# wadx2019/rpo

Measured on AMD Instinct MI355X. Metric: env-steps/sec (whole node), SafeCartpole-v0 (CartSafe-v0) RPODDPG, rollout + one batch-256 constrained policy update per vector step, higher is better.
Workload: dtype f32; 1 GPU; CartSafe-v0 RPODDPG, 4096 vectorised envs per MI355X, scripts/cart_exp.py hyper-parameters, update batch 256 every vector step (reference cadence), replay capacity 20000 per env; envs_per_gpu=4096, global_envs=4096, update_batch=256, hip_graph=True, training_batch_projection=row-wise, rccl_ranks=0, collectives_in_graph=False, graphs_replayed_on_all_ranks=True, graph_capture_fell_back_to_eager=False

## Files before the change

### include/rpo_hip.h

```cpp
#ifndef RPO_HIP_H
#define RPO_HIP_H

#ifdef __cplusplus
extern "C" {
#endif

#define RPO_ABI_VERSION 6

#define RPO_ERR_ARG (-1)
#define RPO_ERR_NULL (-2)

#define RPO_CART_STATE_DIM 6
#define RPO_CART_ACTION_DIM 2
#define RPO_CART_INEQ 6
#define RPO_CART_ROW 24
#define RPO_CART_RING 32
#define RPO_CART_CONSTS_LEN 35

#define RPO_PEND_INTERNAL_DIM 4
#define RPO_PEND_OBS_DIM 5
#define RPO_PEND_ACTION_DIM 2
#define RPO_PEND_ROW 16
#define RPO_PEND_RING 16

// ... 259 lines not shown
int rpo_mlp_split_head(const rpo_mlp* net_host, int n, const float* part, float* out, int out_mode, float scale,
                       float base, void* stream);

typedef struct {
    const rpo_mlp *actor, *actor_target, *critic1, *critic2, *critic_target1, *critic_target2;
    const rpo_mlp_grad *critic1_grad, *critic2_grad, *actor_grad;
    int env;
    int twin;
    int batch;
    const float* rows; long long cap_steps; int n_envs;
    float* batch_out; long long* idx_out; const long long* idx_in;
    unsigned long long sample_seed; unsigned sample_salt;
    const float* eps_in; unsigned long long noise_seed; unsigned noise_id_base, noise_salt;
    const long long* ctrl;
    float scale, base, box_lo, box_hi;
    int max_steps; float corr_lr, corr_eps, corr_momentum;
    const float* consts_host; int partial;
    float alpha, gamma;
    float eps_start, eps_end, eps_decay;
    float *part_pi, *part_q1, *part_q2, *part_qn1, *part_qn2;
    float *x0_1, *h1_1, *x0_2, *h1_2, *x0_a, *h1_a;
    float *logp;
    float *next_actions;
    int *proj_iters;
    float *dq1, *dq2;
    float *loss_partial;
    float *dx0_1, *dx0_2, *dx0_a;
    float *gradmax;
    const float* nu; float* nu_grad;
    float *ap_det, *noise_out, *raw, *actions, *g_act, *lag_partial, *lag_out, *da_part, *dout;
    int shared_embedding;
    long long* rollout_ctrl; float* rollout_stats; int rollout_stats_cap;
    int* prep_step; float prep_beta1, prep_beta2; long long* clock_out; float* gradmax_reset;
    int* prep2_step[3]; float prep2_beta1[3], prep2_beta2[3]; float* gradmax_reset2;
    long long* updates_out;
    float* part_pol;
    unsigned* tile_sync;
    unsigned long long* proj_ws; int proj_store_mode;
    int debug;
} rpo_split_update;


int rpo_split_critic_fwd_a(const rpo_split_update* u, void* stream);
int rpo_split_critic_fwd_b(const rpo_split_update* u, void* stream);
int rpo_split_critic_front(const rpo_split_update* u, void* stream);
int rpo_split_critic_front_pol(const rpo_split_update* u, void* stream);
int rpo_split_critic_mid(const rpo_split_update* u, void* stream);
int rpo_split_critic_mid_pol(const rpo_split_update* u, void* stream);
int rpo_split_critic_pfront(const rpo_split_update* u, void* stream);
int rpo_split_critic_pfront_pol(const rpo_split_update* u, void* stream);
int rpo_xcc_probe(int gx, int gy, int gz, int threads, int* out, void* stream);
int rpo_hw_probe(int gx, int gy, int gz, int threads, int lds_bytes, int spin, int* out, void* stream);
int rpo_split_critic_fwd_b_pol(const rpo_split_update* u, void* stream);
int rpo_split_pend_head_project(const rpo_split_update* u, void* stream);
int rpo_split_critic_bwd_a(const rpo_split_update* u, void* stream);
int rpo_split_critic_bwd_b(const rpo_split_update* u, void* stream);
int rpo_split_policy_a(const rpo_split_update* u, void* stream);
int rpo_split_policy_b(const rpo_split_update* u, void* stream);
int rpo_split_policy_c(const rpo_split_update* u, void* stream);
int rpo_split_policy_d(const rpo_split_update* u, void* stream);
int rpo_split_policy_e(const rpo_split_update* u, void* stream);
int rpo_split_policy_front(const rpo_split_update* u, void* stream);
int rpo_split_policy_front_bc(const rpo_split_update* u, void* stream);

typedef struct {
    int n_envs;
    int gauss;
    float scale, base;
    float* state;
    float* obs;
    float* action;
    int* ep_len; float* ep_ret; unsigned* ep_count;
    float* rows; long long cap_steps;
    float* stats; int stats_cap;
    int noise_mode;
    long long* ctrl;
    float eps_start, eps_end, eps_decay, box_lo, box_hi;
    int max_steps; float corr_lr, corr_eps, corr_momentum;
    int max_episode_steps, auto_reset;
    float viol_thresh;
    unsigned env_id_base;
    unsigned long long seed;
    float* part;
    int lane_begin, lane_end;
    int defer_clock;
} rpo_rollout_rider;

int rpo_split_critic_fwd_a_ride(const rpo_split_update* u, const rpo_rollout_rider* r, void* stream);
int rpo_split_critic_fwd_b_ride(const rpo_split_update* u, const rpo_rollout_rider* r, void* stream);
int rpo_split_critic_bwd_b_ride(const rpo_split_update* u, const rpo_rollout_rider* r, void* stream);
int rpo_split_critic_front_ride(const rpo_split_update* u, const rpo_rollout_rider* r, void* stream);
int rpo_split_critic_mid_ride(const rpo_split_update* u, const rpo_rollout_rider* r, void* stream);
int rpo_split_critic_pfront_ride(const rpo_split_update* u, const rpo_rollout_rider* r, void* stream);

int rpo_mlp_backward(const rpo_mlp* net_host, const rpo_mlp_grad* grad_host, int n, const float* s, int s_stride,
                     const float* a, int a_stride, const float* x0, const float* h1, const float* dout, float* dh,
                     float* dx0, float* da, int param_grads, int first_layer_state_only, float* gradmax,
                     const rpo_td* td, void* stream);

int rpo_mlp_backward_pair(const rpo_mlp* net1_host, const rpo_mlp_grad* grad1_host, const rpo_mlp* net2_host,
                          const rpo_mlp_grad* grad2_host, int n, const float* s, int s_stride, const float* a,
                          int a_stride, const float* x0_1, const float* h1_1, const float* dout_1, float* dh_1,
                          float* dx0_1, float* da_1, const float* x0_2, const float* h1_2, const float* dout_2, float* dh_2,
                          float* dx0_2, float* da_2, int param_grads, int first_layer_state_only, float* gradmax,
                          const rpo_td* td1, const rpo_td* td2, void* stream);


int rpo_evopf_reset(int n_envs, float* state, int* ep_len, float* ep_ret, const unsigned* ep_count,
                    const float* consts_dev, unsigned long long seed, unsigned env_id_base, void* stream);

int rpo_evopf_step(int n_envs, float* state, const float* action, int* ep_len, float* ep_ret, unsigned* ep_count,
                   float* rows, long long cap_steps, float* stats, int stats_cap, long long* ctrl, int max_episode_steps,
                   int auto_reset, float viol_thresh, const float* consts_dev, unsigned long long seed,
                   unsigned env_id_base, void* stream);

int rpo_evopf_act_project(int n, const float* state, int state_stride, const float* ap_raw, const float* noise, float* action, int* iters,
                          int noise_mode, int ap_is_raw, float eps_start, float eps_end, float eps_decay, int max_steps,
                          float corr_lr, float corr_eps, float corr_momentum, float newton_tol, int newton_max_iters,
                          const float* consts_dev, unsigned long long seed, unsigned env_id_base, const long long* ctrl,
                          float* stats, int stats_cap, void* stream);

int rpo_evopf_tanh_box_bwd(int n, const float* state, int state_stride, const float* raw, const float* noise,
                           float eps_start, float eps_end, float eps_decay, const long long* ctrl, const float* dap,
                           float* dout, const float* consts_dev, void* stream);

int rpo_evopf_gauss_head(int n, const float* state, int state_stride, const float* raw, const float* eps, int deterministic,
                         float* ap_out, float* logp_out, const float* consts_dev, void* stream);
int rpo_evopf_gauss_head_bwd(int n, const float* state, int state_stride, const float* raw, const float* eps,
                             const float* dap, float dlogp, float* draw, const float* consts_dev, void* stream);

int rpo_evopf_complete_bwd(int n, const float* action, const float* grad_action, const float* grad_action_b, const float* grad_action2,
                           float* grad_ap, const float* consts_dev, void* stream);

int rpo_evopf_resid(int n, const float* state, int state_stride, const float* action, float* eq_out, float* ineq_out,
                    const float* consts_dev, void* stream);

int rpo_evopf_ineq_partial_grad(int n, const float* state, int state_stride, const float* action, float* step_out, const float* consts_dev,
                                void* stream);

int rpo_evopf_eq_vjp(int n, const float* action, const float* grad_eq, float* grad_action, int autograd_sign,
                     const float* consts_dev, void* stream);

int rpo_evopf_lagrangian(int n, const float* state, int state_stride, const float* action, const float* nu, float scale, float* loss_out,
                         float* grad_action, float* grad_nu, const float* consts_dev, int overwrite, void* stream);


int rpo_cartsafe_rollout(const rpo_mlp* actor_host, int gauss, float scale, float base, int n_envs, float* state,
                         float* action, int* ep_len, float* ep_ret, unsigned* ep_count, float* rows, long long cap_steps,
                         float* stats, int stats_cap, long long* ctrl, int noise_mode, float eps_start, float eps_end,
                         float eps_decay, float box_lo, float box_hi, int max_steps, float corr_lr, float corr_eps,
                         float corr_momentum, const float* consts_host, int partial, int max_episode_steps,
                         int auto_reset, float viol_thresh, unsigned long long seed, unsigned env_id_base, int defer_clock,
                         void* stream);
int rpo_pendulum_rollout(const rpo_mlp* actor_host, int gauss, float scale, float base, int n_envs, float* internal,
                         float* obs, float* action, int* ep_len, float* ep_ret, unsigned* ep_count, float* rows,
                         long long cap_steps, float* stats, int stats_cap, long long* ctrl, int noise_mode,
                         float eps_start, float eps_end, float eps_decay, float box_lo, float box_hi, int max_steps,
                         float corr_lr, float corr_eps, float corr_momentum, int max_episode_steps, int auto_reset,
                         float viol_thresh, unsigned long long seed, unsigned env_id_base, int defer_clock, void* stream);

int rpo_cartsafe_evaluate(const rpo_mlp* actor_host, int gauss, float scale, float base, int n_envs, float* state,
                          float* action, int* ep_len, float* ep_ret, unsigned* ep_count, long long* ctrl, float* acc, int t0,
                          int steps, float box_lo, float box_hi, int max_steps, float corr_lr, float corr_eps,
                          float corr_momentum, const float* consts_host, int partial, int max_episode_steps,
                          float viol_thresh, void* stream);
int rpo_pendulum_evaluate(const rpo_mlp* actor_host, int gauss, float scale, float base, int n_envs, float* internal,
                          float* obs, float* action, int* ep_len, float* ep_ret, unsigned* ep_count, long long* ctrl,
                          float* acc, int t0, int steps, float box_lo, float box_hi, int max_steps, float corr_lr,
                          float corr_eps, float corr_momentum, int max_episode_steps, float viol_thresh, void* stream);

int rpo_cartsafe_evaluate_record(const rpo_mlp* actor_host, int gauss, float scale, float base, int n_envs, float* state,
                                 float* action, int* ep_len, float* ep_ret, unsigned* ep_count, long long* ctrl, float* acc,
                                 int t0, int steps, float box_lo, float box_hi, int max_steps, float corr_lr, float corr_eps,
                                 float corr_momentum, const float* consts_host, int partial, int max_episode_steps,
                                 float viol_thresh, float* trace, int trace_rows, int trace_steps, void* stream);
int rpo_pendulum_evaluate_record(const rpo_mlp* actor_host, int gauss, float scale, float base, int n_envs, float* internal,
                                 float* obs, float* action, int* ep_len, float* ep_ret, unsigned* ep_count, long long* ctrl,
                                 float* acc, int t0, int steps, float box_lo, float box_hi, int max_steps, float corr_lr,
                                 float corr_eps, float corr_momentum, int max_episode_steps, float viol_thresh, float* trace,
                                 int trace_rows, int trace_steps, void* stream);

int rpo_cartsafe_evaluate_constraints(const rpo_mlp* actor_host, int gauss, float scale, float base, int n_envs, float* state,
                                      float* action, int* ep_len, float* ep_ret, unsigned* ep_count, long long* ctrl,
                                      float* acc, int t0, int steps, float box_lo, float box_hi, int max_steps, float corr_lr,
                                      float corr_eps, float corr_momentum, const float* consts_host, int partial,
                                      int max_episode_steps, float viol_thresh, float* trace, int trace_rows, int trace_steps,
                                      float* con, void* stream);
int rpo_pendulum_evaluate_constraints(const rpo_mlp* actor_host, int gauss, float scale, float base, int n_envs,
                                      float* internal, float* obs, float* action, int* ep_len, float* ep_ret,
                                      unsigned* ep_count, long long* ctrl, float* acc, int t0, int steps, float box_lo,
                                      float box_hi, int max_steps, float corr_lr, float corr_eps, float corr_momentum,
                                      int max_episode_steps, float viol_thresh, float* trace, int trace_rows, int trace_steps,
                                      float* con, void* stream);

int rpo_cartsafe_evaluate_noisy(const rpo_mlp* actor_host, int gauss, float scale, float base, int n_envs, float* state,
                                float* action, int* ep_len, float* ep_ret, unsigned* ep_count, long long* ctrl, float* acc,
                                int t0, int steps, float box_lo, float box_hi, int max_steps, float corr_lr, float corr_eps,
                                float corr_momentum, const float* consts_host, int partial, int max_episode_steps,
                                float viol_thresh, float* trace, int trace_rows, int trace_steps, float* con,
                                const float* sigma_host, int sigma_len, unsigned long long noise_seed, void* stream);
int rpo_pendulum_evaluate_noisy(const rpo_mlp* actor_host, int gauss, float scale, float base, int n_envs, float* internal,
                                float* obs, float* action, int* ep_len, float* ep_ret, unsigned* ep_count, long long* ctrl,
                                float* acc, int t0, int steps, float box_lo, float box_hi, int max_steps, float corr_lr,
                                float corr_eps, float corr_momentum, int max_episode_steps, float viol_thresh, float* trace,
                                int trace_rows, int trace_steps, float* con, const float* sigma_host, int sigma_len,
                                unsigned long long noise_seed, void* stream);

int rpo_cartsafe_evaluate_budgets(const rpo_mlp* actor_host, int gauss, float scale, float base, int n_envs, float* state,
                                  float* action, int* ep_len, float* ep_ret, unsigned* ep_count, long long* ctrl, float* acc,
                                  int t0, int steps, float box_lo, float box_hi, int max_steps, float corr_lr, float corr_eps,
                                  float corr_momentum, const float* consts_host, int partial, int max_episode_steps,
                                  float viol_thresh, float* trace, int trace_rows, int trace_steps, float* con,
                                  const int* lane_steps, const float* lane_lr, void* stream);
int rpo_pendulum_evaluate_budgets(const rpo_mlp* actor_host, int gauss, float scale, float base, int n_envs, float* internal,
                                  float* obs, float* action, int* ep_len, float* ep_ret, unsigned* ep_count, long long* ctrl,
                                  float* acc, int t0, int steps, float box_lo, float box_hi, int max_steps, float corr_lr,
                                  float corr_eps, float corr_momentum, int max_episode_steps, float viol_thresh, float* trace,
                                  int trace_rows, int trace_steps, float* con, const int* lane_steps, const float* lane_lr,
                                  void* stream);

int rpo_cartsafe_evaluate_policies(const rpo_mlp* actor_host, int gauss, float scale, float base, int n_envs, float* state,
                                   float* action, int* ep_len, float* ep_ret, unsigned* ep_count, long long* ctrl, float* acc,
                                   int t0, int steps, float box_lo, float box_hi, int max_steps, float corr_lr, float corr_eps,
                                   float corr_momentum, const float* consts_host, int partial, int max_episode_steps,
                                   float viol_thresh, float* con, int policy_stride, int group_lanes, int episodes,
                                   void* stream);
int rpo_pendulum_evaluate_policies(const rpo_mlp* actor_host, int gauss, float scale, float base, int n_envs, float* internal,
                                   float* obs, float* action, int* ep_len, float* ep_ret, unsigned* ep_count, long long* ctrl,
                                   float* acc, int t0, int steps, float box_lo, float box_hi, int max_steps, float corr_lr,
                                   float corr_eps, float corr_momentum, int max_episode_steps, float viol_thresh, float* con,
                                   int policy_stride, int group_lanes, int episodes, void* stream);

int rpo_cartsafe_evaluate_noise_sweep(const rpo_mlp* actor_host, int gauss, float scale, float base, int n_envs, float* state,
                                      float* action, int* ep_len, float* ep_ret, unsigned* ep_count, long long* ctrl,
                                      float* acc, int t0, int steps, float box_lo, float box_hi, int max_steps, float corr_lr,
                                      float corr_eps, float corr_momentum, const float* consts_host, int partial,
                                      int max_episode_steps, float viol_thresh, float* con, const float* sigma_table,
                                      unsigned long long noise_seed, int group_lanes, int episodes, void* stream);
int rpo_pendulum_evaluate_noise_sweep(const rpo_mlp* actor_host, int gauss, float scale, float base, int n_envs,
                                      float* internal, float* obs, float* action, int* ep_len, float* ep_ret,
                                      unsigned* ep_count, long long* ctrl, float* acc, int t0, int steps, float box_lo,
                                      float box_hi, int max_steps, float corr_lr, float corr_eps, float corr_momentum,
                                      int max_episode_steps, float viol_thresh, float* con, const float* sigma_table,
                                      unsigned long long noise_seed, int group_lanes, int episodes, void* stream);

int rpo_eval_obs_noise(int n, const float* obs, int obs_stride, int obs_dim, const float* sigma, unsigned long long seed,
                       int step, float* out, int out_stride, void* stream);

int rpo_cartsafe_policy_act(const rpo_mlp* actor_host, int gauss, float scale, float base, int n, const float* obs,
                            int obs_stride, float* action, float* proposal, int* iters, float* eq_resid, float* ineq_resid,
                            float box_lo, float box_hi, int max_steps, float corr_lr, float corr_eps, float corr_momentum,
                            const float* consts_host, int partial, int form, void* stream);
int rpo_pendulum_policy_act(const rpo_mlp* actor_host, int gauss, float scale, float base, int n, const float* obs,
                            int obs_stride, float* action, float* proposal, int* iters, float* eq_resid, float* ineq_resid,
                            float box_lo, float box_hi, int max_steps, float corr_lr, float corr_eps, float corr_momentum,
                            int form, void* stream);

int rpo_cartsafe_policy_act_profile(const rpo_mlp* actor_host, int gauss, float scale, float base, int n, const float* obs,
                                    int obs_stride, float* action, float* proposal, int* iters, float* eq_resid,
                                    float* ineq_resid, float box_lo, float box_hi, int max_steps, float corr_lr, float corr_eps,
                                    float corr_momentum, const float* consts_host, int partial, float* profile, void* stream);
int rpo_pendulum_policy_act_profile(const rpo_mlp* actor_host, int gauss, float scale, float base, int n, const float* obs,
                                    int obs_stride, float* action, float* proposal, int* iters, float* eq_resid,
                                    float* ineq_resid, float box_lo, float box_hi, int max_steps, float corr_lr, float corr_eps,
                                    float corr_momentum, float* profile, void* stream);
int rpo_cartsafe_project_profile(int n, const float* ap_raw, float* action, int* iters, int max_steps, float corr_lr,
                                 float corr_eps, float corr_momentum, const float* consts_host, int partial, float* profile,
                                 void* stream);
int rpo_pendulum_project_profile(int n, const float* obs, int obs_stride, const float* ap_raw, float* action, int* iters,
                                 int max_steps, float corr_lr, float corr_eps, float corr_momentum, float* profile,
                                 void* stream);

int rpo_eval_record(int n, const float* rows, int row_stride, int reward_col, int done_col, int eq_col, int eq_num,
                    int ineq_col, int ineq_num, const float* obs, int obs_stride, int obs_dim, const float* proposal,
                    int partial_dim, const float* action, int action_dim, const int* iters, int step, const float* acc,
                    float* trace, int trace_rows, int trace_steps, void* stream);

int rpo_eval_constraints(int n, const float* rows, int row_stride, int eq_col, int eq_num, int ineq_col, int ineq_num, int step,
                         float viol_thresh, const float* acc, float* con, void* stream);

int rpo_eval_accumulate(int n, const float* rows, int row_stride, int reward_col, int done_col, int eq_col, int eq_num,
                        int ineq_col, int ineq_num, const int* iters, int step, float viol_thresh, float* acc, void* stream);

int rpo_eval_summarize(int n, const float* acc, const long long* ctrl, double* row_out, double* ws, void* stream);

int rpo_eval_keep_best(long long n_params, const float* src, float* best, const double* row, double* best_row,
                       long long* best_point, long long point, double max_violation_rate, void* stream);

int rpo_cartsafe_ddpg_critic_forward(const rpo_mlp* actor_target_host, const rpo_mlp* critic_target_host,
                                     const rpo_mlp* critic_host, float scale, float base, const float* rows,
                                     long long cap_steps, int n_envs, int batch, float* batch_out, long long* idx_out,
                                     const long long* idx_in, unsigned long long seed, unsigned sample_salt,
                                     const long long* ctrl, int max_steps, float corr_lr, float corr_eps,
                                     float corr_momentum, float box_lo, float box_hi, const float* consts_host,
                                     int partial, float* q_out, float* qn_out, float* x0_save, float* h1_save,
                                     void* stream);

int rpo_ddpg_actor_forward(int env, const rpo_mlp* actor_host, const rpo_mlp* critic_host, float scale, float base,
                                    float box_lo, float box_hi, float eps_start, float eps_end, float eps_decay,
                                    const float* batch, int batch_size, const float* noise_in, unsigned long long seed,
                                    unsigned noise_id_base, unsigned noise_salt, const long long* ctrl, const float* nu,
                                    const float* consts_host, int partial, float* ap_det, float* noise_out,
                                    float* actions, float* q_out, float* dq_out, float* g_act, float* partial_out,
                                    float* actor_x0, float* actor_h1, float* critic_x0, float* critic_h1, void* stream);
int rpo_ddpg_actor_backward(int env, const rpo_mlp* actor_host, const rpo_mlp_grad* actor_grad_host,
                                     const rpo_mlp* critic_host, int shared_embedding, const float* batch,
// ... 73 lines not shown
```

### rpo_amd/algo/rpo_ddpg.py

```python
import torch

from .. import ops as hip_ops
from .agent import PDDDPG_PA
from .model import BoxConstraint
from .agent.flat import FusedAdam
from .trainer import _SALT_ACTOR, RPOTrainerBase, _LagrangianFn, _TDHuberFn


class _LazySum(object):

    def __init__(self, parts):
        self.parts = parts

    def __float__(self):
        return float(self.parts.sum())

    def detach(self):
        return self.parts.sum()


class _LazyDiff(object):

    def __init__(self, pair):
        self.pair = pair
# ... 105 lines not shown
        td = self.backend.Td(q.view(-1), qn.view(-1), None, None, cols[3], cols[4], 0.0, self.agent.gamma,
                             f.buf("dq", B, 1).view(-1), parts)
        self._zero_grads()
        gm = self._critic_gradmax()
        f.backward("critic", cols[0], cols[1], None, gradmax=gm, td=td)
        self._gradmax_ready = gm is not None
        self.last_losses["critic"] = _LazySum(parts)

    def _critic_update(self, cols):
        if self.fused is None:
            return super()._critic_update(cols)
        if self._pipelines:
            su = self._split_state()
            if su is not None:
                return self._critic_update_split(su)
            return self._critic_update_pipeline(cols)
        f, ag, B = self.fused, self.agent, self.batch_size
        state, action, next_state, reward, done = cols[:5]
        next_actions = self._project_batch(next_state, self._actor_out("actor_target", next_state))
        qn, q = f.forward_multi([("critic_target", next_state, next_actions, f.buf("qn", B, 1), False),
                                 ("critic", state, action, f.buf("q", B, 1), True)])
        self._critic_backward_td(cols, q, qn, f.buf("loss_parts", (B + 15) // 16))

    @property
    def _actor_pipeline(self):
        d = self.fused.descs if self.fused is not None else {}
        return (hasattr(self.backend, "ddpg_actor_forward") and "actor" in d and "critic" in d and d["actor"].E == 128
                and d["critic"].E == 128 and not d["critic"].cat and self._box_affine is not None
                and self.kernels.partial_dim == 1 and self.kernels.action_dim == 2
                and self.schedule["fused_actor"] and not self._large_batch)

    def _actor_update_pipeline(self, cols):
        f, ag, B, k = self.fused, self.agent, self.batch_size, self.kernels
        da_, dc = f.descs["actor"], f.descs["critic"]
        scale, base = self._box_affine
        b = f.buf
        parts = b("actor.parts", (B + 15) // 16, 8)
        ap_det, noise, actions = b("act.ap_det", B), b("act.noise", B), b("act_pi", B, k.action_dim)
        q, dq, g_act = b("q_pi", B, 1), b("dq_pi", B, 1), b("g_act", B, k.action_dim)
        noise_in = None
        if self._idx_inject is not None:
            self.backend.philox_normal(self._noise_b, self.seed, self.dist.rank * B * k.partial_dim, _SALT_ACTOR, hip_ops.STREAM_POLICY,
                                       self._uctrl)
            noise_in = self._noise_b.view(-1)
        self.backend.ddpg_actor_forward(k, da_, dc, scale, base, self._box_lo, self._box_hi, self.eps_start, self.eps, self.decay_value,
                             self._batch, noise_in, self.seed, self.dist.rank * B, _SALT_ACTOR, self._uctrl,
                             ag.nju.weight.view(-1), ap_det, noise, actions, q, dq, g_act, parts, b("actor.x0", B, da_.ein),
                             b("actor.h1", B, da_.H), b("critic.x0", B, dc.ein), b("critic.h1", B, dc.H))
        self._zero_grads()
        shared = ag.flat.sizes[1] > 0
        opt = ag.actor_optim
        fuse_max = self._self_cleaning and not self.dist.on and opt.clip_thres and opt.clip_thres != float("inf")
        lag = b("actor.lag", 2)
        self.backend.ddpg_actor_backward(k, da_, dc, shared, self._batch, actions, g_act, ap_det, noise, dq, self.eps_start, self.eps,
                              self.decay_value, self._box_lo, self._box_hi, scale, base, self._uctrl,
                              b("actor.x0", B, da_.ein), b("actor.h1", B, da_.H), b("critic.x0", B, dc.ein),
                              b("critic.h1", B, dc.H), b("actor.dh", B, da_.H), b("actor.dx0", B, da_.ein),
                              b("critic.dh", B, dc.H), b("critic.dx0", B, dc.ein), b("da", B, k.action_dim), b("do", B),
                              parts, lag, ag.nju.weight.grad.view(-1), opt.gradmax if fuse_max else None)
        self._actor_gradmax_ready = bool(fuse_max)
        loss = _LazyDiff(lag)
        self.last_losses["actor"] = loss
        return loss

    def _actor_update(self, cols):
        if self.fused is None:
            return super()._actor_update(cols)
        if self._actor_pipeline:
            su = self._split_state()
            if su is not None:
                lag, _, _ = self._actor_update_split(su)
                loss = _LazyDiff(lag)
                self.last_losses["actor"] = loss
                return loss
            return self._actor_update_pipeline(cols)
        f, ag, B, k = self.fused, self.agent, self.batch_size, self.kernels
        state = cols[0]
        pre, self._actor_pre = getattr(self, "_actor_pre", None), None
        if pre is None:
            pre = self._actor_prefix(cols)
        ap_det, noise, actions, lag, g_act, fa = pre
        q = f.forward("critic", state, actions, f.buf("q_pi", B, 1), save=True)
        dq = self._const_dq(B)
        da = f.buf("da", B, k.action_dim)
        shared = ag.flat.sizes[1] > 0
        f.backward("critic", state, actions, dq, da=da, param_grads=shared, first_layer_state_only=True)
        P = k.partial_dim
        dap, do = f.buf("dap", B * P), f.buf("do", B, P)
        if fa:
            k.complete_bwd(state, da, dap, action=actions, grad_action2=g_act)
        else:
            da.add_(g_act)
            k.complete_bwd(state, da, dap, action=actions)
        if self._box_affine is None:
            k.tanh_box_bwd(state, ap_det, noise, self.eps_start, self.eps, self.decay_value, self._uctrl, dap, do.view(-1))
        else:
            scale, base = self._box_affine
            self.backend.tanh_box_bwd(dap, ap_det, noise, self.eps_start, self.eps, self.decay_value, self._uctrl,
                                      self._box_lo, self._box_hi, scale, base, do.view(-1))
        opt = ag.actor_optim
        fuse_max = self._self_cleaning and not self.dist.on and opt.clip_thres and opt.clip_thres != float("inf") and not shared
        f.backward("actor", state, None, do, gradmax=opt.gradmax if fuse_max else None)
        self._actor_gradmax_ready = bool(fuse_max)
        loss = _LazyMeanDiff(lag, q)
        self.last_losses["actor"] = loss
        return loss

    def _actor_prefix(self, cols):
        f, ag, B, k = self.fused, self.agent, self.batch_size, self.kernels
        state = cols[0]
        ap_det = self._actor_out("actor", state, save=True, tag="pi")
        self.backend.philox_normal(self._noise_b, self.seed, self.dist.rank * B * k.partial_dim, _SALT_ACTOR, hip_ops.STREAM_POLICY,
                                   self._uctrl)
        noise = self._noise_b.view(-1)
        actions = self._complete_only(state, ap_det, noise)
        lag, g_act = f.buf("loss_lag", 1), f.buf("g_act", B, k.action_dim)
        fa = bool(getattr(k, "fused_adds", False))
        if not fa:
            lag.zero_()
        self._zero_grads()
        k.lagrangian(actions, ag.nju.weight.view(-1), 1.0 / B, lag, g_act, ag.nju.weight.grad.view(-1), obs=state,
                     **(dict(overwrite=True) if fa else {}))
        return ap_det, noise, actions, lag, g_act, fa

    def _const_dq(self, B):
        key = ("dq_pi_const", B)
        if key not in self.fused._scratch:
            self.fused._scratch[key] = torch.full((B, 1), -1.0 / B, device=self.device)
        return self.fused._scratch[key]

    def critic_loss(self, state, action, next_state, done, reward, ineq_viol=None, eq_viol=None):
        ag = self.agent
        with torch.no_grad():
            next_partial = ag.take_action(next_state, deterministic=True, target=True)
            next_actions = self.process_action(next_state, next_partial)
            next_q = ag.critic_target(next_state, next_actions)
        q = ag.critic(state, action)
        return _TDHuberFn.apply(self.backend, ag.gamma, 0.0, reward, done, next_q, None, None, q, None)

    def actor_loss(self, state):
        ag = self.agent
        ap = ag.actor(state)
        self.backend.philox_normal(self._noise_b, self.seed, self.dist.rank * self.batch_size * self.kernels.partial_dim, _SALT_ACTOR,
                                   hip_ops.STREAM_POLICY, self._uctrl)
        ap = ag.actor.box_constraint.clip(ap + self._eps_now() * self._noise_b, state)
        actions = self.base_env.complete_partial(state, ap)
        loss = (-ag.critic(state, actions)).mean()
        return loss + _LagrangianFn.apply(self.kernels, actions, ag.nju.weight, state)

    def _critic_step(self, actor_step):
        ag = self.agent
        fuse = actor_step and ag.flat.sizes[1] == 0
        prepared, self._critic_prepared = getattr(self, "_critic_prepared", False), False
        ag.critic_optim.step(target=ag.critic_target_flat if fuse else None, tau=ag.tau,
                             gradmax_ready=self._gradmax_ready, clock=self._clock(not actor_step), prepared=prepared)
        self._gradmax_ready = False

    def _actor_step(self, actor_out):
        ag, fl = self.agent, self.agent.flat
        c = fl.actor_range[0]
        sh = fl.critic_range[1] - c if fl.sizes[1] > 0 else 0
        segs = [ag.actor_optim.segment(target=ag.actor_target_flat, tau=ag.tau,
                                       gradmax_ready=getattr(self, "_actor_gradmax_ready", False),
                                       target2=ag.critic_target_flat[c:c + sh] if sh > 0 else None, n2=sh)]
        self._actor_gradmax_ready = False
        if not self.fixed:
            segs.append(ag.nju_optim.segment())
        if sh > 0 and c > 0:
            segs.append(dict(polyak_only=True, param=fl.param((0, c)), target=ag.critic_target_flat[:c], tau=ag.tau))
        prepared, self._actor_prepared = getattr(self, "_actor_prepared", False), False
        FusedAdam.step_many(self.backend, segs, clock=self._clock(True), prepared=prepared)
```

### rpo_amd/algo/trainer.py

```python
import contextlib
import copy
import os

import numpy as np
import torch
import torch.distributed as dist

from .. import ops as hip_ops
from .agent.fused import FusedNets
from .model import BoxConstraint



class NonFiniteError(FloatingPointError):
    """An env lane was stepped with a NaN action or reached a non-finite state (ctrl[RPO_CTRL_NONFINITE] of the step
    kernels; the reference's `assert self.action_space.contains(action_fixed)`, cartpole.py:170-174, pendulum.py:85-89)."""


_SALT_CRITIC = 1 << 20
_SALT_ACTOR = 2 << 20


class _TDHuberFn(torch.autograd.Function):

# ... 29 lines not shown
        return loss[0]

    @staticmethod
    def backward(ctx, grad_out):
        g_a, g_nu = ctx.saved_tensors
        return None, grad_out * g_a, grad_out * g_nu.view(ctx.nu_shape), None


class _Dist(object):
    def __init__(self, force=False):
        init = dist.is_available() and dist.is_initialized()
        self.on = init and (dist.get_world_size() > 1 or bool(force))
        self.rank = dist.get_rank() if self.on else 0
        self.world = dist.get_world_size() if self.on else 1
        self.in_graph = self.on and dist.get_backend() == "nccl"

    def mean_(self, tensors):
        if not self.on:
            return
        avg = dist.get_backend() == "nccl"
        for t in tensors:
            if avg:
                dist.all_reduce(t, op=dist.ReduceOp.AVG)
            else:
                dist.all_reduce(t, op=dist.ReduceOp.SUM)
                t.mul_(1.0 / self.world)

    def sync_initial_state(self, seed, agent, device):
        bufs = [agent.flat.data, agent.critic_target_flat]
        if agent.actor_target_flat is not None:
            bufs.append(agent.actor_target_flat)
        for b in bufs:
            dist.broadcast(b, src=0)
        s = torch.tensor([int(seed)], dtype=torch.int64, device=device)
        dist.broadcast(s, src=0)
        return int(s.item())

    def sum_(self, t):
        if self.on:
            dist.all_reduce(t, op=dist.ReduceOp.SUM)
        return t

    def all_ok(self, ok, device):
        if not self.on:
            return bool(ok)
        flag = torch.tensor([1 if ok else 0], dtype=torch.int32, device=device)
        dist.all_reduce(flag, op=dist.ReduceOp.MIN)
        return bool(int(flag.item()))

    def replaying_everywhere(self, graphs, device):
        mine = bool(graphs.enabled and not graphs.capture_failed and any(e["graph"] is not None for e in graphs.entries.values()))
        return self.all_ok(mine, device)


_NODE_KINDS = ("kernel", "memcpy", "memset", "host", "graph", "empty", "wait_event", "event_record", "sem_signal", "sem_wait",
               "mem_alloc", "mem_free", "memcpy_from_symbol", "memcpy_to_symbol", "batch_mem_op")


def _graph_node_kinds(g):
    import ctypes
    from .. import _lib
    _lib._bind_to_torch_hip_runtime()
    bundled = os.path.join(os.path.dirname(torch.__file__), "lib", "libamdhip64.so")
    hip = ctypes.CDLL(bundled if os.path.exists(bundled) else "libamdhip64.so", mode=ctypes.RTLD_GLOBAL)
    graph = ctypes.c_void_p(int(g.raw_cuda_graph()))
    n = ctypes.c_size_t(0)
    if hip.hipGraphGetNodes(graph, None, ctypes.byref(n)) != 0:
        raise RuntimeError("hipGraphGetNodes failed")
    nodes = (ctypes.c_void_p * max(1, n.value))()
    if n.value and hip.hipGraphGetNodes(graph, nodes, ctypes.byref(n)) != 0:
        raise RuntimeError("hipGraphGetNodes failed")
    kinds = {}
    for i in range(n.value):
        t = ctypes.c_int(-1)
        if hip.hipGraphNodeGetType(ctypes.c_void_p(nodes[i]), ctypes.byref(t)) != 0:
            raise RuntimeError("hipGraphNodeGetType failed")
        name = _NODE_KINDS[t.value] if 0 <= t.value < len(_NODE_KINDS) else "type_%d" % t.value
        kinds[name] = kinds.get(name, 0) + 1
    return kinds


class _GraphCache(object):

    def __init__(self, enabled, warm=3, owner=None):
        self.enabled, self.warm = enabled, warm
        self.capture_failed = False
        self.entries = {}
        self.side = None
        self.audit = os.environ.get("RPO_GRAPH_AUDIT", "0") == "1"
        import weakref
        self._owner = weakref.ref(owner) if owner is not None else None

    def run(self, key, fn):
        if not self.enabled:
            return fn()
        e = self.entries.setdefault(key, {"count": 0, "graph": None})
        if e["graph"] is not None:
            e["graph"].replay()
            return
        if e["count"] < self.warm:
            e["count"] += 1
            if self.side is None:
                self.side = torch.cuda.Stream()
            cur = torch.cuda.current_stream()
            self.side.wait_stream(cur)
            with torch.cuda.stream(self.side):
                fn()
            cur.wait_stream(self.side)
            return
        g = torch.cuda.CUDAGraph(keep_graph=True) if self.audit else torch.cuda.CUDAGraph()
        owner = self._owner() if self._owner is not None else None
        state = owner._host_state() if owner is not None else None
        import gc
        gc_was_on = gc.isenabled()
        gc.collect()
        gc.disable()
        failure = None
        try:
            try:
                with torch.cuda.graph(g, capture_error_mode="thread_local"):
                    fn()
            except Exception as exc:
                failure = exc
            ok_everywhere = failure is None
            if owner is not None and owner.dist.on and owner.dist.world > 1:
                ok_everywhere = owner.dist.all_ok(failure is None, owner.device)
            if not ok_everywhere:
                import warnings
                why = "%s: %s" % (type(failure).__name__, failure) if failure is not None else "another rank's capture failed"
                warnings.warn("hipGraph capture failed (%s); continuing with eager launches" % why)
                self.enabled = False
                self.capture_failed = True
                del g
                torch.cuda.synchronize()
                if owner is not None:
                    owner._set_host_state(state)
                fn()
                return
            e["graph"] = g
            if self.audit:
                e["node_kinds"] = _graph_node_kinds(g)
            g.replay()
        finally:
            if gc_was_on:
                gc.enable()


def _env_int(name, default):
    v = os.environ.get(name)
    return default if v in (None, "") else int(v)


SCHEDULE_DEFAULTS = dict(fused_mlp=1, fused_rollout=1, fused_critic=1, fused_actor=1, split=1, ride=1, front=1, branch=1,
                         fused_eval=1, fused_act=1, eval_overlap=1, force_dist=0)


def parse_schedule(overrides=None):
    out = dict(SCHEDULE_DEFAULTS)
    text = os.environ.get("RPO_SCHEDULE", "")
    for item in filter(None, (x.strip() for x in text.split(","))):
        k, _, v = item.partition("=")
        if k.strip() not in out:
            raise ValueError("RPO_SCHEDULE: unknown part %r (have: %s)" % (k, ", ".join(sorted(out))))
        out[k.strip()] = int(v) if v.strip() else 1
    for k, v in (overrides or {}).items():
        if k not in out:
            raise ValueError("schedule: unknown part %r (have: %s)" % (k, ", ".join(sorted(out))))
        out[k] = int(v)
    return out


class RPOTrainerBase(object):

    sac = False

    def _setup(self, env, work_dir, name, logger, agent, hp, device, num_envs=None, seed=None, backend=None,
               use_graph=None, updates_per_step=None, fused=None, schedule=None):
        self.env, self.agent, self.device = env, agent, device
        self.schedule = parse_schedule(schedule)
        if fused is not None:
            self.schedule["fused_mlp"] = int(bool(fused))
        self.work_dir, self.name, self.logger = work_dir, name, logger
        for k, v in hp.items():
            setattr(self, k, v)
        if self.eval_steps is None:
            self.eval_steps = self.max_steps
        if self.corr_mode != 0:
            raise ValueError("corr_mode=%r: only corr_mode=0 (reduced-gradient projection) is defined; the reference's "
                             "corr_mode=1 branch (rpo_ddpg.py:276-278) raises a shape error for every env" % (self.corr_mode,))
        self.backend = backend if backend is not None else hip_ops
        self.base_env = getattr(env, "unwrapped", env)
        self.kernels = self.base_env.kernels
        self.env_eval = copy.deepcopy(self.env)
        self.box_constraint = BoxConstraint(*self.base_env.box_constraint, device=device)
        self.decay_value = (hp["eps_start"] - hp["eps"]) / hp["eps_epoch"]
        self.dist = _Dist(force=self.schedule["force_dist"])
        n_total = int(num_envs) if num_envs is not None else _env_int("RPO_NUM_ENVS", 1)
        if n_total % self.dist.world:
            raise ValueError("num_envs (%d) must be divisible by the world size (%d)" % (n_total, self.dist.world))
        self.num_envs, self.n_local = n_total, n_total // self.dist.world
        if seed is None:
            seed = _env_int("RPO_SEED", None)
        if seed is None:
            seed = int(torch.randint(0, 2 ** 62, (1,)).item())
        if self.dist.on:
            seed = self.dist.sync_initial_state(seed, agent, device)
        self.seed = int(seed)
        self.max_episode_steps = getattr(env, "_max_episode_steps", None)
        self.vec = self.base_env.make_vec(self.n_local, seed=self.seed, env_id_base=self.dist.rank * self.n_local,
                                          max_episode_steps=self.max_episode_steps, device=device)
        self.buffer = agent.attach_env(self.kernels, self.n_local, self.seed + 7919 * (self.dist.rank + 1), self.vec.ctrl)
        self._batch = torch.zeros(self.batch_size, self.kernels.row_floats, device=device)
        P = self.kernels.partial_dim
        self._noise_b = torch.zeros(self.batch_size, P, device=device)
        self._noise_n = torch.zeros(self.n_local, P, device=device)
        self._box_lo, self._box_hi = self.base_env.partial_box
        cycle = _env_int("RPO_GRAPH_CYCLE", 16)
        if use_graph is None:
            use_graph = cycle > 0 and device.type == "cuda"
        self._graphs = _GraphCache(use_graph, owner=self)
        self._tail = None
        self._last_cols = self._last_actor_out = None
        self._cycle = max(cycle, 1) // max(1, self.policy_fre) * max(1, self.policy_fre)
        rowwise = _env_int("RPO_ROWWISE_PROJECTION", None)
        self.batch_reference = not bool(rowwise)
        if self.batch_size > 1024 and self.batch_reference and hasattr(self.kernels, "project_batchref"):
            raise ValueError(
                "batch_size=%d > 1024 on %s: the reference's sample-coupled batched projection is defined up to 1024 rows "
                "here; set RPO_ROWWISE_PROJECTION=1 to project training batches row by row (per-sample stop test, "
                "no coupling between samples)" % (self.batch_size, self.kernels.name))
        self.projection_mode = ("batch-reference" if self.batch_reference and hasattr(self.kernels, "project_batchref")
                                else "row-wise")
        self.fused = FusedNets.build(agent, self.backend, device) if self.schedule["fused_mlp"] else None
        if self.fused is not None and self.batch_size >= hip_ops.CONST.get("RPO_SPLITK_FROM", 1 << 30) and device.type == "cuda":
            self.fused.enable_splitk(self.batch_size)
        self.updates_per_step = max(1, int(updates_per_step) if updates_per_step is not None
                                    else _env_int("RPO_UPDATES_PER_STEP", 1))
        self._updates = 0
        box = agent.actor.box_constraint
        self._box_affine = (float(np.asarray(box.scale).reshape(-1)[0]), float(np.asarray(box.base).reshape(-1)[0])) \
            if box is not None and not box.volatile else None
        self._self_cleaning = self.fused is not None
        self._gradmax_ready = False
        for opt in (agent.critic_optim, agent.actor_optim, agent.nju_optim):
            opt.zero_grad_after = self._self_cleaning
        self._act_kw = dict(ap_is_raw=True) if (self.fused is not None and self._box_affine is None) else {}
        self._uctrl, self._uclock_ok, self._ovl_stream = self.vec.ctrl, True, None
        self._ride, self._rider_cache, self._ride_cut = None, None, 0
        self._clock_pending, self._iter_actor_step, self._critic_prepared, self._gradmax_stale = False, None, False, False
        self._actor_prepared, self._actor_gradmax_stale = False, False
        self._bump_updates_now, self._updates_out, self._pol_a_done = False, None, False
        self._bump = self.updates_per_step == 1
        if self.fused is not None and device.type == "cuda" and getattr(self.backend, "ADAM_CLOCK", False):
            self._uctrl, self._uclock_ok = torch.zeros_like(self.vec.ctrl), False
        self.buffer.sample_ctrl = self._uctrl
        self._split_state()
        self._t = 0
        self._harvested = 0
        self._pending = []
        self._vec_eval = None
        self.last_losses = {}
        self._idx_inject = None
        self._eval_init_inject = None
        self.viol_steps, self.env_steps, self.viol_rate, self.proj_iters_mean = 0.0, 0.0, 0.0, 0.0
        from .evaluation import CurveRunner
        ee = getattr(self, "eval_episodes", None)
        if ee is None:
            ee = _env_int("RPO_EVAL_EPISODES", None)
        from .evaluation import check_keep_best, keep_best_from_env
        kb = getattr(self, "keep_best", None)
        if kb is None:
            kb = keep_best_from_env(os.environ.get("RPO_KEEP_BEST"))
        kb = check_keep_best(kb)
        if kb is not None and ee is None:
            raise ValueError("keep_best needs curve mode: the points it chooses among are those of eval_episodes=N "
                             "(RPO_EVAL_EPISODES), which is not set")
        self._curve = CurveRunner(self, ee, keep_best=kb) if ee is not None else None
        self.eval_episodes = self._curve.n if self._curve is not None else None
        self.keep_best = False if kb is None else kb

    def process_action(self, state, action_partial, train=True):
        ref = self.batch_reference
        if train:
            return self.base_env.project(state, action_partial, self.max_steps, self.corr_lr, self.corr_eps,
                                         self.corr_momentum, batch_reference=ref)
        action, iters = self.base_env.project(state, action_partial, self.eval_steps, self.eval_lr, self.corr_eps,
                                              self.corr_momentum, return_iters=True, batch_reference=ref)
        return action, int(iters.max())

    def grad_steps(self, state, action, train=True):
        idx = torch.as_tensor(np.asarray(self.base_env.partial_actions), device=self.device)
        return self.process_action(state, torch.as_tensor(action, device=self.device)[:, idx], train=train)

    def _policy_partial(self, obs, warm):
        raise NotImplementedError

    _gauss_policy = False

    @property
    def _large_batch(self):
        return self.batch_size >= hip_ops.CONST.get("RPO_SPLITK_FROM", 1 << 30)

    @property
    def _rollout_pipeline(self):
        return (self.fused is not None and hasattr(self.kernels, "rollout") and "actor" in self.fused.descs
                and self.schedule["fused_rollout"])

    @property
    def _defer_ok(self):
        return bool(getattr(self, "_pipelines", False) and self._split_state() is not None)

    def _rollout(self, warm, defer_clock=False):
        v = self.vec
        defer_clock = bool(defer_clock and not warm and self._rollout_pipeline and self._defer_ok)
        if not warm and self._rollout_pipeline:
            scale, base = self._box_affine
            self.kernels.rollout(self.fused.descs["actor"], self._gauss_policy, scale, base, v.internal,
                                 None if v.obs is v.internal else v.obs, v.action, v.ep_len, v.ep_ret, v.ep_count,
                                 self.buffer.rows, self.buffer.capacity, v.stats, v.ctrl,
                                 hip_ops.NOISE_NONE if self._gauss_policy else hip_ops.NOISE_PHILOX, self.eps_start,
                                 self.eps, self.decay_value, self._box_lo, self._box_hi, self.max_steps, self.corr_lr,
                                 self.corr_eps, self.corr_momentum, v.max_episode_steps, True, v.viol_thresh, self.seed,
                                 v.env_id_base, **(dict(defer_clock=True) if defer_clock else {}))
            self._clock_pending = defer_clock
            v.steps_host += 1
            return
        with torch.no_grad():
            ap, mode = self._policy_partial(v.obs, warm)
            self.kernels.act_project(v.obs, ap, None, v.action, None, mode, self.eps_start, self.eps, self.decay_value,
                                     self._box_lo, self._box_hi, self.max_steps, self.corr_lr, self.corr_eps,
                                     self.corr_momentum, self.seed, v.env_id_base, v.ctrl, v.stats,
                                     **({} if warm else self._act_kw))
            v.step(v.action, rows=self.buffer.rows, cap_steps=self.buffer.capacity, auto_reset=True)

    def _sample(self):
        self.buffer.sample_rows(self.batch_size, out=self._batch)
        c = self.buffer.split(self._batch)
        return c["state"], c["action"], c["next_state"], c["reward"], c["done"], c["ineq_viol"], c["eq_viol"]

    def _eps_now(self):
        if self.decay_value == 0:
            return self.eps_start
        t = self._uctrl[0].to(torch.float32)
        return torch.clamp(self.eps_start - self.decay_value * t, min=self.eps)

    def _critic_gradmax(self):
        opt = self.agent.critic_optim
        ok = self._self_cleaning and not self.dist.on and opt.clip_thres and opt.clip_thres != float("inf")
        self._gradmax_ready = False
        return opt.gradmax if ok else None

    def _zero_grads(self):
        if not self._self_cleaning:
            self.agent.flat.grad.zero_()
        elif self.fixed:
            self.agent.nju.weight.grad.zero_()

    def _critic_update(self, cols):
        state, action, next_state, reward, done, ineq_viol, eq_viol = cols
        loss = self.critic_loss(state, action, next_state, done, reward, ineq_viol, eq_viol)
        self.agent.flat.grad.zero_()
        loss.backward()
        self.last_losses["critic"] = loss.detach()

    def _actor_update(self, cols):
        out = self.actor_loss(cols[0])
        loss = out[0] if isinstance(out, tuple) else out
        self.agent.flat.grad.zero_()
        loss.backward()
        self.last_losses["actor"] = loss.detach()
        return tuple(x.detach() for x in out) if isinstance(out, tuple) else loss.detach()

    def _segments(self, warm, do_train, actor_step, rollout=True):
        ag, fl = self.agent, self.agent.flat
        segs = []
        if not do_train:
            return [(lambda: self._rollout(warm), [])]

        def s1():
            if rollout:
                self._rollout(warm, defer_clock=True)
            self._last_cols = self._sample()
            self._iter_actor_step = actor_step
            self._bump_updates_now = self._updates_inkernel
            self._critic_update(self._last_cols)
        segs.append((s1, [fl.gradient(fl.critic_range)]))
        if actor_step:
            def s2():
                self._critic_step(actor_step)
                self._last_actor_out = self._actor_update(self._last_cols)
            segs.append((s2, [fl.gradient(fl.policy_bucket)]))

            def s3():
                self._actor_step(self._last_actor_out)
            segs.append((s3, []))
        else:
            segs.append((lambda: self._critic_step(actor_step), []))
        return segs

    def _critic_step(self, actor_step):
        raise NotImplementedError

    def _clock(self, last):
        return self._uctrl if (last and self._bump and self._uctrl is not self.vec.ctrl) else None

    def _sync_uclock(self, rollout_pending):
        if self._uctrl is self.vec.ctrl or self._uclock_ok:
            return
        if rollout_pending:
            torch.add(self.vec.ctrl[0:1], 1, out=self._uctrl[0:1])
        else:
            self._uctrl[0:1].copy_(self.vec.ctrl[0:1])

    def _actor_step(self, actor_out):
        raise NotImplementedError

    def _policy_optims(self):
        ag = self.agent
        out = [ag.actor_optim]
        if not self.fixed:
            out.append(ag.nju_optim)
        if getattr(self, "automatic_entropy_tuning", False):
            out.append(ag.alpha_optim)
        return out

    def _iteration(self, warm, do_train, actor_step, rollout=True):
        segs = self._segments(warm, do_train, actor_step, rollout)
        if do_train:
            self._sync_uclock(rollout_pending=rollout)
        self._uclock_ok = do_train and self._bump
        if not self.dist.on or self.dist.in_graph:
            self._graphs.run((warm, do_train, actor_step, rollout), lambda: self._run_segments(segs))
            return
        tail, self._tail = self._tail, None
        for i, (fn, reduce_after) in enumerate(segs):
            key = (warm, do_train, actor_step, rollout, i)
            if i == 0 and tail is not None:
                prev_fn, first = tail[1], fn
                key, fn = ("after",) + tail[0] + key, (lambda: (prev_fn(), first()))
            if i == len(segs) - 1 and not reduce_after and i > 0:
                self._tail = (key, fn)
                return
            self._graphs.run(key, fn)
            self.dist.mean_(reduce_after)

    def _run_segments(self, segs):
        for fn, reduce_after in segs:
            fn()
            self.dist.mean_(reduce_after)

    def _flush_tail(self):
        tail, self._tail = self._tail, None
        if tail is not None:
            self._graphs.run(tail[0], tail[1])

    @property
    def _updates_inkernel(self):
        return bool(self.updates_per_step > 1 and getattr(self, "_pipelines", False) and getattr(self, "_actor_pipeline", False)
                    and self._split_state() is not None)

    def _extra_body(self, actor_step):
        if self._updates_inkernel:
            self._bump_updates_now = True
        else:
            self._uctrl[hip_ops.CONST["RPO_CTRL_UPDATES"]] += 1
        cols = self._sample()
        self._iter_actor_step = actor_step
        self._critic_update(cols)
        fl = self.agent.flat
        self.dist.mean_([fl.gradient(fl.critic_range)])
        self._critic_step(actor_step)
        if actor_step:
            out = self._actor_update(cols)
            self.dist.mean_([fl.gradient(fl.policy_bucket)])
            self._actor_step(out)

    def _extra_updates(self):
        F, k, U = self.policy_fre, 1, self.updates_per_step
        while k < U:
            L = self._cycle
            if L > 1 and U - k >= L and self._updates % F == 0 and self._graphs.enabled and \
                    (not self.dist.on or self.dist.in_graph):
                base = self._updates
                self._graphs.run(("extra", L), lambda: [self._extra_body((base + j + 1) % F == 0) for j in range(L)])
            else:
                L = 1
                actor_step = (self._updates + 1) % F == 0
                if self.dist.on and not self.dist.in_graph:
                    self._extra_body(actor_step)
                else:
                    self._graphs.run(("extra", actor_step), lambda: self._extra_body(actor_step))
            self._updates += L
            k += L

    def train(self, t):
        self._uclock_ok = False
        self._sync_uclock(rollout_pending=False)
        bump, self._bump = self._bump, False
        try:
            self._train_body(t)
        finally:
            self._bump = bump
            self._uclock_ok = False

    def _train_body(self, t):
        cols = self._sample()
        actor_step = self._iter_actor_step = t % self.policy_fre == 0
        self._critic_update(cols)
        fl = self.agent.flat
        self.dist.mean_([fl.gradient(fl.critic_range)])
        self._critic_step(actor_step)
        if actor_step:
            out = self._actor_update(cols)
            self.dist.mean_([fl.gradient(fl.policy_bucket)])
            self._actor_step(out)

    def _split_state(self):
        if getattr(self, "_split_cache", False) is not False:
            return self._split_cache
        self._split_cache = None
        f, k, be = self.fused, self.kernels, self.backend
        if f is None or not hasattr(be, "SplitUpdate") or not self.schedule["split"] or self._box_affine is None \
                or self.device.type != "cuda":
            return None
        if not isinstance(k, (be.CartSafeKernels, be.PendulumKernels)) or self.batch_size > 1024:
            return None
        if isinstance(k, be.PendulumKernels) and not self.batch_reference:
            return None
        d = f.descs
        names = ("actor", "critic1", "critic2", "critic_target1", "critic_target2") if self.sac else \
            ("actor", "actor_target", "critic", "critic_target")
        if any(n not in d or not be.mlp_split_supported(d[n]) for n in names):
            return None
        B, ag, buf = self.batch_size, self.agent, self.buffer
        T = (B + 15) // 16
        b = f.buf
        descs = dict(actor=d["actor"])
        if self.sac:
            descs.update(critic1=d["critic1"], critic2=d["critic2"], critic_target1=d["critic_target1"],
                         critic_target2=d["critic_target2"])
        else:
            descs.update(actor_target=d["actor_target"], critic1=d["critic"], critic_target1=d["critic_target"])
        scale, base = self._box_affine
        c1 = "critic1" if self.sac else "critic"
        fields = dict(
            rows=buf.rows, cap_steps=buf.capacity, n_envs=buf.n_envs, batch_out=self._batch, sample_seed=buf.seed,
            sample_salt=0, noise_seed=self.seed, noise_id_base=self.dist.rank * B, noise_salt=_SALT_CRITIC, ctrl=self._uctrl,
            scale=scale, base=base, box_lo=self._box_lo, box_hi=self._box_hi, max_steps=self.max_steps,
            corr_lr=self.corr_lr, corr_eps=self.corr_eps, corr_momentum=self.corr_momentum,
            alpha=float(getattr(ag, "alpha", 0.0)), gamma=ag.gamma, eps_start=self.eps_start, eps_end=self.eps,
            eps_decay=self.decay_value,
            part_pi=b("split.part_pi", 8, B, 2), part_pol=b("split.part_pol", 8, B, 2),
            part_q1=b("split.part_q1", 8, B, 2), part_qn1=b("split.part_qn1", 8, B, 2),
            x0_1=b(c1 + ".x0", B, d[c1].ein), h1_1=b(c1 + ".h1", B, d[c1].H), dq1=b("dq1" if self.sac else "dq", B, 1),
            dx0_1=b(c1 + ".dx0", B, d[c1].ein), loss_partial=b("split.loss_parts", 2, T),
            next_actions=b("split.next_actions", B, 2), logp=b("crit.logp", B),
            tile_sync=torch.zeros((3 * T + 1) * 32, dtype=torch.int32, device=self.device))
        if self.sac:
            fields.update(part_q2=b("split.part_q2", 8, B, 2), part_qn2=b("split.part_qn2", 8, B, 2),
                          x0_2=b("critic2.x0", B, d["critic2"].ein), h1_2=b("critic2.h1", B, d["critic2"].H),
                          dq2=b("dq2", B, 1), dx0_2=b("critic2.dx0", B, d["critic2"].ein))
        da_ = d["actor"]
        fields.update(nu=ag.nju.weight.view(-1), nu_grad=ag.nju.weight.grad.view(-1), noise_out=b("act.noise", B),
                      actions=b("act_pi", B, 2), g_act=b("g_act", B, 2), lag_partial=b("actor.parts", T, 8),
                      lag_out=b("actor.lag", 2), da_part=b("split.da_part", 2, 8, B, 2), dout=b("split.dout", B, 2),
                      x0_a=b("actor.x0", B, da_.ein), h1_a=b("actor.h1", B, da_.H), dx0_a=b("actor.dx0", B, da_.ein),
                      shared_embedding=int(ag.flat.sizes[1] > 0))
        if self.sac:
            fields.update(raw=b("pi.raw", B, 2))
        else:
            fields.update(ap_det=b("act.ap_det", B))
        if isinstance(k, be.PendulumKernels) and self.schedule["front"] and B <= 256 and self.max_steps <= 30:
            fields.update(proj_ws=torch.zeros(hip_ops.PROJ_WS_WORDS, dtype=torch.int64, device=self.device), proj_store_mode=1)
        self._split_cache = be.SplitUpdate(k, descs, self.sac, B, fields)
        self._front_cache = bool(self.schedule["front"]) and hasattr(be, "front_launch_ok") and be.front_launch_ok(B, self.sac)
        self._pfront = bool(self._front_cache and "proj_ws" in fields and be.front_launch_ok(B, self.sac, 1))
        self._split_loss = fields["loss_partial"]
        self._split_logp = (fields["logp"], b("pi.logp", B))
        return self._split_cache

    def _actor_update_split(self, su):
        B, ag, k = self.batch_size, self.agent, self.kernels
        noise_in = None
        if self._idx_inject is not None:
            self.backend.philox_normal(self._noise_b, self.seed, self.dist.rank * B * k.partial_dim, _SALT_ACTOR,
                                       hip_ops.STREAM_POLICY, self._uctrl)
            noise_in = self._noise_b.view(-1)
        crit_logp, pi_logp = self._split_logp
        su.set(noise_salt=_SALT_ACTOR, eps_in=noise_in, logp=pi_logp)
        early, self._pol_a_done = self._pol_a_done, False
        front = self._front_ok()
        if front:
            su.run("policy_front_bc" if early else "policy_front")
        else:
            if not early:
                su.run("policy_a")
            su.run("policy_b")
            su.run("policy_c")
        self._zero_grads()
        opt = ag.actor_optim
        fuse_max = self._self_cleaning and not self.dist.on and opt.clip_thres and opt.clip_thres != float("inf")
        su.set(gradmax=opt.gradmax if fuse_max else None)
        if not front:
            su.run("policy_d")
        prep = bool(fuse_max) and bool(getattr(self, "_pipelines", False))
        optims = [o for o in self._policy_optims() if o is not None] if prep else []
        su.set_prep2([(o.step_dev, o.betas[0], o.betas[1]) for o in optims])
        su.set(clock_out=self._clock(True) if prep else None, updates_out=self._updates_out)
        su.run("policy_e")
        su.set(clock_out=None, updates_out=None)
        self._updates_out = None
        self._actor_prepared = prep
        self._actor_gradmax_stale = prep
        su.set(noise_salt=_SALT_CRITIC, eps_in=None, logp=crit_logp)
        self._actor_gradmax_ready = bool(fuse_max)
        f = self.fused
        return f.buf("actor.lag", 2), f.buf("actor.parts", (B + 15) // 16, 8), pi_logp

    def _set_hand_overs(self, su, actor_step):
        opt = self.agent.critic_optim
        prep = actor_step is not None
        self._critic_prepared = bool(prep)
        bump_updates, self._bump_updates_now = self._bump_updates_now, False
        self._updates_out = self._uctrl if bump_updates else None
        pending, self._clock_pending = self._clock_pending, False
        su.set(prep_step=opt.step_dev if prep else None, prep_beta1=opt.betas[0], prep_beta2=opt.betas[1],
               clock_out=self._clock(not actor_step) if prep else None,
               updates_out=self._updates_out if not actor_step else None,
               gradmax_reset=opt.gradmax if (prep or self._gradmax_stale) else None,
               gradmax_reset2=self.agent.actor_optim.gradmax if (prep or self._actor_gradmax_stale) else None,
               rollout_ctrl=self.vec.ctrl if pending else None, rollout_stats=self.vec.stats if pending else None,
               rollout_stats_cap=self.vec.stats.shape[0] if pending else 0)
        self._gradmax_stale, self._actor_gradmax_stale = bool(prep), False

    def _critic_update_split(self, su):
        inject = self._idx_inject is not None
        idx_in = self._idx_inject() if inject else None
        eps_in = None
        if inject and self.sac:
            B = self.batch_size
            self.backend.philox_normal(self._noise_b, self.seed, self.dist.rank * B * self.kernels.partial_dim, _SALT_CRITIC,
                                       hip_ops.STREAM_POLICY, self._uctrl)
            eps_in = self._noise_b.view(-1)
        buf = self.buffer
        su.set(idx_in=idx_in, eps_in=eps_in, rows=buf.rows, cap_steps=buf.capacity, n_envs=buf.n_envs)
        actor_step, self._iter_actor_step = self._iter_actor_step, None
        self._set_hand_overs(su, actor_step)
        ride = self._ride
        if ride is not None:
            n, cut = self.vec.internal.shape[0], self._ride_cut
            ride.set(lane_begin=0, lane_end=cut)
        early = bool(actor_step) and ride is None and self.agent.flat.sizes[1] == 0 and getattr(self, "_actor_pipeline", False)
        if su.st.env == 0 and self._front_ok():
            self._pol_a_done = early
            if ride is not None:
                ride.set(lane_begin=0, lane_end=n)
            su.run("critic_front_pol" if early else "critic_front", rider=ride)
            self._critic_update_split_back(su, ride, bwd_a=False)
            return
        if su.st.env == 1 and self._pfront:
            self._pol_a_done = early
            if ride is not None:
                ride.set(lane_begin=0, lane_end=n)
            su.run("critic_pfront_pol" if early else "critic_pfront", rider=ride)
            self._critic_update_split_back(su, ride, bwd_a=False)
            return
        su.run("critic_fwd_a", rider=ride)
        if su.st.env == 1:
            su.run("pend_head_project")
        if ride is not None:
            ride.set(lane_begin=cut, lane_end=n)
        self._pol_a_done = early
        if su.st.env == 1 and self._front_ok():
            su.run("critic_mid_pol" if early else "critic_mid", rider=ride)
            self._critic_update_split_back(su, ride, bwd_a=False)
            return
        su.run("critic_fwd_b_pol" if early else "critic_fwd_b", rider=ride)
        self._critic_update_split_back(su, ride)

    _HOST_STATE = ("_actor_pre", "_clock_pending", "_iter_actor_step", "_critic_prepared", "_gradmax_stale", "_actor_prepared",
                   "_actor_gradmax_stale", "_pol_a_done", "_gradmax_ready", "_actor_gradmax_ready", "_bump_updates_now",
                   "_updates_out", "_last_cols", "_last_actor_out")

    def _host_state(self):
        import ctypes
        st = {k: getattr(self, k) for k in self._HOST_STATE if hasattr(self, k)}
        st["steps_host"] = self.vec.steps_host
        su = getattr(self, "_split_cache", None)
        if su:
            st["su"] = (ctypes.string_at(ctypes.addressof(su.st), ctypes.sizeof(su.st)), dict(su._held))
        rc = getattr(self, "_rider_cache", None)
        if rc is not None and hasattr(rc, "st"):
            st["rider"] = ctypes.string_at(ctypes.addressof(rc.st), ctypes.sizeof(rc.st))
        return st

    def _set_host_state(self, st):
        import ctypes
        st = dict(st)
        self.vec.steps_host = st.pop("steps_host")
        su_state, rider = st.pop("su", None), st.pop("rider", None)
        if su_state is not None:
            ctypes.memmove(ctypes.addressof(self._split_cache.st), su_state[0], len(su_state[0]))
            self._split_cache._held = dict(su_state[1])
        if rider is not None:
            ctypes.memmove(ctypes.addressof(self._rider_cache.st), rider, len(rider))
        for k, v in st.items():
            setattr(self, k, v)

    def _handover_flags(self):
        su = getattr(self, "_split_cache", None)
        sync = su._held.get("tile_sync") if su else None
        ws = su._held.get("proj_ws") if su else None
        return (sync[-32:-31] if sync is not None and getattr(self, "_front_cache", False) else None,
                ws[hip_ops.PROJ_WS_GAVE_UP:hip_ops.PROJ_WS_GAVE_UP + 1] if ws is not None else None)

    def _device_flags(self):
        f, g = self._handover_flags()
        nf = hip_ops.CONST["RPO_CTRL_NONFINITE"]
        return [(k, x) for k, x in (("front", f), ("proj", g), ("nonfinite", self.vec.ctrl[nf:nf + 1])) if x is not None]

    def _raise_flags(self, vals):
        if vals.get("front"):
            raise RuntimeError("rpo_split_*_front: a workgroup gave up waiting for its row tile (tile_sync flag set); the "
                               "values of that launch are undefined -- rerun with RPO_SCHEDULE=front=0")
        if vals.get("proj"):
            raise RuntimeError("rpo_split_pend_head_project / rpo_split_critic_pfront: a workgroup gave up waiting for another "
                               "one's granules (workspace flag set); the values of that launch are undefined -- rerun with "
                               "RPO_SCHEDULE=front=0")
        if vals.get("nonfinite"):
            raise NonFiniteError("vector step %d (0-based): an env lane was stepped with a NaN action or reached a non-finite "
                                 "next state / reward (ctrl[RPO_CTRL_NONFINITE]).  The reference stops at this point too "
                                 "(`assert self.action_space.contains(action_fixed)`, cartpole.py:170-174); the transitions "
                                 "of that step are in the replay ring, so this trainer must not be trained on or "
                                 "checkpointed -- restart from the last checkpoint" % (int(vals["nonfinite"]) - 1))

    def _check_flags(self):
        vals = {k: int(x[0]) for k, x in self._device_flags()}
        if self.dist.on:
            kinds = ("front", "proj", "nonfinite")
            word = torch.tensor([vals.get(k, 0) for k in kinds], dtype=torch.int64, device=self.device)
            dist.all_reduce(word, op=dist.ReduceOp.MAX)
            vals = dict(zip(kinds, word.tolist()))
        self._raise_flags(vals)

    def _poll_flags(self, every=4):
        if self.device.type != "cuda":
            return self._raise_flags({k: int(x[0]) for k, x in self._device_flags()})
        st = getattr(self, "_flag_poll", None)
        if st is None:
            st = self._flag_poll = dict(event=None, calls=0, host={}, pending=[])
        if st["event"] is not None:
            if not st["event"].query():
                return
            st["event"] = None
            self._raise_flags({k: int(st["host"][k][0]) for k in st["pending"]})
        st["calls"] += 1
        if every > 1 and st["calls"] % every != 1:
            return
        flags = self._device_flags()
        st["pending"] = [k for k, _ in flags]
        for k, x in flags:
            h = st["host"].get(k)
            if h is None or h.dtype != x.dtype:
                h = st["host"][k] = torch.zeros(1, dtype=x.dtype).pin_memory()
            h.copy_(x, non_blocking=True)
        st["event"] = torch.cuda.Event()
        st["event"].record()

    def _front_ok(self):
        return self._front_cache

    def _critic_update_split_back(self, su, ride, bwd_a=True):
        self._zero_grads()
        gm = self._critic_gradmax()
        su.set(gradmax=gm)
        if bwd_a:
            su.run("critic_bwd_a")
        if ride is not None:
            ride.set(defer_clock=int(self._defer_ok))
        su.run("critic_bwd_b", rider=ride)
        if ride is not None:
            self._clock_pending = bool(self._defer_ok)
            self.vec.steps_host += 1
        self._gradmax_ready = gm is not None
        from .rpo_ddpg import _LazySum
        self.last_losses["critic"] = _LazySum(self._split_loss if self.sac else self._split_loss[0])

    def _project_batch(self, state, ap_flat):
        return self.base_env.project(state, ap_flat, self.max_steps, self.corr_lr, self.corr_eps, self.corr_momentum,
                                     batch_reference=self.batch_reference, **self._act_kw)

    def _complete_only(self, state, ap_flat, noise=None):
        f = self.fused
        act = f.buf("act_pi", state.shape[0], self.kernels.action_dim)
        mode = hip_ops.NOISE_NONE if noise is None else hip_ops.NOISE_EXPLICIT
        self.kernels.act_project(state, ap_flat, noise, act, None, mode, self.eps_start, self.eps, self.decay_value,
                                 self._box_lo, self._box_hi, 0, 0.0, self.corr_eps, 0.0, self.seed, 0, self._uctrl, None,
                                 **self._act_kw)
        return act

    def run(self, logger=None, eval=True):
        if logger is not None:
            self.logger = logger
        if self._t == 0:
            self.vec.reset()
        self.run_steps(self.max_epochs - self._t, eval=eval)
        self._harvest(final=True)

    def run_steps(self, n, eval=False, train=True):
        left = int(n)
        while left > 0:
            t = self._t
            warm = t < self.warmup
            do_train = train and (t + 1) >= self.warmup
            actor_step = do_train and (t + 1) % self.policy_fre == 0
            L = self._cycle_len(t, left, warm, do_train, eval)
            eval_now = eval and (t + 1) % self.eval_fre == 0 and (t + 1) > self.warmup
            if eval_now and do_train:
                self._iteration(warm, False, False)
                self._advance_host(t + 1)
                self._flush_tail()
                self._evaluation_point(t + 1)
                self._iteration(warm, True, actor_step, rollout=False)
                self._updates += 1
                if self.updates_per_step > 1:
                    self._flush_tail()
                    self._extra_updates()
                    self._uctrl[hip_ops.CONST["RPO_CTRL_UPDATES"]] = 0
                left -= 1
                if self._curve is not None:
                    self._poll_flags(every=16)
                    if t + 1 - self._harvested >= self.vec.stats.shape[0] // 2:
                        self._harvest()
                continue
            if L > 1:
                if do_train:
                    self._sync_uclock(rollout_pending=True)
                self._uclock_ok = do_train and self._bump
                if self._ride_ok(do_train):
                    self._graphs.run(("cycle", L, True, "ride"), lambda: self._ridden_window(t, L))
                elif self._overlap_ok(do_train):
                    self._graphs.run(("cycle", L, True, "overlap"), lambda: self._overlapped_window(t, L))
                else:
                    self._graphs.run(("cycle", L, do_train), lambda: [self._run_segments(self._segments(
                        False, do_train, do_train and (t + i + 1) % self.policy_fre == 0)) for i in range(L)])
                self._updates += L if do_train else 0
                self._poll_flags()
            else:
                self._iteration(warm, do_train, actor_step)
                self._poll_flags(every=16)
                if do_train:
                    self._updates += 1
                    if self.updates_per_step > 1:
                        self._flush_tail()
                        self._extra_updates()
                        self._uctrl[hip_ops.CONST["RPO_CTRL_UPDATES"]] = 0
            for _ in range(L):
                t = t + 1
                self._advance_host(t)
            left -= L
            if t - self._harvested >= self.vec.stats.shape[0] // 2:
                self._harvest()
            if eval_now:
                self._flush_tail()
                self._evaluation_point(t)
        self._flush_tail()

    def _evaluation_point(self, t):
        if self._curve is not None:
            self._curve.enqueue()
            return
        self._harvest()
        self._print_eval(t, self.eval())

    @property
    def eval_curve(self):
        from .evaluation import EvalCurve
        if self._curve is None:
            return EvalCurve()
        self._curve.harvest()
        return EvalCurve(self._curve.rows)

    @property
    def eval_curve_last(self):
        return None if self._curve is None else self._curve.last()

    @property
    def best(self):
        return None if self._curve is None else self._curve.best_policy()

    def _need_keep_best(self, what):
        if self._curve is None or self._curve.keep_rate is None:
            raise ValueError("%s needs keep_best (with eval_episodes=N): this trainer keeps no best policy" % what)
        return self._curve

    def restore_best(self):
        self._need_keep_best("restore_best()").restore_best()

    @contextlib.contextmanager
    def using_best(self):
        curve = self._need_keep_best("using_best()")
        curve._alloc_best()
        with torch.no_grad():
            stash = curve.live.clone()
        curve.restore_best()
        try:
            yield self
        finally:
            with torch.no_grad():
                curve.live.copy_(stash)

    def policy_params(self):
        from .evaluation import policy_params
        return policy_params(self)

    def using_policy(self, policy):
        from .evaluation import using_policy
        return using_policy(self, policy)

    def _advance_host(self, t):
        self._t = t
        self.buffer.note_step()
        self.agent.eps_decay(self.decay_value, self.eps)
        self.vec.steps_host = t

    def _ride_ok(self, do_train):
        if not (do_train and self._uctrl is not self.vec.ctrl and self.agent.flat.sizes[1] == 0 and self._bump):
            return False
        if not (getattr(self, "_pipelines", False) and self._split_state() is not None and self._rollout_pipeline):
            return False
        return bool(self.schedule["ride"])

    def _rider(self):
        v, buf = self.vec, self.buffer
        if self._rider_cache is None:
            scale, base = self._box_affine
            self._rider_cache = self.backend.RolloutRider(
                ring_floats=self.kernels.ring_floats, n_envs=v.internal.shape[0], gauss=int(self._gauss_policy), scale=scale, base=base, state=v.internal,
                obs=None if v.obs is v.internal else v.obs, action=v.action, ep_len=v.ep_len, ep_ret=v.ep_ret,
                ep_count=v.ep_count, stats=v.stats, stats_cap=v.stats.shape[0], ctrl=v.ctrl,
                noise_mode=hip_ops.NOISE_NONE if self._gauss_policy else hip_ops.NOISE_PHILOX, eps_start=self.eps_start,
                eps_end=self.eps, eps_decay=self.decay_value, box_lo=self._box_lo, box_hi=self._box_hi,
                max_steps=self.max_steps, corr_lr=self.corr_lr, corr_eps=self.corr_eps, corr_momentum=self.corr_momentum,
                max_episode_steps=v.max_episode_steps, auto_reset=1, viol_thresh=v.viol_thresh, seed=self.seed,
                env_id_base=v.env_id_base, part=self.fused.buf("ride.part", 8, v.internal.shape[0], 2))
        self._rider_cache.set(rows=buf.rows, cap_steps=buf.capacity)
        n = v.internal.shape[0]
        self._ride_cut = min(n, (n // 2 + 15) // 16 * 16)
        return self._rider_cache

    def _ridden_window(self, t, L):
        F, fl = self.policy_fre, self.agent.flat
        self._rollout(False, defer_clock=True)
        for i in range(L):
            actor_step = (t + i + 1) % F == 0
            more = i + 1 < L
            ride = more and not actor_step
            self._ride = self._rider() if ride else None
            self._iter_actor_step = actor_step
            try:
                cols = self._last_cols = self._sample()
                self._critic_update(cols)
            finally:
                self._ride = None
            self.dist.mean_([fl.gradient(fl.critic_range)])
            self._critic_step(actor_step)
            if actor_step:
                self._last_actor_out = self._actor_update(cols)
                self.dist.mean_([fl.gradient(fl.policy_bucket)])
                self._actor_step(self._last_actor_out)
            if more and not ride:
                self._rollout(False, defer_clock=True)

    def _overlap_ok(self, do_train):
        if not (do_train and self._uctrl is not self.vec.ctrl and self.agent.flat.sizes[1] == 0 and self._bump):
            return False
        if getattr(self, "_pipelines", False):
            return False
        return bool(self.schedule["branch"] and getattr(self, "_overlap_enabled", True))

    def _policy_prefix_ok(self):
        return bool(self.fused is not None and hasattr(self, "_actor_prefix") and not getattr(self, "_actor_pipeline", False)
                    and self.agent.flat.sizes[1] == 0 and not self.fixed and getattr(self, "_policy_prefix_enabled", True))

    def _overlapped_window(self, t, L):
        F, fl = self.policy_fre, self.agent.flat
        main = torch.cuda.current_stream()
        if self._ovl_stream is None:
            self._ovl_stream = torch.cuda.Stream()
        side = self._ovl_stream
        self._rollout(False)
        for i in range(L):
            actor_step = (t + i + 1) % F == 0
            more = i + 1 < L
            overlap = more and not actor_step

            self._iter_actor_step = actor_step
            cols = self._last_cols = self._sample()
# ... 244 lines not shown
```

### rpo_amd/csrc/fused.hip

```cpp
#include <stdlib.h>

#include <type_traits>

#include "cartsafe_dev.h"
#include "heads_dev.h"
#include "mlp_bwd.h"
#include "mlp_tile.h"
#include "pendulum_dev.h"
#include "rollout_args.h"
#include "rollout_env.h"

namespace {

using namespace rpo_mlp_dev;
using rpo_cart_dev::ActArgs;
using rpo_cart_dev::CartConsts;
using rpo_cart_dev::cart_explore_project;
using rpo_cart_dev::load_consts;

Mlp to_dev(const rpo_mlp* h) {
    return Mlp{h->Ws, h->bs, h->Wa, h->ba, h->W0, h->b0, h->W1, h->b1, h->W1b, h->b1b, h->S, h->A, h->E, h->H, h->n_out, h->cat, h->head_dim};
}


#ifndef RPO_ROLLOUT_SKIP
#define RPO_ROLLOUT_SKIP 0
#endif

template <class ENV, int EIN, int H, int RT>
__global__ __launch_bounds__(kFwdThreads) void rollout_kernel(RolloutArgs<ENV> p, typename ENV::Consts c) {
    typedef TileLds<EIN, RT, 8, 8> Lds;
    __shared__ Lds lds;
    constexpr int kInS = Lds::kS;
    constexpr int kLanes = rpo_mlp_dev::kRows * RT;
    constexpr int kStats = 10;
    const int row0 = blockIdx.x * kLanes;
    const int tid = threadIdx.x;
    const int n = p.step.n;
    const long long t = p.step.ctrl ? p.step.ctrl[RPO_CTRL_T] : 0;
    RpoEpisode ep{0, 0.0f, 0u};
    if (tid < kLanes && row0 + tid < n) ep = ENV::episode(p.step, row0 + tid);
    ENV::stage_obs(p.step, row0, kLanes, lds.in_s, kInS);
    float draw = 0.0f;
    const bool philox_noise = !p.gauss && p.act.noise_mode == RPO_NOISE_PHILOX;
    if (!(RPO_ROLLOUT_SKIP & 8) && tid < kLanes && row0 + tid < n && (p.gauss || philox_noise)) {
        const rpo_u4 u = p.gauss ? rpo_philox(p.act.seed, p.act.env_id_base + (uint32_t)(row0 + tid), (uint32_t)t, RPO_STREAM_POLICY,
                                              (uint32_t)p.step.ctrl[RPO_CTRL_UPDATES])
                                 : rpo_philox(p.act.seed, p.act.env_id_base + (uint32_t)(row0 + tid), (uint32_t)t, RPO_STREAM_ACT);
        draw = rpo_normal(u.x, u.y);
    }
    if (RPO_ROLLOUT_SKIP & 1) {
        if (tid < 2 * kLanes) lds.out[tid] = 0.25f;
        __syncthreads();
    } else {
        mlp_tile_forward<EIN, H, RT, Lds>(p.actor, lds, row0, n, nullptr, nullptr, p.gauss ? 0 : 1, p.scale, p.base);
    }

    float st[kStats];
#pragma unroll
    for (int k = 0; k < kStats; ++k) st[k] = 0.0f;
    float iters_f = 0.0f;
    const int i = row0 + tid;
    if (tid < kLanes && i < n) {
        const float eps_t = fmaxf(p.act.eps_end, p.act.eps_start - p.act.eps_decay * (float)t);
        float ap = lds.out[tid * 2];
        if (p.gauss) {
            ap = rpo_head_dev::gauss_head_row(ap, lds.out[tid * 2 + 1], draw, p.scale, p.base, p.act.box_lo, p.act.box_hi, 0, nullptr);
        }
        int k;
        typename ENV::ActArgs act = p.act;
        if (philox_noise) {
            ap = rpo_explore_clip(ap, eps_t, draw, p.act.box_lo, p.act.box_hi);
            act.noise_mode = RPO_NOISE_NONE;
        }
        float2 a;
        if (RPO_ROLLOUT_SKIP & 2) { a = make_float2(ap, 0.5f * ap); k = 0; }
        else a = ENV::project(act, c, lds.in_s + tid * kInS, i, ap, eps_t, t, k);
        iters_f = (float)k;
        reinterpret_cast<float2*>(p.act.action)[i] = a;
        const long long ring_base = p.step.rows ? (t % p.step.cap_steps) * (long long)n : 0;
        if (!(RPO_ROLLOUT_SKIP & 4)) ENV::lane(p.step, c, i, lds.in_s + tid * kInS, a, ep, ring_base, st);
    }
    if (RPO_ROLLOUT_SKIP & 16) return;
    if (p.step.stats && tid < 64) {
        float* srow = rpo_stats_row(p.step.stats, p.step.stats_cap, t);
        const int slot[kStats + 1] = {RPO_STAT_REWARD_SUM, RPO_STAT_EPISODES, RPO_STAT_RETURN_SUM, RPO_STAT_LENGTH_SUM,
                                      RPO_STAT_MAX_INEQ_SUM, RPO_STAT_MAX_EQ_SUM, RPO_STAT_VIOL_COUNT, RPO_STAT_TERMINATED,
                                      RPO_STAT_MAX_INEQ_MAX, RPO_STAT_MAX_EQ_MAX, RPO_STAT_PROJ_ITERS};
        float red[kStats + 1];
#pragma unroll
        for (int k = 0; k < kStats; ++k) red[k] = st[k];
        red[kStats] = iters_f;
        if (kLanes <= 16) rpo_row16_reduce_many(red, 3u << 8);
        else rpo_wave_reduce_many<kStats + 1, 32>(red, 3u << 8);
        rpo_stats_commit(red, 3u << 8, slot, srow);
    }
    if (!p.defer_clock) rpo_step_epilogue(p.step.ctrl, t, p.step.stats, p.step.stats_cap);
}

template <class ENV>
int launch_rollout(const RolloutArgs<ENV>& args, const typename ENV::Consts& c, int n_envs, void* stream) {
    {
        const int sel = rpo_tune(RPO_TUNE_ROLLOUT_WIDE);
        if (sel == 3 || sel == 4 || (sel == 2 && n_envs >= RPO_ROLLOUT_STREAM_FROM)) {
            const int e = rpo_rollout_stream_launch(std::is_same<ENV, CartEnv>::value ? 0 : 1, &args, &c, n_envs, stream);
            if (e >= 0) return e;
        }
    }
    const int wide_sel = rpo_tune(RPO_TUNE_ROLLOUT_WIDE);
    const int E = args.actor.E;
    const bool wide = E == 128 && (wide_sel == 0 || wide_sel == 1 ? wide_sel != 0 : n_envs >= 64 * 192);
    if (E == 128 && wide) {
        hipLaunchKernelGGL((rollout_kernel<ENV, 128, 256, 4>), dim3((n_envs + 63) / 64), dim3(kFwdThreads), 0,
                           (hipStream_t)stream, args, c);
    } else if (E == 128) {
        hipLaunchKernelGGL((rollout_kernel<ENV, 128, 256, 1>), dim3((n_envs + 15) / 16), dim3(kFwdThreads), 0,
                           (hipStream_t)stream, args, c);
    } else if (E == 256) {
        hipLaunchKernelGGL((rollout_kernel<ENV, 256, 256, 1>), dim3((n_envs + 15) / 16), dim3(kFwdThreads), 0,
                           (hipStream_t)stream, args, c);
    } else {
        return RPO_ERR_ARG;
    }
    RPO_LAUNCH_CHECK();
    return 0;
}

int check_actor(const Mlp& actor, int obs_dim, int gauss) {
    if (actor.hd > 1 || actor.S != obs_dim || actor.A != 0 || actor.n_out != (gauss ? 2 : 1) || actor.cat || actor.H != 256 || !actor.Ws ||
        !actor.W0 || !actor.W1 || (gauss && !actor.W1b))
        return RPO_ERR_ARG;
    return 0;
}

struct CriticFwdArgs {
    Mlp actor_target, critic_target, critic;
    float scale, base;
    const float* rows;
    long long cap_steps;
    int n_envs;
    int batch;
    float* batch_out;
    long long* idx_out;
    const long long* idx_in;
    uint64_t seed;
    uint32_t salt;
    const long long* ctrl;
    int max_steps; float corr_lr, corr_eps, corr_momentum, box_lo, box_hi;
    float* q_out;
    float* qn_out;
    float* x0_save; float* h1_save;
};

template <int EIN, int H>
__global__ __launch_bounds__(kFwdThreads) void cart_ddpg_critic_forward_kernel(CriticFwdArgs p, CartConsts c) {
    __shared__ TileLds<EIN> lds;
    __shared__ __attribute__((aligned(16))) float4 tile[kRows * 6];
    const int row0 = blockIdx.x * kRows;
    const int tid = threadIdx.x;
    const int B = p.batch;
    const long long t = p.ctrl[RPO_CTRL_T];
    if (tid < kRows * 6) {
        const int r = tid / 6, ch = tid - r * 6;
        float4 v = make_float4(0.0f, 0.0f, 0.0f, 0.0f);
        if (row0 + r < B) {
            long long row;
            if (p.idx_in) {
                row = p.idx_in[row0 + r];
            } else {
                const unsigned long long n_valid = (unsigned long long)((t < p.cap_steps ? t : p.cap_steps) * (long long)p.n_envs);
                const rpo_u4 u = rpo_philox(p.seed, (uint32_t)(row0 + r), (uint32_t)t + p.salt, RPO_STREAM_SAMPLE,
                                            (uint32_t)p.ctrl[RPO_CTRL_UPDATES]);
                row = (long long)__umul64hi(((unsigned long long)u.x << 32) | u.y, n_valid);
            }
            v = reinterpret_cast<const float4*>(p.rows)[row * (RPO_CART_RING / 4) + ch];
            if (blockIdx.y == 0) {
                reinterpret_cast<float4*>(p.batch_out)[(size_t)(row0 + r) * 6 + ch] = v;
                if (p.idx_out && ch == 0) p.idx_out[row0 + r] = row;
            }
        }
        tile[tid] = v;
    }
    __syncthreads();
    const float* tf = reinterpret_cast<const float*>(tile);
    if (blockIdx.y == 0) {
        if (tid < kRows * 6) {
            const int r = tid / 6, i = tid - r * 6;
            lds.in_s[r * kInS + i] = tf[r * 24 + 8 + i];
        }
        mlp_tile_forward<EIN, H>(p.actor_target, lds, row0, B, nullptr, nullptr, 1, p.scale, p.base);
        if (tid < kRows) {
            ActArgs a{};
            a.noise_mode = RPO_NOISE_NONE;
            a.max_steps = p.max_steps; a.corr_lr = p.corr_lr; a.corr_eps = p.corr_eps; a.corr_momentum = p.corr_momentum;
            a.box_lo = p.box_lo; a.box_hi = p.box_hi;
            int k;
            const float2 act = cart_explore_project(a, c, row0 + tid, lds.out[tid * 2], 0.0f, t, k);
            lds.in_a[tid * kInA] = act.x;
            lds.in_a[tid * kInA + 1] = act.y;
        }
        mlp_tile_forward<EIN, H>(p.critic_target, lds, row0, B, nullptr, nullptr, 0, 1.0f, 0.0f);
        if (tid < kRows && row0 + tid < B) p.qn_out[row0 + tid] = lds.out[tid * 2];
    } else {
        if (tid < kRows * 6) {
            const int r = tid / 6, i = tid - r * 6;
            lds.in_s[r * kInS + i] = tf[r * 24 + i];
        }
        if (tid < kRows * 2) {
            const int r = tid >> 1, i = tid & 1;
            lds.in_a[r * kInA + i] = tf[r * 24 + 6 + i];
        }
        mlp_tile_forward<EIN, H>(p.critic, lds, row0, B, p.x0_save, p.h1_save, 0, 1.0f, 0.0f);
        if (tid < kRows && row0 + tid < B) p.q_out[row0 + tid] = lds.out[tid * 2];
    }
}

struct CartRow { static constexpr int ROW = 24, CH = 6, RCH = RPO_CART_RING / 4, S = 6, A_OFF = 6, NS_OFF = 8; };
struct PendRow { static constexpr int ROW = 16, CH = 4, RCH = RPO_PEND_RING / 4, S = 5, A_OFF = 5, NS_OFF = 7; };

struct SacCriticFwdArgs {
    Mlp actor, critic_target1, critic_target2, critic1, critic2;
    float scale, base;
    const float* rows;
    long long cap_steps;
    int n_envs;
    int batch;
    float* batch_out;
    long long* idx_out;
    const long long* idx_in;
    const float* eps_in;
    uint64_t seed, sample_seed;
    uint32_t salt, noise_salt, noise_id_base;
    const long long* ctrl;
    int max_steps; float corr_lr, corr_eps, corr_momentum, box_lo, box_hi;
    float* q1_out; float* q2_out;
    float* qn1_out; float* qn2_out;
    float* x0_save1; float* h1_save1; float* x0_save2; float* h1_save2;
    float* ap_out; float* logp_out;
    const float* next_actions; const float* logp_in;
};

template <class L>
__device__ __forceinline__ void sac_sample(const SacCriticFwdArgs& p, float4* tile, int row0, long long t) {
    const int tid = threadIdx.x, B = p.batch;
    if (tid < kRows * L::CH) {
        const int r = tid / L::CH, ch = tid - r * L::CH;
        float4 v = make_float4(0.0f, 0.0f, 0.0f, 0.0f);
        if (row0 + r < B) {
            long long row;
            if (p.idx_in) {
// ... 357 lines not shown
};

template <class ENV, int EIN, int H>
__global__ __launch_bounds__(kFwdThreads) void sac_actor_forward_kernel(SacActorFwdArgs p, typename ENV::Consts c) {
    __shared__ TileLds<EIN> lds;
    const int row0 = blockIdx.x * kRows, tid = threadIdx.x, B = p.B, role = blockIdx.y;
    const long long t = p.ctrl[RPO_CTRL_T];
    if (tid < kRows * ENV::S) {
        const int r = tid / ENV::S, i = tid - r * ENV::S;
        lds.in_s[r * kInS + i] = row0 + r < B ? p.batch[(size_t)(row0 + r) * ENV::ROW + i] : 0.0f;
    }
    mlp_tile_forward<EIN, H>(p.actor, lds, row0, B, role == 0 ? p.ax0 : nullptr, role == 0 ? p.ah1 : nullptr, 0, 1.0f, 0.0f);
    float vals[7] = {0, 0, 0, 0, 0, 0, 0};
    const float inv_b = 1.0f / (float)B;
    const bool live = tid < kRows && row0 + tid < B;
    if (tid < kRows) {
        float2 act = make_float2(0.0f, 0.0f);
        if (live) {
            const int i = row0 + tid;
            const float rm = lds.out[tid * 2], rl = lds.out[tid * 2 + 1];
            float e;
            if (p.noise_in) {
                e = p.noise_in[i];
            } else {
                const rpo_u4 u = rpo_philox(p.seed, p.noise_id_base + (uint32_t)i, (uint32_t)t + p.noise_salt, RPO_STREAM_POLICY,
                                            (uint32_t)p.ctrl[RPO_CTRL_UPDATES]);
                e = rpo_normal(u.x, u.y);
            }
            float logp = 0.0f;
            const float ap = rpo_head_dev::gauss_head_row(rm, rl, e, p.scale, p.base, p.box_lo, p.box_hi, 0, &logp);
            act = ENV::complete(c, lds.in_s + tid * kInS, i, ap, t);
            if (role == 0) {
                reinterpret_cast<float2*>(p.raw)[i] = make_float2(rm, rl);
                p.noise_out[i] = e;
                p.logp[i] = logp;
                reinterpret_cast<float2*>(p.actions)[i] = act;
                float dist[6];
                float2 g;
                vals[0] = ENV::lagr(c, act.x, act.y, p.nu, inv_b, dist, g);
#pragma unroll
                for (int j = 0; j < 6; ++j) vals[1 + j] = dist[j];
                reinterpret_cast<float2*>(p.g_act)[i] = g;
            }
        }
        lds.in_a[tid * kInA] = act.x;
        lds.in_a[tid * kInA + 1] = act.y;
    }
    if (role == 0) mlp_tile_forward<EIN, H>(p.critic1, lds, row0, B, p.c1x0, p.c1h1, 0, 1.0f, 0.0f);
    else mlp_tile_forward<EIN, H>(p.critic2, lds, row0, B, p.c2x0, p.c2h1, 0, 1.0f, 0.0f);
    if (live) (role == 0 ? p.dq1 : p.dq2)[row0 + tid] = lds.out[tid * 2];
    if (role == 0 && tid < 64) {
        rpo_wave_reduce_many(vals, 0u);
#pragma unroll
        for (int k = 0; k < 7; ++k)
            if (tid == 0) p.partial[blockIdx.x * 8 + k] = vals[k];
    }
}

struct SacActorBwdArgs {
    BwdArgs critic1, critic2, actor;
    const float* g_act; const float* raw; const float* noise;
    float dlogp, box_lo, box_hi, scale, base;
    float* dout;
    float* partial; int n_parts;
    const float* logp;
    float* q_dq1; float* q_dq2;
    float* lag_out;
    float* nu_grad; int n_ineq;
    int shared_embedding;
};

template <class ENV, int EIN, int H>
__global__ __launch_bounds__(kThreads) void sac_actor_backward_kernel(SacActorBwdArgs p, typename ENV::Consts c) {
    const int row0 = blockIdx.x * kRows, tid = threadIdx.x, B = p.actor.n;
    if (tid < 64) {
        float v = 0.0f;
        if (tid < kRows && row0 + tid < B) {
            const int i = row0 + tid;
            const float q1 = p.q_dq1[i], q2 = p.q_dq2[i];
            const float w1 = (q1 < q2 ? 1.0f : 0.0f) + (q1 == q2 ? 0.5f : 0.0f);
            const float inv_b = 1.0f / (float)B;
            p.q_dq1[i] = w1 * -inv_b;
            p.q_dq2[i] = (1.0f - w1) * -inv_b;
            v = p.dlogp * (float)B * p.logp[i] - fminf(q1, q2);
        }
        const float sum = rpo_wave_sum(v);
        if (tid == 0) p.partial[blockIdx.x * 8 + 7] = sum;
    }
    __syncthreads();
    mlp_bwd_rows_body<EIN, H>(p.critic1);
    __syncthreads();
    mlp_bwd_rows_body<EIN, H>(p.critic2);
    __syncthreads();
    if (tid < kRows && row0 + tid < B) {
        const int i = row0 + tid;
        const float2 d1 = reinterpret_cast<const float2*>(p.critic1.da)[i], d2 = reinterpret_cast<const float2*>(p.critic2.da)[i];
        const float2 g = reinterpret_cast<const float2*>(p.g_act)[i];
        const float da0 = (d1.x + d2.x) + g.x, da1 = (d1.y + d2.y) + g.y;
        const float dap = ENV::complete_bwd(c, p.actor.s + (size_t)i * p.actor.s_stride, da0, da1);
        const float2 r = reinterpret_cast<const float2*>(p.raw)[i];
        reinterpret_cast<float2*>(p.dout)[i] = rpo_head_dev::gauss_head_bwd_row(r.x, r.y, p.noise[i], dap, p.dlogp, p.scale,
                                                                                p.base, p.box_lo, p.box_hi);
    }
    __syncthreads();
    mlp_bwd_rows_body<EIN, H>(p.actor);
    if (p.shared_embedding) {
        __syncthreads();
        for (int idx = tid; idx < kRows * EIN; idx += kThreads) {
            const int r = idx / EIN, e = idx - r * EIN;
            if (row0 + r < B) {
                const size_t o = (size_t)(row0 + r) * EIN + e;
                p.actor.dx0[o] += p.critic1.dx0[o] + p.critic2.dx0[o];
            }
        }
    }
    if (blockIdx.x == 0 && tid < 7) {
        float sacc = 0.0f;
        for (int g = 0; g < p.n_parts; ++g) sacc += p.partial[g * 8 + tid];
        const float inv_b = 1.0f / (float)B;
        if (tid == 0) p.lag_out[0] = inv_b * sacc;
        else if (tid - 1 < p.n_ineq) p.nu_grad[tid - 1] += inv_b * sacc;
    }
}

}

extern "C" {

int rpo_cartsafe_rollout(const rpo_mlp* actor_host, int gauss, float scale, float base, int n_envs, float* state,
                         float* action, int* ep_len, float* ep_ret, unsigned* ep_count, float* rows, long long cap_steps,
                         float* stats, int stats_cap, long long* ctrl, int noise_mode, float eps_start, float eps_end,
                         float eps_decay, float box_lo, float box_hi, int max_steps, float corr_lr, float corr_eps,
                         float corr_momentum, const float* consts_host, int partial, int max_episode_steps,
                         int auto_reset, float viol_thresh, unsigned long long seed, unsigned env_id_base, int defer_clock,
                         void* stream) {
    if (!actor_host) return RPO_ERR_NULL;
    if (n_envs <= 0 || max_episode_steps <= 0 || max_steps < 0) return RPO_ERR_ARG;
    if (noise_mode != RPO_NOISE_NONE && noise_mode != RPO_NOISE_PHILOX && noise_mode != RPO_NOISE_CLIP_ONLY) return RPO_ERR_ARG;
    if (!state || !action || !ep_len || !ep_ret || !ep_count || !ctrl) return RPO_ERR_NULL;
    if ((rows && cap_steps <= 0) || (stats && stats_cap <= 0)) return RPO_ERR_ARG;
    RolloutArgs<CartEnv> args{};
    args.actor = to_dev(actor_host);
    if (int e = check_actor(args.actor, 6, gauss)) return e;
    CartConsts c;
    if (int e = load_consts(c, consts_host, partial)) return e;
    args.scale = scale; args.base = base; args.gauss = gauss; args.defer_clock = defer_clock ? 1 : 0;
    args.act = rpo_cart_dev::ActArgs{n_envs, nullptr, nullptr, action, nullptr, noise_mode, eps_start, eps_end, eps_decay,
                                     box_lo, box_hi, max_steps, corr_lr, corr_eps, corr_momentum, (uint64_t)seed,
                                     (uint32_t)env_id_base, ctrl, stats, stats_cap};
    args.step = rpo_cart_dev::StepArgs{n_envs, state, action, ep_len, ep_ret, ep_count, rows, cap_steps, stats, stats_cap,
                                       ctrl, max_episode_steps, auto_reset, viol_thresh, (uint64_t)seed,
                                       (uint32_t)env_id_base, 0};
    return launch_rollout<CartEnv>(args, c, n_envs, stream);
}

int rpo_pendulum_rollout(const rpo_mlp* actor_host, int gauss, float scale, float base, int n_envs, float* internal,
                         float* obs, float* action, int* ep_len, float* ep_ret, unsigned* ep_count, float* rows,
                         long long cap_steps, float* stats, int stats_cap, long long* ctrl, int noise_mode,
                         float eps_start, float eps_end, float eps_decay, float box_lo, float box_hi, int max_steps,
                         float corr_lr, float corr_eps, float corr_momentum, int max_episode_steps, int auto_reset,
                         float viol_thresh, unsigned long long seed, unsigned env_id_base, int defer_clock, void* stream) {
    if (!actor_host) return RPO_ERR_NULL;
    if (n_envs <= 0 || max_episode_steps <= 0 || max_steps < 0) return RPO_ERR_ARG;
    if (noise_mode != RPO_NOISE_NONE && noise_mode != RPO_NOISE_PHILOX && noise_mode != RPO_NOISE_CLIP_ONLY) return RPO_ERR_ARG;
    if (!internal || !action || !ep_len || !ep_ret || !ep_count || !ctrl) return RPO_ERR_NULL;
    if ((rows && cap_steps <= 0) || (stats && stats_cap <= 0)) return RPO_ERR_ARG;
    RolloutArgs<PendEnv> args{};
    args.actor = to_dev(actor_host);
    if (int e = check_actor(args.actor, 5, gauss)) return e;
    args.scale = scale; args.base = base; args.gauss = gauss; args.defer_clock = defer_clock ? 1 : 0;
    args.act = rpo_pend_dev::ActArgs{n_envs, nullptr, 5, nullptr, nullptr, action, nullptr, noise_mode, eps_start, eps_end,
                                     eps_decay, box_lo, box_hi, max_steps, corr_lr, corr_eps, corr_momentum, (uint64_t)seed,
                                     (uint32_t)env_id_base, ctrl, stats, stats_cap};
    args.step = rpo_pend_dev::StepArgs{n_envs, internal, obs, action, ep_len, ep_ret, ep_count, rows, cap_steps, stats,
                                       stats_cap, ctrl, max_episode_steps, auto_reset, viol_thresh, (uint64_t)seed,
                                       (uint32_t)env_id_base};
    return launch_rollout<PendEnv>(args, PendEnv::Consts{0}, n_envs, stream);
}

int rpo_cartsafe_ddpg_critic_forward(const rpo_mlp* actor_target_host, const rpo_mlp* critic_target_host,
                                     const rpo_mlp* critic_host, float scale, float base, const float* rows,
                                     long long cap_steps, int n_envs, int batch, float* batch_out, long long* idx_out,
                                     const long long* idx_in, unsigned long long seed, unsigned sample_salt,
                                     const long long* ctrl, int max_steps, float corr_lr, float corr_eps,
                                     float corr_momentum, float box_lo, float box_hi, const float* consts_host,
                                     int partial, float* q_out, float* qn_out, float* x0_save, float* h1_save,
                                     void* stream) {
    if (!actor_target_host || !critic_target_host || !critic_host) return RPO_ERR_NULL;
    if (batch <= 0 || cap_steps <= 0 || n_envs <= 0 || max_steps < 0) return RPO_ERR_ARG;
    if (!rows || !batch_out || !ctrl || !q_out || !qn_out || !x0_save || !h1_save) return RPO_ERR_NULL;
    CriticFwdArgs a{};
    a.actor_target = to_dev(actor_target_host); a.critic_target = to_dev(critic_target_host); a.critic = to_dev(critic_host);
    const Mlp& at = a.actor_target;
    const Mlp& ct = a.critic_target;
    const Mlp& cr = a.critic;
    if (at.S != 6 || at.A != 0 || at.n_out != 1 || at.cat || ct.S != 6 || ct.A != 2 || ct.cat || cr.S != 6 || cr.A != 2 || cr.cat ||
        at.H != 256 || ct.H != 256 || cr.H != 256 || at.E != ct.E || at.E != cr.E || ct.n_out != 1 || cr.n_out != 1)
        return RPO_ERR_ARG;
    CartConsts c;
    if (int e = load_consts(c, consts_host, partial)) return e;
    a.scale = scale; a.base = base; a.rows = rows; a.cap_steps = cap_steps; a.n_envs = n_envs; a.batch = batch;
    a.batch_out = batch_out; a.idx_out = idx_out; a.idx_in = idx_in; a.seed = (uint64_t)seed; a.salt = (uint32_t)sample_salt;
    a.ctrl = ctrl; a.max_steps = max_steps; a.corr_lr = corr_lr; a.corr_eps = corr_eps; a.corr_momentum = corr_momentum;
    a.box_lo = box_lo; a.box_hi = box_hi; a.q_out = q_out; a.qn_out = qn_out; a.x0_save = x0_save; a.h1_save = h1_save;
    const int grid = (batch + kRows - 1) / kRows;
    if (at.E == 128) {
        hipLaunchKernelGGL((cart_ddpg_critic_forward_kernel<128, 256>), dim3(grid, 2), dim3(kFwdThreads), 0, (hipStream_t)stream, a, c);
    } else if (at.E == 256) {
        hipLaunchKernelGGL((cart_ddpg_critic_forward_kernel<256, 256>), dim3(grid, 2), dim3(kFwdThreads), 0, (hipStream_t)stream, a, c);
    } else {
        return RPO_ERR_ARG;
    }
    RPO_LAUNCH_CHECK();
    return 0;
}

int rpo_cartsafe_sac_critic_forward(const rpo_mlp* actor_host, const rpo_mlp* critic_target1_host,
                                    const rpo_mlp* critic_target2_host, const rpo_mlp* critic1_host,
                                    const rpo_mlp* critic2_host, float scale, float base, const float* rows,
                                    long long cap_steps, int n_envs, int batch, float* batch_out, long long* idx_out,
                                    const long long* idx_in, const float* eps_in, unsigned long long sample_seed,
                                    unsigned sample_salt, unsigned long long noise_seed, unsigned noise_id_base,
                                    unsigned noise_salt, const long long* ctrl, int max_steps, float corr_lr,
                                    float corr_eps, float corr_momentum, float box_lo, float box_hi,
                                    const float* consts_host, int partial, float* q1_out, float* q2_out,
                                    float* qn1_out, float* qn2_out, float* logp_out, float* x0_save1, float* h1_save1,
                                    float* x0_save2, float* h1_save2, void* stream) {
    if (!actor_host || !critic_target1_host || !critic_target2_host || !critic1_host || !critic2_host) return RPO_ERR_NULL;
    if (batch <= 0 || cap_steps <= 0 || n_envs <= 0 || max_steps < 0) return RPO_ERR_ARG;
    if (!rows || !batch_out || !ctrl || !q1_out || !q2_out || !qn1_out || !qn2_out || !logp_out || !x0_save1 || !h1_save1 ||
        !x0_save2 || !h1_save2)
        return RPO_ERR_NULL;
    SacCriticFwdArgs a{};
    a.actor = to_dev(actor_host);
    a.critic_target1 = to_dev(critic_target1_host); a.critic_target2 = to_dev(critic_target2_host);
    a.critic1 = to_dev(critic1_host); a.critic2 = to_dev(critic2_host);
    if (int e = check_actor(a.actor, 6, 1)) return e;
    const Mlp* qs[4] = {&a.critic_target1, &a.critic_target2, &a.critic1, &a.critic2};
    for (const Mlp* q : qs)
        if (q->S != 6 || q->A != 2 || q->cat || q->H != 256 || q->E != a.actor.E || q->n_out != 1 || q->hd > 1) return RPO_ERR_ARG;
    CartConsts c;
    if (int e = load_consts(c, consts_host, partial)) return e;
    a.scale = scale; a.base = base; a.rows = rows; a.cap_steps = cap_steps; a.n_envs = n_envs; a.batch = batch;
    a.batch_out = batch_out; a.idx_out = idx_out; a.idx_in = idx_in; a.eps_in = eps_in; a.seed = (uint64_t)noise_seed;
    a.sample_seed = (uint64_t)sample_seed; a.salt = (uint32_t)sample_salt; a.noise_salt = (uint32_t)noise_salt;
    a.noise_id_base = (uint32_t)noise_id_base; a.ctrl = ctrl; a.max_steps = max_steps; a.corr_lr = corr_lr;
    a.corr_eps = corr_eps; a.corr_momentum = corr_momentum; a.box_lo = box_lo; a.box_hi = box_hi;
    a.q1_out = q1_out; a.q2_out = q2_out; a.qn1_out = qn1_out; a.qn2_out = qn2_out; a.logp_out = logp_out;
    a.x0_save1 = x0_save1; a.h1_save1 = h1_save1; a.x0_save2 = x0_save2; a.h1_save2 = h1_save2;
    const int grid = (batch + kRows - 1) / kRows;
    if (a.actor.E == 128) {
        hipLaunchKernelGGL((cart_sac_critic_forward_kernel<128, 256>), dim3(grid, 4), dim3(kFwdThreads), 0, (hipStream_t)stream, a, c);
    } else if (a.actor.E == 256) {
        hipLaunchKernelGGL((cart_sac_critic_forward_kernel<256, 256>), dim3(grid, 4), dim3(kFwdThreads), 0, (hipStream_t)stream, a, c);
    } else {
        return RPO_ERR_ARG;
    }
    RPO_LAUNCH_CHECK();
    return 0;
}

static int fill_sac_args(SacCriticFwdArgs& a, int obs_dim, const rpo_mlp* actor_host, const rpo_mlp* ct1, const rpo_mlp* ct2,
                         const rpo_mlp* c1, const rpo_mlp* c2, bool need_actor, bool need_critics) {
    if (need_actor) {
        if (!actor_host) return RPO_ERR_NULL;
        a.actor = to_dev(actor_host);
        if (int e = check_actor(a.actor, obs_dim, 1)) return e;
    }
    if (need_critics) {
        if (!ct1 || !ct2 || !c1 || !c2) return RPO_ERR_NULL;
        a.critic_target1 = to_dev(ct1); a.critic_target2 = to_dev(ct2); a.critic1 = to_dev(c1); a.critic2 = to_dev(c2);
        const Mlp* qs[4] = {&a.critic_target1, &a.critic_target2, &a.critic1, &a.critic2};
        for (const Mlp* q : qs)
            if (q->S != obs_dim || q->A != 2 || q->cat || q->H != 256 || (q->E != 128 && q->E != 256) || q->E != qs[0]->E ||
                q->n_out != 1 || q->hd > 1)
                return RPO_ERR_ARG;
    }
    return 0;
}

int rpo_pendulum_sac_critic_front(const rpo_mlp* actor_host, float scale, float base, float box_lo, float box_hi,
                                  const float* rows, long long cap_steps, int n_envs, int batch, float* batch_out,
                                  long long* idx_out, const long long* idx_in, const float* eps_in,
                                  unsigned long long sample_seed, unsigned sample_salt, unsigned long long noise_seed,
                                  unsigned noise_id_base, unsigned noise_salt, const long long* ctrl, float* ap_out,
                                  float* logp_out, void* stream) {
    if (batch <= 0 || cap_steps <= 0 || n_envs <= 0) return RPO_ERR_ARG;
    if (!rows || !batch_out || !ctrl || !ap_out || !logp_out) return RPO_ERR_NULL;
    SacCriticFwdArgs a{};
    if (int e = fill_sac_args(a, 5, actor_host, nullptr, nullptr, nullptr, nullptr, true, false)) return e;
    a.scale = scale; a.base = base; a.box_lo = box_lo; a.box_hi = box_hi; a.rows = rows; a.cap_steps = cap_steps;
    a.n_envs = n_envs; a.batch = batch; a.batch_out = batch_out; a.idx_out = idx_out; a.idx_in = idx_in; a.eps_in = eps_in;
    a.sample_seed = (uint64_t)sample_seed; a.salt = (uint32_t)sample_salt; a.seed = (uint64_t)noise_seed;
    a.noise_id_base = (uint32_t)noise_id_base; a.noise_salt = (uint32_t)noise_salt; a.ctrl = ctrl; a.ap_out = ap_out;
    a.logp_out = logp_out;
    const int grid = (batch + kRows - 1) / kRows;
    if (a.actor.E == 128) {
        hipLaunchKernelGGL((pend_sac_critic_front_kernel<128, 256>), dim3(grid), dim3(kFwdThreads), 0, (hipStream_t)stream, a);
    } else if (a.actor.E == 256) {
        hipLaunchKernelGGL((pend_sac_critic_front_kernel<256, 256>), dim3(grid), dim3(kFwdThreads), 0, (hipStream_t)stream, a);
    } else {
        return RPO_ERR_ARG;
    }
    RPO_LAUNCH_CHECK();
    return 0;
}
// ... 277 lines not shown
```

### rpo_amd/csrc/train_ops.hip

```cpp
#include <stdlib.h>
#include "common.h"
#include "heads_dev.h"

namespace {

__global__ __launch_bounds__(RPO_BLOCK) void td_huber_kernel(
    int n, const float* __restrict__ q1, const float* __restrict__ q2, const float* __restrict__ qn1,
    const float* __restrict__ qn2, const float* __restrict__ logp, float alpha, const float* __restrict__ reward,
    int reward_stride, const float* __restrict__ done, int done_stride, float gamma, float* __restrict__ loss_out,
    float* __restrict__ grad_q1, float* __restrict__ grad_q2, float* __restrict__ target_out) {
    __shared__ float red[RPO_BLOCK / RPO_WAVE];
    const float inv_n = 1.0f / (float)n;
    float acc = 0.0f;
    for (int i = blockIdx.x * RPO_BLOCK + threadIdx.x; i < n; i += gridDim.x * RPO_BLOCK) {
        const float qn = rpo_head_dev::td_next_value(qn1[i], qn2 ? qn2[i] : 0.0f, qn2 != nullptr,
                                                     logp ? logp[i] : 0.0f, logp != nullptr, alpha);
        const float y = rpo_head_dev::td_target(reward[(size_t)i * reward_stride], done[(size_t)i * done_stride], gamma,
                                                qn);
        if (target_out) target_out[i] = y;
        float h1 = 0.0f, h2 = 0.0f;
        const float g1 = rpo_head_dev::td_huber_row(q1[i], y, inv_n, &h1);
        if (grad_q1) grad_q1[i] = g1;
        if (q2) {
            const float g2 = rpo_head_dev::td_huber_row(q2[i], y, inv_n, &h2);
            if (grad_q2) grad_q2[i] = g2;
        }
        acc += h1 + h2;
    }
    const float r = rpo_wave_sum(acc);
    if ((threadIdx.x & (RPO_WAVE - 1)) == 0) red[threadIdx.x / RPO_WAVE] = r;
    __syncthreads();
    if (threadIdx.x == 0 && loss_out) {
        float s = 0.0f;
        for (int w = 0; w < RPO_BLOCK / RPO_WAVE; ++w) s += red[w];
        atomicAdd(loss_out, s);
    }
}

__global__ __launch_bounds__(RPO_BLOCK) void absmax_kernel(long long n, const float* __restrict__ x,
                                                           float* __restrict__ max_out, int slotted) {
    __shared__ float red[RPO_BLOCK / RPO_WAVE];
    float m = 0.0f;
    const long long n4 = n / 4;
    const float4* x4 = reinterpret_cast<const float4*>(x);
    for (long long i = (long long)blockIdx.x * RPO_BLOCK + threadIdx.x; i < n4; i += (long long)gridDim.x * RPO_BLOCK) {
        const float4 v = x4[i];
        m = fmaxf(fmaxf(m, fabsf(v.x)), fmaxf(fabsf(v.y), fmaxf(fabsf(v.z), fabsf(v.w))));
    }
    for (long long i = n4 * 4 + (long long)blockIdx.x * RPO_BLOCK + threadIdx.x; i < n; i += (long long)gridDim.x * RPO_BLOCK)
        m = fmaxf(m, fabsf(x[i]));
    m = rpo_wave_max(m);
    if ((threadIdx.x & (RPO_WAVE - 1)) == 0) red[threadIdx.x / RPO_WAVE] = m;
    __syncthreads();
    if (threadIdx.x == 0) {
        for (int w = 1; w < RPO_BLOCK / RPO_WAVE; ++w) m = fmaxf(m, red[w]);
        m = fmaxf(m, red[0]);
        float* dst = slotted ? max_out + (blockIdx.x % RPO_GRADMAX_SLOTS) * (RPO_GRADMAX_LEN / RPO_GRADMAX_SLOTS) : max_out;
        if (m > 0.0f) rpo_atomic_max_nonneg(dst, m);
    }
}

struct AdamArgs {
    long long n;
    float* param;
    float* grad;
    float* m;
    float* v;
    int* step_dev;
    float lr, beta1, beta2, eps, weight_decay;
    int maximize;
    float clip_thres;
    float* gradmax;
    int reset_gradmax;
    int zero_grad;
    int clamp_min0;
    float* target;
    float tau;
    long long* arrive;
    float* target2;
    long long n2;
    int polyak_only;
    long long* clock;
    int prepared;
};

__device__ __forceinline__ void adam_body(const AdamArgs& p) {
    if (p.polyak_only) {
        for (long long i = (long long)blockIdx.x * RPO_BLOCK + threadIdx.x; i < p.n; i += (long long)gridDim.x * RPO_BLOCK)
            p.target[i] = p.target[i] * (1.0f - p.tau) + p.param[i] * p.tau;
        return;
    }
    const long long i0 = (long long)blockIdx.x * RPO_BLOCK + threadIdx.x, stride = (long long)gridDim.x * RPO_BLOCK;
    float g0 = 0.0f, w0 = 0.0f, m0 = 0.0f, v0 = 0.0f, t0 = 0.0f, t20 = 0.0f;
    if (i0 < p.n) {
        g0 = p.grad[i0]; w0 = p.param[i0]; m0 = p.m[i0]; v0 = p.v[i0];
        if (p.target) t0 = p.target[i0];
        if (p.target2 && i0 < p.n2) t20 = p.target2[i0];
    }
    asm volatile("" ::: "memory");
    float gm = 0.0f;
    if (p.clip_thres > 0.0f) {
#pragma unroll
        for (int j = 0; j < RPO_GRADMAX_SLOTS; ++j) gm = fmaxf(gm, p.gradmax[j * (RPO_GRADMAX_LEN / RPO_GRADMAX_SLOTS)]);
    }
    const int step = p.prepared ? p.step_dev[0] : p.step_dev[0] + 1;
    double* cache = reinterpret_cast<double*>(p.step_dev + 4);
    double bc1 = cache[0], bc2s = cache[1];
    if (bc1 == 0.0 || p.step_dev[1] != step) {
        bc1 = 1.0 - pow((double)p.beta1, (double)step);
        bc2s = sqrt(1.0 - pow((double)p.beta2, (double)step));
    }
    const float step_size = (float)((double)p.lr / bc1);
    const float bc2_sqrt = (float)bc2s;
    const float coef = p.clip_thres > 0.0f ? fminf(p.clip_thres / (gm + 1e-6f), 1.0f) : 1.0f;
    const float omb1 = 1.0f - p.beta1, omb2 = 1.0f - p.beta2;
    for (long long i = i0; i < p.n; i += stride) {
        if (i != i0) {
            g0 = p.grad[i]; w0 = p.param[i]; m0 = p.m[i]; v0 = p.v[i];
            if (p.target) t0 = p.target[i];
            if (p.target2 && i < p.n2) t20 = p.target2[i];
        }
        float g = g0 * coef;
        if (p.zero_grad) p.grad[i] = 0.0f;
        else if (p.clip_thres > 0.0f) p.grad[i] = g;
        if (p.maximize) g = -g;
        float w = w0;
        if (p.weight_decay != 0.0f) g += p.weight_decay * w;
        float m = m0, v = v0;
        m = m + (g - m) * omb1;
        v = v * p.beta2 + omb2 * g * g;
        const float denom = sqrtf(v) / bc2_sqrt + p.eps;
        w = w - step_size * (m / denom);
        if (p.clamp_min0) w = fmaxf(w, 0.0f);
        p.param[i] = w; p.m[i] = m; p.v[i] = v;
        if (p.target) p.target[i] = t0 * (1.0f - p.tau) + w * p.tau;
        if (p.target2 && i < p.n2) p.target2[i] = t20 * (1.0f - p.tau) + w * p.tau;
    }
    if (p.prepared) return;
    __syncthreads();
    if (threadIdx.x == 0) {
        const unsigned n = gridDim.x, sub = blockIdx.x % 16u;
        unsigned long long* top = reinterpret_cast<unsigned long long*>(p.arrive);
        bool last;
        if (n <= 16u) {
            last = atomicAdd(top, 1ull) == (unsigned long long)n - 1ull;
        } else {
            unsigned long long* sc = reinterpret_cast<unsigned long long*>(p.step_dev + 32 + 32 * sub);
            const unsigned long long in_sub = (n - sub + 15u) / 16u;
            last = false;
            if (atomicAdd(sc, 1ull) == in_sub - 1ull) {
                *sc = 0;
                last = atomicAdd(top, 1ull) == 15ull;
            }
        }
        if (last) {
            *top = 0;
            p.step_dev[0] = step;
            cache[0] = 1.0 - pow((double)p.beta1, (double)(step + 1));
            cache[1] = sqrt(1.0 - pow((double)p.beta2, (double)(step + 1)));
            p.step_dev[1] = step + 1;
            if (p.reset_gradmax && p.gradmax)
                for (int j = 0; j < RPO_GRADMAX_SLOTS; ++j) p.gradmax[j * (RPO_GRADMAX_LEN / RPO_GRADMAX_SLOTS)] = 0.0f;
            if (p.clock) p.clock[0] += 1;
        }
    }
}

__global__ __launch_bounds__(RPO_BLOCK) void adam_kernel(AdamArgs p) { adam_body(p); }

struct AdamArgs4 {
    AdamArgs seg[4];
};
__global__ __launch_bounds__(RPO_BLOCK) void adam_multi_kernel(AdamArgs4 p) { adam_body(p.seg[blockIdx.y]); }

__global__ __launch_bounds__(RPO_BLOCK) void min_q_bwd_kernel(int n, const float* __restrict__ q1, const float* __restrict__ q2,
                                                              float scale, float* __restrict__ dq1, float* __restrict__ dq2) {
    for (int i = blockIdx.x * RPO_BLOCK + threadIdx.x; i < n; i += gridDim.x * RPO_BLOCK) {
        const float a = q1[i], b = q2[i];
        const float w = (a < b ? 1.0f : 0.0f) + 0.5f * (a == b ? 1.0f : 0.0f);
        dq1[i] = w * scale;
        dq2[i] = (1.0f - w) * scale;
    }
}

__global__ __launch_bounds__(RPO_BLOCK) void polyak_kernel(long long n, const float* __restrict__ param,
                                                           float* __restrict__ target, float tau) {
    for (long long i = (long long)blockIdx.x * RPO_BLOCK + threadIdx.x; i < n; i += (long long)gridDim.x * RPO_BLOCK)
        target[i] = target[i] * (1.0f - tau) + param[i] * tau;
}

__global__ __launch_bounds__(RPO_BLOCK) void philox_fill_kernel(int n, uint32_t* __restrict__ out, uint64_t seed,
                                                                uint32_t id_base, uint32_t index, uint32_t tag) {
    for (int i = blockIdx.x * RPO_BLOCK + threadIdx.x; i < n; i += gridDim.x * RPO_BLOCK) {
        const rpo_u4 r = rpo_philox(seed, id_base + (uint32_t)i, index, tag);
        reinterpret_cast<uint4*>(out)[i] = make_uint4(r.x, r.y, r.z, r.w);
    }
}

__global__ __launch_bounds__(RPO_BLOCK) void philox_normal_kernel(int n, float* __restrict__ out, uint64_t seed,
                                                                  uint32_t id_base, uint32_t salt, uint32_t tag,
                                                                  const long long* __restrict__ ctrl) {
    const uint32_t t = ctrl ? (uint32_t)ctrl[RPO_CTRL_T] : 0u;
    const uint32_t sub = ctrl ? (uint32_t)ctrl[RPO_CTRL_UPDATES] : 0u;
    for (int i = blockIdx.x * RPO_BLOCK + threadIdx.x; i < n; i += gridDim.x * RPO_BLOCK) {
        const rpo_u4 r = rpo_philox(seed, id_base + (uint32_t)i, t + salt, tag, sub);
        out[i] = rpo_normal(r.x, r.y);
    }
}

}

int g_rpo_tune[RPO_TUNE_COUNT] = { 1,  16,  1,  1,
                                   1,  2,  1,
                                   1,  0};

extern "C" {

int rpo_philox_normal(int n, float* out, unsigned long long seed, unsigned id_base, unsigned salt,
                      unsigned stream_tag, const long long* ctrl, void* stream) {
    if (n <= 0) return RPO_ERR_ARG;
    if (!out) return RPO_ERR_NULL;
    hipLaunchKernelGGL(philox_normal_kernel, dim3(rpo_grid_for(n)), dim3(RPO_BLOCK), 0, (hipStream_t)stream, n, out,
                       (uint64_t)seed, (uint32_t)id_base, (uint32_t)salt, (uint32_t)stream_tag, ctrl);
    RPO_LAUNCH_CHECK();
    return 0;
}

int rpo_abi_version(void) { return RPO_ABI_VERSION; }

int rpo_tuning(int key, int value) {
    if (key < 0 || key >= RPO_TUNE_COUNT) return RPO_ERR_ARG;
    const int old = g_rpo_tune[key];
    if (value >= 0) g_rpo_tune[key] = value;
    return old;
}

int rpo_philox_fill(int n, unsigned* out, unsigned long long seed, unsigned id_base, unsigned index,
                    unsigned stream_tag, void* stream) {
    if (n <= 0) return RPO_ERR_ARG;
    if (!out) return RPO_ERR_NULL;
    hipLaunchKernelGGL(philox_fill_kernel, dim3(rpo_grid_for(n)), dim3(RPO_BLOCK), 0, (hipStream_t)stream, n, out,
                       (uint64_t)seed, (uint32_t)id_base, (uint32_t)index, (uint32_t)stream_tag);
    RPO_LAUNCH_CHECK();
    return 0;
}

int rpo_td_huber(int n, const float* q1, const float* q2, const float* qn1, const float* qn2, const float* logp,
                 float alpha, const float* reward, int reward_stride, const float* done, int done_stride, float gamma,
                 float* loss_out, float* grad_q1, float* grad_q2, float* target_out, void* stream) {
    if (n <= 0 || reward_stride <= 0 || done_stride <= 0) return RPO_ERR_ARG;
    if (!q1 || !qn1 || !reward || !done) return RPO_ERR_NULL;
    hipLaunchKernelGGL(td_huber_kernel, dim3(rpo_grid_for(n)), dim3(RPO_BLOCK), 0, (hipStream_t)stream, n, q1, q2, qn1,
                       qn2, logp, alpha, reward, reward_stride, done, done_stride, gamma, loss_out, grad_q1, grad_q2,
                       target_out);
    RPO_LAUNCH_CHECK();
    return 0;
}

int rpo_absmax(long long n, const float* x, float* max_out, void* stream) {
    if (n <= 0) return RPO_ERR_ARG;
    if (!x || !max_out) return RPO_ERR_NULL;
    if ((reinterpret_cast<uintptr_t>(x) & 15u) != 0) return RPO_ERR_ARG;
    hipLaunchKernelGGL(absmax_kernel, dim3(rpo_grid_for(n / 4 + 1)), dim3(RPO_BLOCK), 0, (hipStream_t)stream, n, x,
                       max_out, 0);
    RPO_LAUNCH_CHECK();
    return 0;
}

int rpo_absmax_slots(long long n, const float* x, float* gradmax, void* stream) {
    if (n <= 0) return RPO_ERR_ARG;
    if (!x || !gradmax) return RPO_ERR_NULL;
    if ((reinterpret_cast<uintptr_t>(x) & 15u) != 0) return RPO_ERR_ARG;
    hipLaunchKernelGGL(absmax_kernel, dim3(rpo_grid_for(n / 4 + 1)), dim3(RPO_BLOCK), 0, (hipStream_t)stream, n, x,
                       gradmax, 1);
    RPO_LAUNCH_CHECK();
    return 0;
}

int rpo_adam_step(long long n, float* param, float* grad, float* exp_avg, float* exp_avg_sq, int* step_dev,
                  float lr, float beta1, float beta2, float eps, float weight_decay, int maximize, float clip_thres,
                  float* gradmax, int reset_gradmax, int zero_grad, int clamp_min0, float* target, float tau,
                  long long* clock, int prepared, void* stream) {
    if (n <= 0) return RPO_ERR_ARG;
    if (!param || !grad || !exp_avg || !exp_avg_sq || !step_dev) return RPO_ERR_NULL;
    if (clip_thres > 0.0f && !gradmax) return RPO_ERR_NULL;
    AdamArgs a{n, param, grad, exp_avg, exp_avg_sq, step_dev, lr, beta1, beta2, eps, weight_decay, maximize,
               clip_thres, gradmax, reset_gradmax, zero_grad, clamp_min0, target, tau,
               reinterpret_cast<long long*>(step_dev + 2), nullptr, 0, 0, clock, prepared ? 1 : 0};
    hipLaunchKernelGGL(adam_kernel, dim3(rpo_grid_for(n)), dim3(RPO_BLOCK), 0, (hipStream_t)stream, a);
// ... 49 lines not shown
```

### rpo_amd/ops.py

```python
import ctypes
import os

import numpy as np
import torch

from . import _lib
from ._lib import CONST, RpoHipError, check

NOISE_NONE = CONST["RPO_NOISE_NONE"]
NOISE_EXPLICIT = CONST["RPO_NOISE_EXPLICIT"]
NOISE_PHILOX = CONST["RPO_NOISE_PHILOX"]
NOISE_UNIFORM = CONST["RPO_NOISE_UNIFORM"]
NOISE_CLIP_ONLY = CONST["RPO_NOISE_CLIP_ONLY"]
STREAM_POLICY = CONST["RPO_STREAM_POLICY"]
ADAM_CLOCK = True
STATS_LEN = CONST["RPO_STATS_LEN"]
STATS_SUB = CONST["RPO_STATS_SUB"]
CTRL_LEN = CONST["RPO_CTRL_LEN"]
PROJ_WS_WORDS = CONST["RPO_PROJ_WS_WORDS"]
PROJ_WS_GAVE_UP = CONST["RPO_PROJ_WS_GAVE_UP"]
STAT = {k[len("RPO_STAT_"):].lower(): v for k, v in CONST.items()
        if k.startswith("RPO_STAT_") and k not in ("RPO_STATS_LEN", "RPO_STATS_SUB")}


TUNE = {k[len("RPO_TUNE_"):].lower(): v for k, v in CONST.items() if k.startswith("RPO_TUNE_") and k != "RPO_TUNE_COUNT"}


class tuning(object):

    def __init__(self, **values):
        lib = _lib.load()
        self._old = {}
        for name, value in values.items():
            if name not in TUNE:
                raise RpoHipError("unknown tuning key %r (have: %s)" % (name, ", ".join(sorted(TUNE))))
            old = lib.rpo_tuning(TUNE[name], int(value))
            if old < 0:
                raise RpoHipError("rpo_tuning(%s) failed" % name)
            self._old[name] = old

    @staticmethod
    def get(name):
        return _lib.load().rpo_tuning(TUNE[name], -1)

    def __enter__(self):
        return self

    def __exit__(self, *exc):
        lib = _lib.load()
        for name, old in self._old.items():
            lib.rpo_tuning(TUNE[name], old)
        return False


def new_stats(stats_cap, device):
    return torch.zeros(int(stats_cap), STATS_SUB, STATS_LEN, device=device)


def reduce_stats(rows):
    out = rows.sum(dim=-2)
    for key in ("max_ineq_max", "max_eq_max"):
        out[..., STAT[key]] = rows[..., STAT[key]].max(dim=-1).values
    return out


def _stream():
    return ctypes.c_void_p(torch.cuda.current_stream().cuda_stream)


def _p(t, dtype=torch.float32, allow_none=False, contiguous=True):
    if t is None:
        if allow_none:
            return None
        raise RpoHipError("required tensor is None")
    if not t.is_cuda:
        raise RpoHipError("rpo_amd kernels need GPU tensors (got %s); there is no CPU fallback" % t.device)
    if t.dtype != dtype:
        raise RpoHipError("expected %s, got %s" % (dtype, t.dtype))
    if contiguous and not t.is_contiguous():
        raise RpoHipError("expected a contiguous tensor, got strides %s" % (t.stride(),))
    return ctypes.c_void_p(t.data_ptr())


def _row_view(t, width):
    if t.dim() != 2 or t.shape[1] != width or t.stride(1) != 1:
        raise RpoHipError("expected a [n,%d] row view with unit column stride, got %s / %s" % (width, tuple(t.shape), t.stride()))
    return _p(t, contiguous=False), int(t.stride(0)) if t.shape[0] > 1 else width


def _col_view(t):
    if t.dim() == 2:
        if t.shape[1] != 1:
            raise RpoHipError("expected [n,1], got %s" % (tuple(t.shape),))
        return _p(t, contiguous=False), int(t.stride(0))
    return _p(t, contiguous=False), int(t.stride(0))


def _ring(rows, ring_floats, allow_none=True):
    if rows is None:
        return _p(rows, allow_none=allow_none)
    if rows.dim() != 2 or rows.shape[-1] != ring_floats:
        raise RpoHipError("replay ring must be [rows, %d] float32 (the kernels' compiled ring stride), got %s"
                          % (ring_floats, tuple(rows.shape)))
    return _p(rows)


def _host_ptr(arr):
    return arr.ctypes.data_as(ctypes.c_void_p)



def philox_fill(out, seed, id_base, index, stream_tag):
    check(_lib.load().rpo_philox_fill(out.shape[0], _p(out, torch.int32), seed, id_base, index, stream_tag, _stream()),
          "rpo_philox_fill")


def philox_normal(out, seed, id_base, salt, stream_tag, ctrl=None):
    check(_lib.load().rpo_philox_normal(out.numel(), _p(out), seed, id_base, salt, stream_tag,
                                        _p(ctrl, torch.int64, allow_none=True), _stream()), "rpo_philox_normal")


def replay_gather(rows, idx, out):
    check(_lib.load().rpo_replay_gather(_p(rows), rows.shape[-1], out.shape[-1], idx.shape[0], _p(idx, torch.int64), _p(out),
                                        _stream()), "rpo_replay_gather")


def replay_sample_gather(rows, cap_steps, n_envs, out, idx_out, seed, salt, ctrl):
    check(_lib.load().rpo_replay_sample_gather(_p(rows), rows.shape[-1], out.shape[-1], cap_steps, n_envs, out.shape[0], _p(out),
                                               _p(idx_out, torch.int64, allow_none=True), seed, salt,
                                               _p(ctrl, torch.int64), _stream()), "rpo_replay_sample_gather")


def td_huber(q1, q2, qn1, qn2, logp, alpha, reward, done, gamma, loss_out, grad_q1, grad_q2, target_out=None):
    n = q1.shape[0]
    rp, rs = _col_view(reward)
    dp, ds = _col_view(done)
    check(_lib.load().rpo_td_huber(n, _p(q1), _p(q2, allow_none=True), _p(qn1), _p(qn2, allow_none=True),
                                   _p(logp, allow_none=True), alpha, rp, rs, dp, ds, gamma, _p(loss_out),
                                   _p(grad_q1, allow_none=True), _p(grad_q2, allow_none=True),
                                   _p(target_out, allow_none=True), _stream()), "rpo_td_huber")


def absmax(x, max_out):
    if max_out.numel() >= CONST["RPO_GRADMAX_LEN"]:
        check(_lib.load().rpo_absmax_slots(x.numel(), _p(x), _p(max_out), _stream()), "rpo_absmax_slots")
    else:
        check(_lib.load().rpo_absmax(x.numel(), _p(x), _p(max_out), _stream()), "rpo_absmax")


def adam_step(param, grad, exp_avg, exp_avg_sq, step_dev, lr, beta1=0.9, beta2=0.999, eps=1e-8, weight_decay=0.0,
              maximize=False, clip_thres=0.0, gradmax=None, reset_gradmax=True, clamp_min0=False, target=None,
              tau=0.0, zero_grad=False, clock=None, prepared=False):
    if step_dev.numel() < CONST["RPO_ADAM_STATE_LEN"]:
        raise RpoHipError("step_dev must be int32[RPO_ADAM_STATE_LEN]: {step, pad, arrival word, cached bias corrections, "
                          "sub-counters} (include/rpo_hip.h)")
    check(_lib.load().rpo_adam_step(param.numel(), _p(param), _p(grad), _p(exp_avg), _p(exp_avg_sq),
                                    _p(step_dev, torch.int32), lr, beta1, beta2, eps, weight_decay, int(maximize),
                                    clip_thres, _p(gradmax, allow_none=True), int(reset_gradmax), int(zero_grad), int(clamp_min0),
                                    _p(target, allow_none=True), tau, _p(clock, torch.int64, allow_none=True), int(prepared),
                                    _stream()),
          "rpo_adam_step")


class _AdamSegStruct(ctypes.Structure):
    _fields_ = [("n", ctypes.c_longlong), ("param", ctypes.c_void_p), ("grad", ctypes.c_void_p), ("exp_avg", ctypes.c_void_p),
                ("exp_avg_sq", ctypes.c_void_p), ("step_dev", ctypes.c_void_p), ("lr", ctypes.c_float),
                ("beta1", ctypes.c_float), ("beta2", ctypes.c_float), ("eps", ctypes.c_float),
                ("weight_decay", ctypes.c_float), ("maximize", ctypes.c_int), ("clip_thres", ctypes.c_float),
                ("gradmax", ctypes.c_void_p), ("reset_gradmax", ctypes.c_int), ("zero_grad", ctypes.c_int),
                ("clamp_min0", ctypes.c_int), ("target", ctypes.c_void_p), ("tau", ctypes.c_float),
                ("target2", ctypes.c_void_p), ("n2", ctypes.c_longlong), ("polyak_only", ctypes.c_int),
                ("prepared", ctypes.c_int)]


def adam_step_multi(segs, clock=None, prepared=False):
    arr = (_AdamSegStruct * len(segs))()
    vp = lambda t, dt=torch.float32: None if t is None else _p(t, dt).value
    for a, g in zip(arr, segs):
        a.n, a.param, a.tau = g["param"].numel(), vp(g["param"]), g.get("tau", 0.0)
        a.target, a.target2, a.n2 = vp(g.get("target")), vp(g.get("target2")), int(g.get("n2", 0))
        a.polyak_only = int(bool(g.get("polyak_only", False)))
        if a.polyak_only:
            continue
        a.grad, a.exp_avg, a.exp_avg_sq = vp(g["grad"]), vp(g["exp_avg"]), vp(g["exp_avg_sq"])
        if g["step_dev"].numel() < CONST["RPO_ADAM_STATE_LEN"]:
            raise RpoHipError("step_dev must be int32[RPO_ADAM_STATE_LEN] (include/rpo_hip.h)")
        a.step_dev = vp(g["step_dev"], torch.int32)
        a.lr, a.beta1, a.beta2, a.eps = g["lr"], g.get("beta1", 0.9), g.get("beta2", 0.999), g.get("eps", 1e-8)
        a.weight_decay, a.maximize, a.clip_thres = g.get("weight_decay", 0.0), int(g.get("maximize", False)), g.get("clip_thres", 0.0)
        a.gradmax, a.reset_gradmax = vp(g.get("gradmax")), int(g.get("reset_gradmax", True))
        a.zero_grad, a.clamp_min0 = int(g.get("zero_grad", False)), int(g.get("clamp_min0", False))
        a.prepared = int(bool(prepared))
    check(_lib.load().rpo_adam_step_multi(len(segs), arr, _p(clock, torch.int64, allow_none=True), _stream()),
          "rpo_adam_step_multi")


def min_q_bwd(q1, q2, scale, dq1, dq2):
    check(_lib.load().rpo_min_q_bwd(q1.numel(), _p(q1), _p(q2), scale, _p(dq1), _p(dq2), _stream()), "rpo_min_q_bwd")


def polyak(param, target, tau):
    check(_lib.load().rpo_polyak(param.numel(), _p(param), _p(target), tau, _stream()), "rpo_polyak")


EVAL_LEN = CONST["RPO_EVAL_LEN"]
EVAL_LANE_STEPS = CONST["RPO_EVAL_LANE_STEPS"]


def _eval_acc(acc, n):
    if acc.dim() != 2 or acc.shape[0] != n or acc.shape[1] != EVAL_LEN:
        raise RpoHipError("evaluation accumulators must be [%d, %d] float32, got %s" % (n, EVAL_LEN, tuple(acc.shape)))
    return _p(acc)


def eval_accumulate(rows, cols, iters, step, viol_thresh, acc):
    n = acc.shape[0]
    rp, stride = _row_view(rows[:n], rows.shape[1])
    (r0, _), (d0, _) = cols["reward"], cols["done"]
    (e0, e1), (i0, i1) = cols["eq_viol"], cols["ineq_viol"]
    check(_lib.load().rpo_eval_accumulate(n, rp, stride, r0, d0, e0, e1 - e0, i0, i1 - i0,
                                          _p(iters, torch.int32, allow_none=True), int(step), viol_thresh, _eval_acc(acc, n),
                                          _stream()), "rpo_eval_accumulate")


TRACE_ALIGN = CONST["RPO_TRACE_ALIGN"]
TRACE_TAIL = CONST["RPO_TRACE_TAIL"]
TRACE_MAX_BYTES = CONST["RPO_TRACE_MAX_BYTES"]
TRACE_SLOT = {k: CONST["RPO_TRACE_" + k.upper()] for k in ("reward", "done", "ineq", "eq")}


def trace_layout(obs_dim, partial_dim, action_dim):
    head = (obs_dim + partial_dim + action_dim + 1 + TRACE_ALIGN - 1) // TRACE_ALIGN * TRACE_ALIGN
    return head, head + TRACE_TAIL


def _trace(trace, n, width):
    if trace.dim() != 3 or trace.shape[2] != width or not 1 <= trace.shape[1] <= n:
        raise RpoHipError("trace buffer must be [steps, 1..%d, %d] float32, got %s" % (n, width, tuple(trace.shape)))
    return _p(trace), int(trace.shape[1]), int(trace.shape[0])


def eval_record(rows, cols, obs, proposal, action, iters, step, acc, trace):
    n = acc.shape[0]
    rp, stride = _row_view(rows[:n], rows.shape[1])
    op, ostride = _row_view(obs, obs.shape[1])
    (r0, _), (d0, _) = cols["reward"], cols["done"]
    (e0, e1), (i0, i1) = cols["eq_viol"], cols["ineq_viol"]
    O, A = obs.shape[1], action.shape[1]
    P = proposal.numel() // n
    if obs.shape[0] != n or action.shape[0] != n or proposal.numel() != n * P or P < 1:
        raise RpoHipError("eval_record: obs / proposal / action do not have %d rows" % n)
    tp, R, T = _trace(trace, n, trace_layout(O, P, A)[1])
    check(_lib.load().rpo_eval_record(n, rp, stride, r0, d0, e0, e1 - e0, i0, i1 - i0, op, ostride, O, _p(proposal), P,
                                      _p(action), A, _p(iters, torch.int32, allow_none=True), int(step), _eval_acc(acc, n),
                                      tp, R, T, _stream()), "rpo_eval_record")


CON_ALIGN = CONST["RPO_CON_ALIGN"]


def con_width(ineq_num, eq_num):
    return (2 * ineq_num + eq_num + CON_ALIGN - 1) // CON_ALIGN * CON_ALIGN


def _con(con, n, width):
    if con.dim() != 2 or tuple(con.shape) != (n, width):
        raise RpoHipError("constraint report must be [%d, %d] float32, got %s" % (n, width, tuple(con.shape)))
    return _p(con)


def eval_constraints(rows, cols, step, viol_thresh, acc, con):
    n = acc.shape[0]
    rp, stride = _row_view(rows[:n], rows.shape[1])
    (e0, e1), (i0, i1) = cols["eq_viol"], cols["ineq_viol"]
    check(_lib.load().rpo_eval_constraints(n, rp, stride, e0, e1 - e0, i0, i1 - i0, int(step), viol_thresh, _eval_acc(acc, n),
                                           _con(con, n, con_width(i1 - i0, e1 - e0)), _stream()), "rpo_eval_constraints")


STREAM_EVAL_OBS = CONST["RPO_STREAM_EVAL_OBS"]


def eval_obs_noise(obs, sigma, seed, step, out):
    n, O = obs.shape
    op, ostride = _row_view(obs, O)
    dp, dstride = _row_view(out, O)
    if out.shape[0] != n or sigma.numel() != O:
        raise RpoHipError("eval_obs_noise: out must have %d rows and sigma %d entries" % (n, O))
    check(_lib.load().rpo_eval_obs_noise(n, op, ostride, O, _p(sigma), int(seed), int(step), dp, dstride, _stream()),
          "rpo_eval_obs_noise")


def _eval_noise(noise, obs_dim):
    sigma, seed = noise
    sigma = np.ascontiguousarray(sigma, dtype=np.float32)
    if sigma.shape != (obs_dim,):
        raise RpoHipError("evaluate: noise sigma must be float32 [%d], got %s" % (obs_dim, sigma.shape))
    return sigma, (_host_ptr(sigma), obs_dim, int(seed))


def _eval_lanes(lane_steps, lane_lr, n):
    if tuple(lane_steps.shape) != (n,) or tuple(lane_lr.shape) != (n,):
        raise RpoHipError("evaluate_budgets: lane_steps / lane_lr must be [%d], got %s / %s"
                          % (n, tuple(lane_steps.shape), tuple(lane_lr.shape)))
    return _p(lane_steps, torch.int32), _p(lane_lr)


POLICY_GROUP_ALIGN = 64


def _eval_policies(actor_desc, bank, n, group_lanes, episodes):
    if bank.dim() != 2 or not bank.is_contiguous() or bank.dtype != torch.float32:
        raise RpoHipError("evaluate_policies: the bank must be a contiguous float32 [P, stride] tensor, got %s %s"
                          % (bank.dtype, tuple(bank.shape)))
    P, stride = int(bank.shape[0]), int(bank.shape[1])
    lo = _p(bank).value
    for key, t in actor_desc.tensors.items():
        if t is not None and not (lo <= t.data_ptr() and t.data_ptr() + 4 * t.numel() <= lo + 4 * stride and t.is_contiguous()):
            raise RpoHipError("evaluate_policies: tensor %s of the descriptor does not lie inside policy 0 of the bank" % key)
    if group_lanes <= 0 or n != P * group_lanes:
        raise RpoHipError("evaluate_policies: %d lanes are not %d policies x %d lanes" % (n, P, group_lanes))
    return stride, int(group_lanes), int(episodes)


def _eval_noise_sweep(sigma_table, seed, n, group_lanes, episodes):
    if sigma_table.dim() != 2 or sigma_table.shape[1] != 8 or not sigma_table.is_contiguous() or sigma_table.dtype != torch.float32:
        raise RpoHipError("evaluate_noise_sweep: the sigma table must be a contiguous float32 [S, 8] tensor, got %s %s"
                          % (sigma_table.dtype, tuple(sigma_table.shape)))
    S = int(sigma_table.shape[0])
    if group_lanes <= 0 or n != S * group_lanes:
        raise RpoHipError("evaluate_noise_sweep: %d lanes are not %d noise levels x %d lanes" % (n, S, group_lanes))
    return _p(sigma_table), int(seed), int(group_lanes), int(episodes)


CURVE_LEN = CONST["RPO_CURVE_LEN"]
CURVE_WS = CONST["RPO_CURVE_WS"]


def eval_summarize(acc, ctrl, row_out, ws):
    n = acc.shape[0]
    if row_out.numel() != CURVE_LEN or ws.numel() < CURVE_WS:
        raise RpoHipError("curve row must be float64[%d] and the workspace float64[>= %d]" % (CURVE_LEN, CURVE_WS))
    check(_lib.load().rpo_eval_summarize(n, _eval_acc(acc, n), _p(ctrl, torch.int64), _p(row_out, torch.float64),
                                         _p(ws, torch.float64), _stream()), "rpo_eval_summarize")


def eval_keep_best(src, best, row, best_row, best_point, point, max_violation_rate):
    n = src.numel()
    if src.dim() != 1 or best.dim() != 1 or best.numel() != n or n < 1:
        raise RpoHipError("src and best must be float32 vectors of one length >= 1, got %s and %s"
                          % (tuple(src.shape), tuple(best.shape)))
    if row.numel() != CURVE_LEN or best_row.numel() != CURVE_LEN or best_point.numel() != 1:
        raise RpoHipError("row and best_row must be float64[%d] and best_point int64[1]" % CURVE_LEN)
    check(_lib.load().rpo_eval_keep_best(n, _p(src), _p(best), _p(row, torch.float64), _p(best_row, torch.float64),
                                         _p(best_point, torch.int64), int(point), float(max_violation_rate), _stream()),
          "rpo_eval_keep_best")


def _act_outputs(kernels, n, action, proposal, iters, eq_resid, ineq_resid):
    want = (("action", action, (n, kernels.action_dim)), ("proposal", proposal, (n, kernels.partial_dim)), ("iters", iters, (n,)),
            ("eq_resid", eq_resid, (n, kernels.eq_num)), ("ineq_resid", ineq_resid, (n, kernels.ineq_num)))
    for name, t, shape in want:
        if t is not None and tuple(t.shape) != shape:
            raise RpoHipError("policy_act: %s must be %s, got %s" % (name, shape, tuple(t.shape)))
    if action is None or n < 1:
        raise RpoHipError("policy_act: needs n >= 1 rows and an action buffer")


def _act_profile(profile, n, steps):
    if profile is None or tuple(profile.shape) != (int(steps) + 1, n, 4):
        raise RpoHipError("profile must be [%d, %d, 4], got %s" % (int(steps) + 1, n, None if profile is None else tuple(profile.shape)))
    return _p(profile)



class CartSafeKernels(object):

    name = "CartSafe-v0"
    obs_dim, internal_dim, action_dim, eq_num, ineq_num, partial_dim = 6, 6, 2, 1, 6, 1
    row_floats = CONST["RPO_CART_ROW"]
    ring_floats = CONST["RPO_CART_RING"]
    cols = dict(state=(0, 6), action=(6, 8), next_state=(8, 14), reward=(14, 15), done=(15, 16), eq_viol=(16, 17),
                ineq_viol=(17, 23))

    def __init__(self, consts, partial):
        self.consts = np.ascontiguousarray(consts, dtype=np.float32)
        if self.consts.shape != (CONST["RPO_CART_CONSTS_LEN"],):
            raise RpoHipError("bad CartSafe constant table")
        self.partial = int(partial)

    @property
    def _cptr(self):
        return _host_ptr(self.consts)

    def reset(self, internal, obs, ep_len, ep_ret, ep_count, seed, env_id_base):
        check(_lib.load().rpo_cartsafe_reset(internal.shape[0], _p(internal), _p(ep_len, torch.int32), _p(ep_ret),
                                             _p(ep_count, torch.int32), seed, env_id_base, _stream()),
              "rpo_cartsafe_reset")

    def step(self, internal, obs, action, ep_len, ep_ret, ep_count, rows, cap_steps, stats, ctrl, max_episode_steps,
             auto_reset, viol_thresh, seed, env_id_base):
        check(_lib.load().rpo_cartsafe_step(
            internal.shape[0], _p(internal), _p(action), _p(ep_len, torch.int32), _p(ep_ret),
            _p(ep_count, torch.int32), _ring(rows, self.ring_floats), cap_steps, _p(stats, allow_none=True),
            0 if stats is None else stats.shape[0], _p(ctrl, torch.int64, allow_none=True), self._cptr, self.partial,
            max_episode_steps, int(auto_reset), viol_thresh, seed, env_id_base, _stream()), "rpo_cartsafe_step")

    def act_project(self, obs, ap_raw, noise, action, iters, noise_mode, eps_start, eps_end, eps_decay, box_lo, box_hi,
                    max_steps, corr_lr, corr_eps, corr_momentum, seed=0, env_id_base=0, ctrl=None, stats=None):
        check(_lib.load().rpo_cartsafe_act_project(
            action.shape[0], _p(ap_raw, allow_none=True), _p(noise, allow_none=True), _p(action),
            _p(iters, torch.int32, allow_none=True), noise_mode, eps_start, eps_end, eps_decay, box_lo, box_hi,
            max_steps, corr_lr, corr_eps, corr_momentum, self._cptr, self.partial, seed, env_id_base,
            _p(ctrl, torch.int64, allow_none=True), _p(stats, allow_none=True),
            0 if stats is None else stats.shape[0], _stream()), "rpo_cartsafe_act_project")

    def rollout(self, actor_desc, gauss, scale, base, internal, obs, action, ep_len, ep_ret, ep_count, rows, cap_steps,
                stats, ctrl, noise_mode, eps_start, eps_end, eps_decay, box_lo, box_hi, max_steps, corr_lr, corr_eps,
                corr_momentum, max_episode_steps, auto_reset, viol_thresh, seed, env_id_base, defer_clock=False):
        net = actor_desc.net_struct()
        check(_lib.load().rpo_cartsafe_rollout(
            ctypes.byref(net), int(gauss), scale, base, internal.shape[0], _p(internal), _p(action),
            _p(ep_len, torch.int32), _p(ep_ret), _p(ep_count, torch.int32), _ring(rows, self.ring_floats), cap_steps,
            _p(stats, allow_none=True), 0 if stats is None else stats.shape[0], _p(ctrl, torch.int64), noise_mode,
            eps_start, eps_end, eps_decay, box_lo, box_hi, max_steps, corr_lr, corr_eps, corr_momentum, self._cptr,
            self.partial, max_episode_steps, int(auto_reset), viol_thresh, seed, env_id_base, int(defer_clock), _stream()),
            "rpo_cartsafe_rollout")

    def evaluate(self, actor_desc, gauss, scale, base, internal, obs, action, ep_len, ep_ret, ep_count, ctrl, acc, t0, steps,
                 box_lo, box_hi, max_steps, corr_lr, corr_eps, corr_momentum, max_episode_steps, viol_thresh, trace=None,
                 con=None, noise=None):
        net = actor_desc.net_struct()
        n = internal.shape[0]
        args = (ctypes.byref(net), int(gauss), scale, base, n, _p(internal), _p(action), _p(ep_len, torch.int32),
                _p(ep_ret), _p(ep_count, torch.int32), _p(ctrl, torch.int64, allow_none=True), _eval_acc(acc, n),
                int(t0), int(steps), box_lo, box_hi, max_steps, corr_lr, corr_eps, corr_momentum, self._cptr, self.partial,
                max_episode_steps, viol_thresh)
        if noise is not None:
            tr = (None, 0, 0) if trace is None else _trace(trace, n, trace_layout(self.obs_dim, self.partial_dim, self.action_dim)[1])
            sigma, tail = _eval_noise(noise, self.obs_dim)
            check(_lib.load().rpo_cartsafe_evaluate_noisy(*args, *tr, None if con is None else _con(con, n, con_width(self.ineq_num, self.eq_num)),
                                                    *tail, _stream()), "rpo_cartsafe_evaluate_noisy")
        elif con is not None:
            tr = (None, 0, 0) if trace is None else _trace(trace, n, trace_layout(self.obs_dim, self.partial_dim, self.action_dim)[1])
            check(_lib.load().rpo_cartsafe_evaluate_constraints(*args, *tr, _con(con, n, con_width(self.ineq_num, self.eq_num)),
                                                                _stream()), "rpo_cartsafe_evaluate_constraints")
        elif trace is None:
            check(_lib.load().rpo_cartsafe_evaluate(*args, _stream()), "rpo_cartsafe_evaluate")
        else:
            tr = _trace(trace, n, trace_layout(self.obs_dim, self.partial_dim, self.action_dim)[1])
            check(_lib.load().rpo_cartsafe_evaluate_record(*args, *tr, _stream()), "rpo_cartsafe_evaluate_record")

    def evaluate_budgets(self, actor_desc, gauss, scale, base, internal, obs, action, ep_len, ep_ret, ep_count, ctrl, acc, t0,
                         steps, box_lo, box_hi, lane_steps, lane_lr, corr_eps, corr_momentum, max_episode_steps, viol_thresh,
                         con=None):
        net = actor_desc.net_struct()
        n = internal.shape[0]
        sp, lp = _eval_lanes(lane_steps, lane_lr, n)
        check(_lib.load().rpo_cartsafe_evaluate_budgets(
            ctypes.byref(net), int(gauss), scale, base, n, _p(internal), _p(action), _p(ep_len, torch.int32), _p(ep_ret),
            _p(ep_count, torch.int32), _p(ctrl, torch.int64, allow_none=True), _eval_acc(acc, n), int(t0), int(steps), box_lo,
            box_hi, 0, 0.0, corr_eps, corr_momentum, self._cptr, self.partial, max_episode_steps, viol_thresh, None, 0, 0,
            None if con is None else _con(con, n, con_width(self.ineq_num, self.eq_num)), sp, lp, _stream()),
            "rpo_cartsafe_evaluate_budgets")

    def evaluate_policies(self, actor_desc, gauss, scale, base, internal, obs, action, ep_len, ep_ret, ep_count, ctrl, acc, t0,
                          steps, box_lo, box_hi, max_steps, corr_lr, corr_eps, corr_momentum, max_episode_steps, viol_thresh, bank,
                          group_lanes, episodes, con=None):
        net = actor_desc.net_struct()
        n = internal.shape[0]
        tail = _eval_policies(actor_desc, bank, n, group_lanes, episodes)
        check(_lib.load().rpo_cartsafe_evaluate_policies(
            ctypes.byref(net), int(gauss), scale, base, n, _p(internal), _p(action), _p(ep_len, torch.int32), _p(ep_ret),
            _p(ep_count, torch.int32), _p(ctrl, torch.int64, allow_none=True), _eval_acc(acc, n), int(t0), int(steps), box_lo,
            box_hi, max_steps, corr_lr, corr_eps, corr_momentum, self._cptr, self.partial, max_episode_steps, viol_thresh,
            None if con is None else _con(con, n, con_width(self.ineq_num, self.eq_num)), *tail, _stream()),
            "rpo_cartsafe_evaluate_policies")

    def evaluate_noise_sweep(self, actor_desc, gauss, scale, base, internal, obs, action, ep_len, ep_ret, ep_count, ctrl, acc, t0,
                             steps, box_lo, box_hi, max_steps, corr_lr, corr_eps, corr_momentum, max_episode_steps, viol_thresh,
                             sigma_table, seed, group_lanes, episodes, con=None):
        net = actor_desc.net_struct()
        n = internal.shape[0]
        tail = _eval_noise_sweep(sigma_table, seed, n, group_lanes, episodes)
        check(_lib.load().rpo_cartsafe_evaluate_noise_sweep(
            ctypes.byref(net), int(gauss), scale, base, n, _p(internal), _p(action), _p(ep_len, torch.int32), _p(ep_ret),
            _p(ep_count, torch.int32), _p(ctrl, torch.int64, allow_none=True), _eval_acc(acc, n), int(t0), int(steps), box_lo,
            box_hi, max_steps, corr_lr, corr_eps, corr_momentum, self._cptr, self.partial, max_episode_steps, viol_thresh,
            None if con is None else _con(con, n, con_width(self.ineq_num, self.eq_num)), *tail, _stream()),
            "rpo_cartsafe_evaluate_noise_sweep")

    def policy_act(self, actor_desc, gauss, scale, base, obs, action, proposal, iters, eq_resid, ineq_resid, box_lo, box_hi,
                   max_steps, corr_lr, corr_eps, corr_momentum, form=0):
        net = actor_desc.net_struct()
        op, ostride = _row_view(obs, self.obs_dim)
        _act_outputs(self, obs.shape[0], action, proposal, iters, eq_resid, ineq_resid)
        check(_lib.load().rpo_cartsafe_policy_act(
            ctypes.byref(net), int(gauss), scale, base, obs.shape[0], op, ostride, _p(action), _p(proposal, allow_none=True),
            _p(iters, torch.int32, allow_none=True), _p(eq_resid, allow_none=True), _p(ineq_resid, allow_none=True), box_lo,
            box_hi, int(max_steps), corr_lr, corr_eps, corr_momentum, self._cptr, self.partial, int(form), _stream()),
            "rpo_cartsafe_policy_act")

    def policy_act_profile(self, actor_desc, gauss, scale, base, obs, action, proposal, iters, eq_resid, ineq_resid, box_lo,
                           box_hi, max_steps, corr_lr, corr_eps, corr_momentum, profile):
        net = actor_desc.net_struct()
        op, ostride = _row_view(obs, self.obs_dim)
        _act_outputs(self, obs.shape[0], action, proposal, iters, eq_resid, ineq_resid)
        check(_lib.load().rpo_cartsafe_policy_act_profile(
            ctypes.byref(net), int(gauss), scale, base, obs.shape[0], op, ostride, _p(action), _p(proposal, allow_none=True),
            _p(iters, torch.int32, allow_none=True), _p(eq_resid, allow_none=True), _p(ineq_resid, allow_none=True), box_lo,
            box_hi, int(max_steps), corr_lr, corr_eps, corr_momentum, self._cptr, self.partial,
            _act_profile(profile, obs.shape[0], max_steps), _stream()), "rpo_cartsafe_policy_act_profile")

    def project_profile(self, obs, ap_raw, action, iters, max_steps, corr_lr, corr_eps, corr_momentum, profile):
        n = action.shape[0]
        check(_lib.load().rpo_cartsafe_project_profile(
            n, _p(ap_raw), _p(action), _p(iters, torch.int32, allow_none=True), int(max_steps), corr_lr, corr_eps, corr_momentum,
            self._cptr, self.partial, _act_profile(profile, n, max_steps), _stream()), "rpo_cartsafe_project_profile")

    def ddpg_critic_forward(self, actor_target, critic_target, critic, scale, base, rows, cap_steps, n_envs, batch_out,
                            idx_out, idx_in, seed, salt, ctrl, max_steps, corr_lr, corr_eps, corr_momentum, box_lo, box_hi,
                            q_out, qn_out, x0_save, h1_save):
        at, ct, cr = actor_target.net_struct(), critic_target.net_struct(), critic.net_struct()
        check(_lib.load().rpo_cartsafe_ddpg_critic_forward(
            ctypes.byref(at), ctypes.byref(ct), ctypes.byref(cr), scale, base, _ring(rows, self.ring_floats, False), cap_steps, n_envs,
            batch_out.shape[0], _p(batch_out), _p(idx_out, torch.int64, allow_none=True),
            _p(idx_in, torch.int64, allow_none=True), seed, salt, _p(ctrl, torch.int64), max_steps, corr_lr, corr_eps,
            corr_momentum, box_lo, box_hi, self._cptr, self.partial, _p(q_out), _p(qn_out), _p(x0_save), _p(h1_save),
            _stream()), "rpo_cartsafe_ddpg_critic_forward")

    def sac_critic_forward(self, actor, critic_target1, critic_target2, critic1, critic2, scale, base, rows, cap_steps,
                           n_envs, batch_out, idx_out, idx_in, eps_in, sample_seed, sample_salt, noise_seed, noise_id_base,
                           noise_salt, ctrl, max_steps, corr_lr, corr_eps, corr_momentum, box_lo, box_hi,
                           q1_out, q2_out, qn1_out, qn2_out, logp_out, x0_save1, h1_save1, x0_save2, h1_save2):
        nets = [d.net_struct() for d in (actor, critic_target1, critic_target2, critic1, critic2)]
        check(_lib.load().rpo_cartsafe_sac_critic_forward(
            *[ctypes.byref(n) for n in nets], scale, base, _ring(rows, self.ring_floats, False), cap_steps, n_envs, batch_out.shape[0], _p(batch_out),
            _p(idx_out, torch.int64, allow_none=True), _p(idx_in, torch.int64, allow_none=True),
            _p(eps_in, allow_none=True), sample_seed, sample_salt, noise_seed, noise_id_base, noise_salt,
            _p(ctrl, torch.int64), max_steps, corr_lr, corr_eps, corr_momentum, box_lo, box_hi, self._cptr, self.partial,
            _p(q1_out), _p(q2_out), _p(qn1_out), _p(qn2_out), _p(logp_out), _p(x0_save1), _p(h1_save1),
            _p(x0_save2), _p(h1_save2), _stream()), "rpo_cartsafe_sac_critic_forward")

    def complete_bwd(self, obs, grad_action, grad_ap, action=None):
        check(_lib.load().rpo_cartsafe_complete_bwd(grad_action.shape[0], _p(grad_action), _p(grad_ap), self._cptr,
                                                    self.partial, _stream()), "rpo_cartsafe_complete_bwd")

    def resid(self, obs, action, eq_out, ineq_out):
        check(_lib.load().rpo_cartsafe_resid(action.shape[0], _p(action), _p(eq_out, allow_none=True),
                                             _p(ineq_out, allow_none=True), self._cptr, self.partial, _stream()),
              "rpo_cartsafe_resid")

    def ineq_partial_grad(self, obs, action, step_out):
        check(_lib.load().rpo_cartsafe_ineq_partial_grad(action.shape[0], _p(action), _p(step_out), self._cptr,
                                                         self.partial, _stream()), "rpo_cartsafe_ineq_partial_grad")

    def lagrangian(self, action, nu, scale, loss_out, grad_action, grad_nu, obs=None):
        check(_lib.load().rpo_cartsafe_lagrangian(action.shape[0], _p(action), _p(nu), scale, _p(loss_out),
                                                  _p(grad_action, allow_none=True), _p(grad_nu, allow_none=True),
                                                  self._cptr, self.partial, _stream()), "rpo_cartsafe_lagrangian")


class EvopfKernels(object):

    name = "EVOPF-v0"
    obs_dim = internal_dim = CONST["RPO_EVOPF_STATE"]
    action_dim, partial_dim = CONST["RPO_EVOPF_ACTION"], CONST["RPO_EVOPF_PARTIAL"]
    eq_num, ineq_num = CONST["RPO_EVOPF_EQ"], CONST["RPO_EVOPF_INEQ"]
    row_floats = ring_floats = CONST["RPO_EVOPF_ROW"]
    cols = dict(state=(0, 57), action=(57, 100), next_state=(100, 157), reward=(157, 158), done=(158, 159),
                eq_viol=(159, 187), ineq_viol=(187, 245))
    newton_tol, newton_max_iters = 1e-5, 50
    episode_steps = 24
    partial = 0
    CASE14_ADJ = (19, 31, 14, 350, 59, 7216, 456, 192, 9032, 1792, 1568, 6176, 14368, 12544)

    def __init__(self, consts):
        self.consts = np.ascontiguousarray(consts, dtype=np.float32)
        if self.consts.shape != (CONST["RPO_EVOPF_CONSTS_LEN"],):
            raise RpoHipError("bad EVOPF constant table")
# ... 646 lines not shown
```

Before: 102.0 million env-steps/s.

## Fuse deferred critic Adam step into next rollout kernel launch

On non-actor update steps the critic Adam step is deferred and run as extra workgroups inside the next cartsafe rollout kernel. The rollout's actor workgroups apply the pending update to the shared trunk weights themselves, and the Adam workgroups that own the shared region spin on a sync counter until every rollout workgroup has read the old weights. This removes one kernel launch per vector step and overlaps the optimizer with the rollout. In exchange it adds an inter-workgroup spin barrier with a give-up flag, and it only applies in the serial-window schedule under narrow tuning conditions.

```diff
diff --git a/include/rpo_hip.h b/include/rpo_hip.h
--- a/include/rpo_hip.h
+++ b/include/rpo_hip.h
@@ -435,6 +435,14 @@
                          float corr_momentum, const float* consts_host, int partial, int max_episode_steps,
                          int auto_reset, float viol_thresh, unsigned long long seed, unsigned env_id_base, int defer_clock,
                          void* stream);
+int rpo_cartsafe_rollout_adam(const rpo_mlp* actor_host, int gauss, float scale, float base, int n_envs, float* state,
+                              float* action, int* ep_len, float* ep_ret, unsigned* ep_count, float* rows, long long cap_steps,
+                              float* stats, int stats_cap, long long* ctrl, int noise_mode, float eps_start, float eps_end,
+                              float eps_decay, float box_lo, float box_hi, int max_steps, float corr_lr, float corr_eps,
+                              float corr_momentum, const float* consts_host, int partial, int max_episode_steps,
+                              int auto_reset, float viol_thresh, unsigned long long seed, unsigned env_id_base, int defer_clock,
+                              const rpo_adam_seg* adam, long long shared_begin, unsigned* ride_sync, unsigned* gave_up,
+                              void* stream);
 int rpo_pendulum_rollout(const rpo_mlp* actor_host, int gauss, float scale, float base, int n_envs, float* internal,
                          float* obs, float* action, int* ep_len, float* ep_ret, unsigned* ep_count, float* rows,
                          long long cap_steps, float* stats, int stats_cap, long long* ctrl, int noise_mode,
diff --git a/rpo_amd/algo/rpo_ddpg.py b/rpo_amd/algo/rpo_ddpg.py
--- a/rpo_amd/algo/rpo_ddpg.py
+++ b/rpo_amd/algo/rpo_ddpg.py
@@ -281,8 +281,11 @@
         ag = self.agent
         fuse = actor_step and ag.flat.sizes[1] == 0
         prepared, self._critic_prepared = getattr(self, "_critic_prepared", False), False
-        ag.critic_optim.step(target=ag.critic_target_flat if fuse else None, tau=ag.tau,
-                             gradmax_ready=self._gradmax_ready, clock=self._clock(not actor_step), prepared=prepared)
+        if self._adam_ride_next and prepared and self._gradmax_ready and not actor_step:
+            self._adam_pending = ag.critic_optim.segment(tau=ag.tau, gradmax_ready=True)
+        else:
+            ag.critic_optim.step(target=ag.critic_target_flat if fuse else None, tau=ag.tau,
+                                 gradmax_ready=self._gradmax_ready, clock=self._clock(not actor_step), prepared=prepared)
         self._gradmax_ready = False
 
     def _actor_step(self, actor_out):
diff --git a/rpo_amd/algo/trainer.py b/rpo_amd/algo/trainer.py
--- a/rpo_amd/algo/trainer.py
+++ b/rpo_amd/algo/trainer.py
@@ -205,7 +205,7 @@
 
 
 SCHEDULE_DEFAULTS = dict(fused_mlp=1, fused_rollout=1, fused_critic=1, fused_actor=1, split=1, ride=1, front=1, branch=1,
-                         fused_eval=1, fused_act=1, eval_overlap=1, force_dist=0)
+                         fused_eval=1, fused_act=1, eval_overlap=1, adam_ride=1, force_dist=0)
 
 
 def parse_schedule(overrides=None):
@@ -303,6 +303,7 @@
         self._clock_pending, self._iter_actor_step, self._critic_prepared, self._gradmax_stale = False, None, False, False
         self._actor_prepared, self._actor_gradmax_stale = False, False
         self._bump_updates_now, self._updates_out, self._pol_a_done = False, None, False
+        self._adam_ride_next, self._adam_pending, self._adam_ride_sync = False, None, None
         self._bump = self.updates_per_step == 1
         if self.fused is not None and device.type == "cuda" and getattr(self.backend, "ADAM_CLOCK", False):
             self._uctrl, self._uclock_ok = torch.zeros_like(self.vec.ctrl), False
@@ -366,15 +367,25 @@
     def _rollout(self, warm, defer_clock=False):
         v = self.vec
         defer_clock = bool(defer_clock and not warm and self._rollout_pipeline and self._defer_ok)
+        pend, self._adam_pending = self._adam_pending, None
+        if pend is not None and (warm or not self._rollout_pipeline):
+            self._adam_launch(pend)
+            pend = None
         if not warm and self._rollout_pipeline:
             scale, base = self._box_affine
-            self.kernels.rollout(self.fused.descs["actor"], self._gauss_policy, scale, base, v.internal,
-                                 None if v.obs is v.internal else v.obs, v.action, v.ep_len, v.ep_ret, v.ep_count,
-                                 self.buffer.rows, self.buffer.capacity, v.stats, v.ctrl,
-                                 hip_ops.NOISE_NONE if self._gauss_policy else hip_ops.NOISE_PHILOX, self.eps_start,
-                                 self.eps, self.decay_value, self._box_lo, self._box_hi, self.max_steps, self.corr_lr,
-                                 self.corr_eps, self.corr_momentum, v.max_episode_steps, True, v.viol_thresh, self.seed,
-                                 v.env_id_base, **(dict(defer_clock=True) if defer_clock else {}))
+            launch, kw = self.kernels.rollout, {}
+            if pend is not None:
+                fl = self.agent.flat
+                launch = self.kernels.rollout_adam
+                kw = dict(adam=pend, shared_begin=fl.actor_range[0] - fl.critic_range[0], ride_sync=self._adam_ride_sync,
+                          gave_up=self._split_state()._held["tile_sync"][-32:])
+            launch(self.fused.descs["actor"], self._gauss_policy, scale, base, v.internal,
+                   None if v.obs is v.internal else v.obs, v.action, v.ep_len, v.ep_ret, v.ep_count,
+                   self.buffer.rows, self.buffer.capacity, v.stats, v.ctrl,
+                   hip_ops.NOISE_NONE if self._gauss_policy else hip_ops.NOISE_PHILOX, self.eps_start,
+                   self.eps, self.decay_value, self._box_lo, self._box_hi, self.max_steps, self.corr_lr,
+                   self.corr_eps, self.corr_momentum, v.max_episode_steps, True, v.viol_thresh, self.seed,
+                   v.env_id_base, **(dict(defer_clock=True) if defer_clock else {}), **kw)
             self._clock_pending = defer_clock
             v.steps_host += 1
             return
@@ -502,7 +513,43 @@
             fn()
             self.dist.mean_(reduce_after)
 
+    def _adam_ride_ok(self):
+        if not self.schedule["adam_ride"] or self.sac or self.dist.on or self.agent.flat.sizes[1] == 0:
+            return False
+        if self.updates_per_step != 1 or not self._bump or not self._rollout_pipeline or not hasattr(self.kernels, "rollout_adam"):
+            return False
+        if not getattr(self, "_pipelines", False):
+            return False
+        su = self._split_state()
+        if su is None or su.st.env != 0 or "tile_sync" not in su._held:
+            return False
+        if not self.kernels.rollout_adam_ok(self.fused.descs["actor"], self.vec.internal.shape[0]):
+            return False
+        if self._adam_ride_sync is None:
+            self._adam_ride_sync = torch.zeros(32, dtype=torch.int32, device=self.device)
+        return True
+
+    def _adam_launch(self, seg):
+        from .agent.flat import FusedAdam
+        FusedAdam.step_many(self.backend, [seg], prepared=True)
+
+    def _flush_adam(self):
+        pend, self._adam_pending = self._adam_pending, None
+        if pend is not None:
+            self._adam_launch(pend)
+
+    def _serial_window(self, t, L, do_train, ride=False):
+        try:
+            for i in range(L):
+                actor_step = do_train and (t + i + 1) % self.policy_fre == 0
+                self._adam_ride_next = ride and not actor_step and i + 1 < L
+                self._run_segments(self._segments(False, do_train, actor_step))
+        finally:
+            self._adam_ride_next = False
+        self._flush_adam()
+
     def _flush_tail(self):
+        self._flush_adam()
         tail, self._tail = self._tail, None
         if tail is not None:
             self._graphs.run(tail[0], tail[1])
@@ -733,7 +780,7 @@
 
     _HOST_STATE = ("_actor_pre", "_clock_pending", "_iter_actor_step", "_critic_prepared", "_gradmax_stale", "_actor_prepared",
                    "_actor_gradmax_stale", "_pol_a_done", "_gradmax_ready", "_actor_gradmax_ready", "_bump_updates_now",
-                   "_updates_out", "_last_cols", "_last_actor_out")
+                   "_updates_out", "_last_cols", "_last_actor_out", "_adam_ride_next", "_adam_pending")
 
     def _host_state(self):
         import ctypes
@@ -764,7 +811,8 @@
         su = getattr(self, "_split_cache", None)
         sync = su._held.get("tile_sync") if su else None
         ws = su._held.get("proj_ws") if su else None
-        return (sync[-32:-31] if sync is not None and getattr(self, "_front_cache", False) else None,
+        armed = getattr(self, "_front_cache", False) or self._adam_ride_sync is not None
+        return (sync[-32:-31] if sync is not None and armed else None,
                 ws[hip_ops.PROJ_WS_GAVE_UP:hip_ops.PROJ_WS_GAVE_UP + 1] if ws is not None else None)
 
     def _device_flags(self):
@@ -774,8 +822,9 @@
 
     def _raise_flags(self, vals):
         if vals.get("front"):
-            raise RuntimeError("rpo_split_*_front: a workgroup gave up waiting for its row tile (tile_sync flag set); the "
-                               "values of that launch are undefined -- rerun with RPO_SCHEDULE=front=0")
+            raise RuntimeError("rpo_split_*_front / rpo_cartsafe_rollout_adam: a workgroup gave up waiting for its row tile / "
+                               "for the rollout's workgroups (tile_sync flag set); the values of that launch are undefined -- "
+                               "rerun with RPO_SCHEDULE=front=0,adam_ride=0")
         if vals.get("proj"):
             raise RuntimeError("rpo_split_pend_head_project / rpo_split_critic_pfront: a workgroup gave up waiting for another "
                                "one's granules (workspace flag set); the values of that launch are undefined -- rerun with "
@@ -895,8 +944,8 @@
                 elif self._overlap_ok(do_train):
                     self._graphs.run(("cycle", L, True, "overlap"), lambda: self._overlapped_window(t, L))
                 else:
-                    self._graphs.run(("cycle", L, do_train), lambda: [self._run_segments(self._segments(
-                        False, do_train, do_train and (t + i + 1) % self.policy_fre == 0)) for i in range(L)])
+                    adam_ride = bool(do_train and self._adam_ride_ok())
+                    self._graphs.run(("cycle", L, do_train), lambda: self._serial_window(t, L, do_train, adam_ride))
                 self._updates += L if do_train else 0
                 self._poll_flags()
             else:
diff --git a/rpo_amd/csrc/adam_dev.h b/rpo_amd/csrc/adam_dev.h
--- /dev/null
+++ b/rpo_amd/csrc/adam_dev.h
@@ -0,0 +1,92 @@
+#pragma once
+#include "common.h"
+
+namespace rpo_adam_dev {
+
+struct AdamArgs {
+    long long n;
+    float* param;
+    float* grad;
+    float* m;
+    float* v;
+    int* step_dev;
+    float lr, beta1, beta2, eps, weight_decay;
+    int maximize;
+    float clip_thres;
+    float* gradmax;
+    int reset_gradmax;
+    int zero_grad;
+    int clamp_min0;
+    float* target;
+    float tau;
+    long long* arrive;
+    float* target2;
+    long long n2;
+    int polyak_only;
+    long long* clock;
+    int prepared;
+};
+
+struct AdamCoef {
+    int step;
+    float coef;
+    float step_size, bc2_sqrt, omb1, omb2;
+};
+
+struct AdamElem {
+    float w, m, v, g;
+};
+
+template <bool kCached = false>
+__device__ __forceinline__ AdamCoef adam_prologue(const AdamArgs& p) {
+    float gm = 0.0f;
+    if (p.clip_thres > 0.0f) {
+#pragma unroll
+        for (int j = 0; j < RPO_GRADMAX_SLOTS; ++j) gm = fmaxf(gm, p.gradmax[j * (RPO_GRADMAX_LEN / RPO_GRADMAX_SLOTS)]);
+    }
+    AdamCoef k;
+    k.step = p.prepared ? p.step_dev[0] : p.step_dev[0] + 1;
+    const double* cache = reinterpret_cast<const double*>(p.step_dev + 4);
+    double bc1 = cache[0], bc2s = cache[1];
+    if (!kCached && (bc1 == 0.0 || p.step_dev[1] != k.step)) {
+        bc1 = 1.0 - pow((double)p.beta1, (double)k.step);
+        bc2s = sqrt(1.0 - pow((double)p.beta2, (double)k.step));
+    }
+    k.step_size = (float)((double)p.lr / bc1);
+    k.bc2_sqrt = (float)bc2s;
+    k.coef = p.clip_thres > 0.0f ? fminf(p.clip_thres / (gm + 1e-6f), 1.0f) : 1.0f;
+    k.omb1 = 1.0f - p.beta1;
+    k.omb2 = 1.0f - p.beta2;
+    return k;
+}
+
+__device__ __forceinline__ AdamElem adam_element(const AdamArgs& p, const AdamCoef& k, float g0, float w0, float m0, float v0) {
+    AdamElem o;
+    float g = g0 * k.coef;
+    o.g = g;
+    if (p.maximize) g = -g;
+    float w = w0;
+    if (p.weight_decay != 0.0f) g += p.weight_decay * w;
+    float m = m0, v = v0;
+    m = m + (g - m) * k.omb1;
+    v = v * p.beta2 + k.omb2 * g * g;
+    const float denom = sqrtf(v) / k.bc2_sqrt + p.eps;
+    w = w - k.step_size * (m / denom);
+    if (p.clamp_min0) w = fmaxf(w, 0.0f);
+    o.w = w; o.m = m; o.v = v;
+    return o;
+}
+
+__device__ __forceinline__ float adam_polyak(float t, float w, float tau) {
+    return t * (1.0f - tau) + w * tau;
+}
+
+__device__ __forceinline__ void adam_store(const AdamArgs& p, long long i, const AdamElem& o, float t0, float t20) {
+    if (p.zero_grad) p.grad[i] = 0.0f;
+    else if (p.clip_thres > 0.0f) p.grad[i] = o.g;
+    p.param[i] = o.w; p.m[i] = o.m; p.v[i] = o.v;
+    if (p.target) p.target[i] = adam_polyak(t0, o.w, p.tau);
+    if (p.target2 && i < p.n2) p.target2[i] = adam_polyak(t20, o.w, p.tau);
+}
+
+}
diff --git a/rpo_amd/csrc/fused.hip b/rpo_amd/csrc/fused.hip
--- a/rpo_amd/csrc/fused.hip
+++ b/rpo_amd/csrc/fused.hip
@@ -2,6 +2,7 @@
 
 #include <type_traits>
 
+#include "adam_dev.h"
 #include "cartsafe_dev.h"
 #include "heads_dev.h"
 #include "mlp_bwd.h"
@@ -26,6 +27,78 @@
 #ifndef RPO_ROLLOUT_SKIP
 #define RPO_ROLLOUT_SKIP 0
 #endif
+
+struct AdamRide {
+    rpo_adam_dev::AdamArgs adam;
+    long long shared_lo;
+    unsigned* sync;
+    unsigned* gave_up;
+    int n_roll;
+    int n_owners;
+};
+constexpr int kRideSpinMax = 1 << 18;
+
+__device__ __forceinline__ void ride_adam_block(const AdamRide& r, int b) {
+    const rpo_adam_dev::AdamArgs& p = r.adam;
+    const long long i = (long long)b * kFwdThreads + threadIdx.x;
+    float g0 = 0.0f, w0 = 0.0f, m0 = 0.0f, v0 = 0.0f, t0 = 0.0f;
+    if (i < p.n) {
+        g0 = p.grad[i]; w0 = p.param[i]; m0 = p.m[i]; v0 = p.v[i];
+        if (p.target) t0 = p.target[i];
+    }
+    asm volatile("" ::: "memory");
+    const rpo_adam_dev::AdamCoef k = rpo_adam_dev::adam_prologue<true>(p);
+    const rpo_adam_dev::AdamElem o = rpo_adam_dev::adam_element(p, k, g0, w0, m0, v0);
+    if (((long long)b + 1) * kFwdThreads > r.shared_lo) {
+        if (threadIdx.x == 0) {
+            int polls = 0;
+            while (__hip_atomic_fetch_or(r.sync, 0u, __ATOMIC_RELAXED, __HIP_MEMORY_SCOPE_AGENT) != (unsigned)r.n_roll) {
+                if (++polls >= kRideSpinMax) { __hip_atomic_store(r.gave_up, 1u, __ATOMIC_RELAXED, __HIP_MEMORY_SCOPE_AGENT); break; }
+                __builtin_amdgcn_s_sleep(1);
+            }
+            if (__hip_atomic_fetch_add(r.sync + 1, 1u, __ATOMIC_RELAXED, __HIP_MEMORY_SCOPE_AGENT) == (unsigned)r.n_owners - 1u) {
+                __hip_atomic_store(r.sync, 0u, __ATOMIC_RELAXED, __HIP_MEMORY_SCOPE_AGENT);
+                __hip_atomic_store(r.sync + 1, 0u, __ATOMIC_RELAXED, __HIP_MEMORY_SCOPE_AGENT);
+            }
+        }
+        asm volatile("" ::: "memory");
+        __syncthreads();
+    }
+    if (i < p.n) rpo_adam_dev::adam_store(p, i, o, t0, 0.0f);
+}
+
+template <int TPW>
+struct RideOps {
+    float g[TPW][2], w[TPW][2], m[TPW][2], v[TPW][2];
+};
+template <int TPW>
+__device__ __forceinline__ void ride_request(const AdamRide& r, const Mlp& net, RideOps<TPW>& q) {
+    const int lane = threadIdx.x & 63, wave = threadIdx.x >> 6, li = lane & 15, lg = lane >> 4;
+    const rpo_adam_dev::AdamArgs& p = r.adam;
+#pragma unroll
+    for (int t = 0; t < TPW; ++t) {
+        const int e = (wave + t * kFwdWaves) * 16 + li;
+        const long long ib = (net.bs + e) - p.param;
+        const long long i0 = (lg >= 2 && lg - 2 < net.S) ? (net.Ws + e * net.S + (lg - 2)) - p.param : ib;
+        const long long i1 = 2 + lg < net.S ? (net.Ws + e * net.S + 2 + lg) - p.param : ib;
+        q.g[t][0] = p.grad[i0]; q.w[t][0] = p.param[i0]; q.m[t][0] = p.m[i0]; q.v[t][0] = p.v[i0];
+        q.g[t][1] = p.grad[i1]; q.w[t][1] = p.param[i1]; q.m[t][1] = p.m[i1]; q.v[t][1] = p.v[i1];
+    }
+}
+template <int EIN, int H, int RT>
+__device__ __forceinline__ void ride_step(const AdamRide& r, const Mlp& net, const RideOps<TileWeights<EIN, H, RT>::TPW>& q,
+                                          TileWeights<EIN, H, RT>& w) {
+    constexpr int TPW = TileWeights<EIN, H, RT>::TPW;
+    const int lg = (threadIdx.x & 63) >> 4;
+    const rpo_adam_dev::AdamCoef k = rpo_adam_dev::adam_prologue<true>(r.adam);
+#pragma unroll
+    for (int t = 0; t < TPW; ++t) {
+        const float n0 = rpo_adam_dev::adam_element(r.adam, k, q.g[t][0], q.w[t][0], q.m[t][0], q.v[t][0]).w;
+        const float n1 = rpo_adam_dev::adam_element(r.adam, k, q.g[t][1], q.w[t][1], q.m[t][1], q.v[t][1]).w;
+        if (lg == 0 || (lg >= 2 && lg - 2 < net.S)) w.wk[t][0] = n0;
+        if (2 + lg < net.S) w.wk[t][1] = n1;
+    }
+}
 
 template <class ENV, int EIN, int H, int RT>
 __global__ __launch_bounds__(kFwdThreads) void rollout_kernel(RolloutArgs<ENV> p, typename ENV::Consts c) {
@@ -96,6 +169,82 @@
         rpo_stats_commit(red, 3u << 8, slot, srow);
     }
     if (!p.defer_clock) rpo_step_epilogue(p.step.ctrl, t, p.step.stats, p.step.stats_cap);
+}
+
+template <class ENV, int EIN, int H>
+__global__ __launch_bounds__(kFwdThreads, 4) void rollout_adam_kernel(RolloutArgs<ENV> p, typename ENV::Consts c, AdamRide r) {
+    if ((int)blockIdx.x >= r.n_roll) {
+        ride_adam_block(r, (int)blockIdx.x - r.n_roll);
+        return;
+    }
+    typedef TileLds<EIN, 1, 8, 8> Lds;
+    __shared__ Lds lds;
+    constexpr int kInS = Lds::kS;
+    constexpr int kLanes = rpo_mlp_dev::kRows;
+    constexpr int kStats = 10;
+    const int row0 = blockIdx.x * kLanes;
+    const int tid = threadIdx.x;
+    const int n = p.step.n;
+    const long long t = p.step.ctrl ? p.step.ctrl[RPO_CTRL_T] : 0;
+    RpoEpisode ep{0, 0.0f, 0u};
+    if (tid < kLanes && row0 + tid < n) ep = ENV::episode(p.step, row0 + tid);
+    RideOps<TileWeights<EIN, H, 1>::TPW> rq;
+    ride_request(r, p.actor, rq);
+    asm volatile("" ::: "memory");
+    ENV::stage_obs(p.step, row0, kLanes, lds.in_s, kInS);
+    float draw = 0.0f;
+    const bool philox_noise = !p.gauss && p.act.noise_mode == RPO_NOISE_PHILOX;
+    if (tid < kLanes && row0 + tid < n && (p.gauss || philox_noise)) {
+        const rpo_u4 u = p.gauss ? rpo_philox(p.act.seed, p.act.env_id_base + (uint32_t)(row0 + tid), (uint32_t)t, RPO_STREAM_POLICY,
+                                              (uint32_t)p.step.ctrl[RPO_CTRL_UPDATES])
+                                 : rpo_philox(p.act.seed, p.act.env_id_base + (uint32_t)(row0 + tid), (uint32_t)t, RPO_STREAM_ACT);
+        draw = rpo_normal(u.x, u.y);
+    }
+    {
+        TileWeights<EIN, H, 1> w;
+        tile_load_weights<EIN, H, 1>(p.actor, w);
+        asm volatile("" ::: "memory");
+        ride_step<EIN, H, 1>(r, p.actor, rq, w);
+        tile_compute<EIN, H, 1, Lds>(p.actor, w, lds, row0, n, nullptr, nullptr, p.gauss ? 0 : 1, p.scale, p.base);
+        asm volatile("s_waitcnt vmcnt(0)" ::: "memory");
+        __syncthreads();
+        if (tid == 0) __hip_atomic_fetch_add(r.sync, 1u, __ATOMIC_RELAXED, __HIP_MEMORY_SCOPE_AGENT);
+    }
+
+    float st[kStats];
+#pragma unroll
+    for (int k = 0; k < kStats; ++k) st[k] = 0.0f;
+    float iters_f = 0.0f;
+    const int i = row0 + tid;
+    if (tid < kLanes && i < n) {
+        const float eps_t = fmaxf(p.act.eps_end, p.act.eps_start - p.act.eps_decay * (float)t);
+        float ap = lds.out[tid * 2];
+        if (p.gauss) ap = rpo_head_dev::gauss_head_row(ap, lds.out[tid * 2 + 1], draw, p.scale, p.base, p.act.box_lo, p.act.box_hi, 0, nullptr);
+        int k;
+        typename ENV::ActArgs act = p.act;
+        if (philox_noise) {
+            ap = rpo_explore_clip(ap, eps_t, draw, p.act.box_lo, p.act.box_hi);
+            act.noise_mode = RPO_NOISE_NONE;
+        }
+        const float2 a = ENV::project(act, c, lds.in_s + tid * kInS, i, ap, eps_t, t, k);
+        iters_f = (float)k;
+        reinterpret_cast<float2*>(p.act.action)[i] = a;
+        const long long ring_base = p.step.rows ? (t % p.step.cap_steps) * (long long)n : 0;
+        ENV::lane(p.step, c, i, lds.in_s + tid * kInS, a, ep, ring_base, st);
+    }
+    if (p.step.stats && tid < 64) {
+        float* srow = rpo_stats_row(p.step.stats, p.step.stats_cap, t);
+        const int slot[kStats + 1] = {RPO_STAT_REWARD_SUM, RPO_STAT_EPISODES, RPO_STAT_RETURN_SUM, RPO_STAT_LENGTH_SUM,
+                                      RPO_STAT_MAX_INEQ_SUM, RPO_STAT_MAX_EQ_SUM, RPO_STAT_VIOL_COUNT, RPO_STAT_TERMINATED,
+                                      RPO_STAT_MAX_INEQ_MAX, RPO_STAT_MAX_EQ_MAX, RPO_STAT_PROJ_ITERS};
+        float red[kStats + 1];
+#pragma unroll
+        for (int k = 0; k < kStats; ++k) red[k] = st[k];
+        red[kStats] = iters_f;
+        rpo_row16_reduce_many(red, 3u << 8);
+        rpo_stats_commit(red, 3u << 8, slot, srow);
+    }
+    if (!p.defer_clock) rpo_step_epilogue_at(p.step.ctrl, t, p.step.stats, p.step.stats_cap, blockIdx.x, (unsigned)r.n_roll);
 }
 
 template <class ENV>
@@ -759,6 +908,59 @@
                                        ctrl, max_episode_steps, auto_reset, viol_thresh, (uint64_t)seed,
                                        (uint32_t)env_id_base, 0};
     return launch_rollout<CartEnv>(args, c, n_envs, stream);
+}
+
+int rpo_cartsafe_rollout_adam(const rpo_mlp* actor_host, int gauss, float scale, float base, int n_envs, float* state,
+                              float* action, int* ep_len, float* ep_ret, unsigned* ep_count, float* rows, long long cap_steps,
+                              float* stats, int stats_cap, long long* ctrl, int noise_mode, float eps_start, float eps_end,
+                              float eps_decay, float box_lo, float box_hi, int max_steps, float corr_lr, float corr_eps,
+                              float corr_momentum, const float* consts_host, int partial, int max_episode_steps,
+                              int auto_reset, float viol_thresh, unsigned long long seed, unsigned env_id_base, int defer_clock,
+                              const rpo_adam_seg* adam, long long shared_begin, unsigned* ride_sync, unsigned* gave_up,
+                              void* stream) {
+    if (!actor_host || !adam) return RPO_ERR_NULL;
+    if (n_envs <= 0 || max_episode_steps <= 0 || max_steps < 0) return RPO_ERR_ARG;
+    if (noise_mode != RPO_NOISE_NONE && noise_mode != RPO_NOISE_PHILOX && noise_mode != RPO_NOISE_CLIP_ONLY) return RPO_ERR_ARG;
+    if (!state || !action || !ep_len || !ep_ret || !ep_count || !ctrl || !ride_sync || !gave_up) return RPO_ERR_NULL;
+    if ((rows && cap_steps <= 0) || (stats && stats_cap <= 0)) return RPO_ERR_ARG;
+    if ((reinterpret_cast<uintptr_t>(ride_sync) & 127u) != 0) return RPO_ERR_ARG;
+    const rpo_adam_seg& g = *adam;
+    if (g.n <= 0 || g.n > (1ll << 20) || !g.prepared || g.polyak_only || g.target2 || g.n2 != 0) return RPO_ERR_ARG;
+    if (!g.param || !g.grad || !g.exp_avg || !g.exp_avg_sq || !g.step_dev) return RPO_ERR_NULL;
+    if (g.clip_thres > 0.0f && !g.gradmax) return RPO_ERR_NULL;
+    RolloutArgs<CartEnv> args{};
+    args.actor = to_dev(actor_host);
+    if (int e = check_actor(args.actor, 6, gauss)) return e;
+    const Mlp& a = args.actor;
+    const int sel = rpo_tune(RPO_TUNE_ROLLOUT_WIDE);
+    if (a.E != 128 || a.l1_vec || !a.bs || !(sel == 0 || (sel == 2 && n_envs < 64 * 192))) return RPO_ERR_ARG;
+    if (shared_begin < 0 || shared_begin >= g.n) return RPO_ERR_ARG;
+    const float *lo = g.param + shared_begin, *hi = g.param + g.n;
+    if (a.Ws < lo || a.Ws + (size_t)a.E * a.S > hi || a.bs < lo || a.bs + a.E > hi) return RPO_ERR_ARG;
+    const float* outside[] = {a.W0, a.b0, a.W1, a.b1, a.W1b, a.b1b};
+    for (const float* q : outside)
+        if (q && q >= g.param && q < hi) return RPO_ERR_ARG;
+    CartConsts c;
+    if (int e = load_consts(c, consts_host, partial)) return e;
+    args.scale = scale; args.base = base; args.gauss = gauss; args.defer_clock = defer_clock ? 1 : 0;
+    args.act = rpo_cart_dev::ActArgs{n_envs, nullptr, nullptr, action, nullptr, noise_mode, eps_start, eps_end, eps_decay,
+                                     box_lo, box_hi, max_steps, corr_lr, corr_eps, corr_momentum, (uint64_t)seed,
+                                     (uint32_t)env_id_base, ctrl, stats, stats_cap};
+    args.step = rpo_cart_dev::StepArgs{n_envs, state, action, ep_len, ep_ret, ep_count, rows, cap_steps, stats, stats_cap,
+                                       ctrl, max_episode_steps, auto_reset, viol_thresh, (uint64_t)seed,
+                                       (uint32_t)env_id_base, 0};
+    AdamRide r{};
+    r.adam = rpo_adam_dev::AdamArgs{g.n, g.param, g.grad, g.exp_avg, g.exp_avg_sq, g.step_dev, g.lr, g.beta1, g.beta2, g.eps,
+                                    g.weight_decay, g.maximize, g.clip_thres, g.gradmax, g.reset_gradmax, g.zero_grad,
+                                    g.clamp_min0, g.target, g.tau, nullptr, nullptr, 0, 0, nullptr, 1};
+    const int n_adam = (int)((g.n + kFwdThreads - 1) / kFwdThreads);
+    r.shared_lo = shared_begin; r.sync = ride_sync; r.gave_up = gave_up;
+    r.n_roll = (n_envs + 15) / 16;
+    r.n_owners = n_adam - (int)(shared_begin / kFwdThreads);
+    hipLaunchKernelGGL((rollout_adam_kernel<CartEnv, 128, 256>), dim3(r.n_roll + n_adam), dim3(kFwdThreads), 0,
+                       (hipStream_t)stream, args, c, r);
+    RPO_LAUNCH_CHECK();
+    return 0;
 }
 
 int rpo_pendulum_rollout(const rpo_mlp* actor_host, int gauss, float scale, float base, int n_envs, float* internal,
diff --git a/rpo_amd/csrc/train_ops.hip b/rpo_amd/csrc/train_ops.hip
--- a/rpo_amd/csrc/train_ops.hip
+++ b/rpo_amd/csrc/train_ops.hip
@@ -1,5 +1,6 @@
 #include <stdlib.h>
 #include "common.h"
+#include "adam_dev.h"
 #include "heads_dev.h"
 
 namespace {
@@ -60,34 +61,12 @@
     }
 }
 
-struct AdamArgs {
-    long long n;
-    float* param;
-    float* grad;
-    float* m;
-    float* v;
-    int* step_dev;
-    float lr, beta1, beta2, eps, weight_decay;
-    int maximize;
-    float clip_thres;
-    float* gradmax;
-    int reset_gradmax;
-    int zero_grad;
-    int clamp_min0;
-    float* target;
-    float tau;
-    long long* arrive;
-    float* target2;
-    long long n2;
-    int polyak_only;
-    long long* clock;
-    int prepared;
-};
+using rpo_adam_dev::AdamArgs;
 
 __device__ __forceinline__ void adam_body(const AdamArgs& p) {
     if (p.polyak_only) {
         for (long long i = (long long)blockIdx.x * RPO_BLOCK + threadIdx.x; i < p.n; i += (long long)gridDim.x * RPO_BLOCK)
-            p.target[i] = p.target[i] * (1.0f - p.tau) + p.param[i] * p.tau;
+            p.target[i] = rpo_adam_dev::adam_polyak(p.target[i], p.param[i], p.tau);
         return;
     }
     const long long i0 = (long long)blockIdx.x * RPO_BLOCK + threadIdx.x, stride = (long long)gridDim.x * RPO_BLOCK;
@@ -98,43 +77,16 @@
         if (p.target2 && i0 < p.n2) t20 = p.target2[i0];
     }
     asm volatile("" ::: "memory");
-    float gm = 0.0f;
-    if (p.clip_thres > 0.0f) {
-#pragma unroll
-        for (int j = 0; j < RPO_GRADMAX_SLOTS; ++j) gm = fmaxf(gm, p.gradmax[j * (RPO_GRADMAX_LEN / RPO_GRADMAX_SLOTS)]);
-    }
-    const int step = p.prepared ? p.step_dev[0] : p.step_dev[0] + 1;
+    const rpo_adam_dev::AdamCoef k = rpo_adam_dev::adam_prologue(p);
+    const int step = k.step;
     double* cache = reinterpret_cast<double*>(p.step_dev + 4);
-    double bc1 = cache[0], bc2s = cache[1];
-    if (bc1 == 0.0 || p.step_dev[1] != step) {
-        bc1 = 1.0 - pow((double)p.beta1, (double)step);
-        bc2s = sqrt(1.0 - pow((double)p.beta2, (double)step));
-    }
-    const float step_size = (float)((double)p.lr / bc1);
-    const float bc2_sqrt = (float)bc2s;
-    const float coef = p.clip_thres > 0.0f ? fminf(p.clip_thres / (gm + 1e-6f), 1.0f) : 1.0f;
-    const float omb1 = 1.0f - p.beta1, omb2 = 1.0f - p.beta2;
     for (long long i = i0; i < p.n; i += stride) {
         if (i != i0) {
             g0 = p.grad[i]; w0 = p.param[i]; m0 = p.m[i]; v0 = p.v[i];
             if (p.target) t0 = p.target[i];
             if (p.target2 && i < p.n2) t20 = p.target2[i];
         }
-        float g = g0 * coef;
-        if (p.zero_grad) p.grad[i] = 0.0f;
-        else if (p.clip_thres > 0.0f) p.grad[i] = g;
-        if (p.maximize) g = -g;
-        float w = w0;
-        if (p.weight_decay != 0.0f) g += p.weight_decay * w;
-        float m = m0, v = v0;
-        m = m + (g - m) * omb1;
-        v = v * p.beta2 + omb2 * g * g;
-        const float denom = sqrtf(v) / bc2_sqrt + p.eps;
-        w = w - step_size * (m / denom);
-        if (p.clamp_min0) w = fmaxf(w, 0.0f);
-        p.param[i] = w; p.m[i] = m; p.v[i] = v;
-        if (p.target) p.target[i] = t0 * (1.0f - p.tau) + w * p.tau;
-        if (p.target2 && i < p.n2) p.target2[i] = t20 * (1.0f - p.tau) + w * p.tau;
+        rpo_adam_dev::adam_store(p, i, rpo_adam_dev::adam_element(p, k, g0, w0, m0, v0), t0, t20);
     }
     if (p.prepared) return;
     __syncthreads();
diff --git a/rpo_amd/ops.py b/rpo_amd/ops.py
--- a/rpo_amd/ops.py
+++ b/rpo_amd/ops.py
@@ -174,6 +174,12 @@
 
 
 def adam_step_multi(segs, clock=None, prepared=False):
+    arr = _adam_seg_array(segs, prepared)
+    check(_lib.load().rpo_adam_step_multi(len(segs), arr, _p(clock, torch.int64, allow_none=True), _stream()),
+          "rpo_adam_step_multi")
+
+
+def _adam_seg_array(segs, prepared=False):
     arr = (_AdamSegStruct * len(segs))()
     vp = lambda t, dt=torch.float32: None if t is None else _p(t, dt).value
     for a, g in zip(arr, segs):
@@ -191,8 +197,7 @@
         a.gradmax, a.reset_gradmax = vp(g.get("gradmax")), int(g.get("reset_gradmax", True))
         a.zero_grad, a.clamp_min0 = int(g.get("zero_grad", False)), int(g.get("clamp_min0", False))
         a.prepared = int(bool(prepared))
-    check(_lib.load().rpo_adam_step_multi(len(segs), arr, _p(clock, torch.int64, allow_none=True), _stream()),
-          "rpo_adam_step_multi")
+    return arr
 
 
 def min_q_bwd(q1, q2, scale, dq1, dq2):
@@ -425,6 +430,26 @@
             eps_start, eps_end, eps_decay, box_lo, box_hi, max_steps, corr_lr, corr_eps, corr_momentum, self._cptr,
             self.partial, max_episode_steps, int(auto_reset), viol_thresh, seed, env_id_base, int(defer_clock), _stream()),
             "rpo_cartsafe_rollout")
+
+    @staticmethod
+    def rollout_adam_ok(actor_desc, n_envs):
+        sel = tuning.get("rollout_wide")
+        return bool(actor_desc.E == 128 and (sel == 0 or (sel == 2 and n_envs < 64 * 192)))
+
+    def rollout_adam(self, actor_desc, gauss, scale, base, internal, obs, action, ep_len, ep_ret, ep_count, rows, cap_steps,
+                     stats, ctrl, noise_mode, eps_start, eps_end, eps_decay, box_lo, box_hi, max_steps, corr_lr, corr_eps,
+                     corr_momentum, max_episode_steps, auto_reset, viol_thresh, seed, env_id_base, defer_clock=False,
+                     adam=None, shared_begin=0, ride_sync=None, gave_up=None):
+        net = actor_desc.net_struct()
+        seg = _adam_seg_array([adam], prepared=True)
+        check(_lib.load().rpo_cartsafe_rollout_adam(
+            ctypes.byref(net), int(gauss), scale, base, internal.shape[0], _p(internal), _p(action),
+            _p(ep_len, torch.int32), _p(ep_ret), _p(ep_count, torch.int32), _ring(rows, self.ring_floats), cap_steps,
+            _p(stats, allow_none=True), 0 if stats is None else stats.shape[0], _p(ctrl, torch.int64), noise_mode,
+            eps_start, eps_end, eps_decay, box_lo, box_hi, max_steps, corr_lr, corr_eps, corr_momentum, self._cptr,
+            self.partial, max_episode_steps, int(auto_reset), viol_thresh, seed, env_id_base, int(defer_clock), seg,
+            int(shared_begin), _p(ride_sync, torch.int32), _p(gave_up, torch.int32), _stream()),
+            "rpo_cartsafe_rollout_adam")
 
     def evaluate(self, actor_desc, gauss, scale, base, internal, obs, action, ep_len, ep_ret, ep_count, ctrl, acc, t0, steps,
                  box_lo, box_hi, max_steps, corr_lr, corr_eps, corr_momentum, max_episode_steps, viol_thresh, trace=None,
```

After: 99.91 million env-steps/s. 0.979x the previous value.
